# ChenWu98/cycle-diffusion

Measured on NVIDIA H100. Metric: images/sec (512x512, 50-step encode+decode) at 1/2/4/8 H100; ms/U-Net-call, higher is better.
Workload: dtype fp32

## Files before the change

cycle_diffusion_b200/_cabi.py:

```python
import ctypes as C
import os

HERE = os.path.dirname(os.path.abspath(__file__))
LIB_PATH = os.path.join(HERE, 'libcdx.so')

CDX_UNET_OPENAI = 1
CDX_UNET_IDDPM = 2
CDX_UNET_DDPM = 3
CDX_TEXT_OPENCLIP = 4
CDX_PRED_EPS = 0
CDX_PRED_V = 1


class UnetConfig(C.Structure):
    _fields_ = [('kind', C.c_int), ('in_channels', C.c_int), ('out_channels', C.c_int), ('model_channels', C.c_int),
                ('num_res_blocks', C.c_int), ('n_mult', C.c_int), ('channel_mult', C.c_int * 8), ('n_attn', C.c_int),
                ('attention_ds', C.c_int * 8), ('num_heads', C.c_int), ('num_head_channels', C.c_int),
                ('context_dim', C.c_int)]


class VaeConfig(C.Structure):
    _fields_ = [('ch', C.c_int), ('n_mult', C.c_int), ('ch_mult', C.c_int * 8), ('num_res_blocks', C.c_int),
                ('in_channels', C.c_int), ('out_ch', C.c_int), ('z_channels', C.c_int), ('embed_dim', C.c_int), ('vq', C.c_int), ('n_embed', C.c_int)]


class TextConfig(C.Structure):
    _fields_ = [('vocab_size', C.c_int), ('width', C.c_int), ('layers', C.c_int), ('heads', C.c_int), ('max_len', C.c_int),
                ('mlp_width', C.c_int), ('kind', C.c_int), ('dim_head', C.c_int), ('proj_dim', C.c_int), ('patch', C.c_int), ('image_size', C.c_int)]


class DdimCoef(C.Structure):
    _fields_ = [('sqrt_at', C.c_float), ('sqrt_1m_at', C.c_float), ('sqrt_1m_at_tab', C.c_float),
                ('sqrt_aprev', C.c_float), ('dir_coef', C.c_float), ('sigma', C.c_float)]


class PixelCoef(C.Structure):
    _fields_ = [('ddpm', C.c_int), ('sqrt_at', C.c_float), ('sqrt_1m_at', C.c_float), ('sqrt_at_next', C.c_float),
                ('c1', C.c_float), ('c2', C.c_float), ('w0', C.c_float), ('wt', C.c_float), ('post_std', C.c_float),
                ('weight', C.c_float), ('inv_sqrt_1m_bt', C.c_float), ('std_model', C.c_float), ('mask', C.c_float)]


_P = C.c_void_p


class AttnControl(C.Structure):
    _fields_ = [('cross_steps', C.c_int), ('self_steps', C.c_int), ('self_max_tokens', C.c_int), ('token_map', C.c_void_p)]


class GemmDesc(C.Structure):
    _fields_ = [('mode', C.c_int), ('M', C.c_int), ('N', C.c_int), ('K', C.c_int),
                ('A', _P), ('lda', C.c_int), ('C1', C.c_int), ('A2', _P), ('lda2', C.c_int), ('C2', C.c_int),
                ('Hin', C.c_int), ('Win', C.c_int), ('Hout', C.c_int), ('Wout', C.c_int), ('stride', C.c_int), ('pad', C.c_int),
                ('w', _P), ('ldb', C.c_int), ('b_kn', C.c_int), ('bias', _P),
                ('rowvec', _P), ('ld_rowvec', C.c_int), ('rows_per_batch', C.c_int), ('residual', _P), ('ldr', C.c_int),
                ('alpha', C.c_float), ('geglu', C.c_int), ('out_nchw', C.c_int), ('rows_per_img', C.c_int),
                ('C', _P), ('ldc', C.c_int), ('C_lo', _P), ('Ct_hi', _P), ('Ct_lo', _P), ('t_col0', C.c_int), ('ldt', C.c_int64),
                ('a_amax', _P), ('a2_amax', _P), ('c_amax', _P), ('c_stats', _P), ('w_range', C.c_float),
                ('batch', C.c_int), ('heads', C.c_int),
                ('sA_b', C.c_int64), ('sA_h', C.c_int64), ('sB_b', C.c_int64), ('sB_h', C.c_int64), ('sC_b', C.c_int64), ('sC_h', C.c_int64),
                ('up', C.c_int)]


class AttentionNetDesc(C.Structure):
    _fields_ = [('kind', C.c_int), ('causal', C.c_int), ('qkv', C.c_void_p), ('q', C.c_void_p), ('kv', C.c_void_p), ('k', C.c_void_p),
                ('v', C.c_void_p), ('B', C.c_int), ('N', C.c_int), ('L', C.c_int), ('ctx_lp', C.c_int), ('heads', C.c_int), ('d', C.c_int),
                ('scale', C.c_float), ('qk_rows', C.POINTER(C.c_int)), ('kv_rows', C.POINTER(C.c_int)), ('acc_rows', C.POINTER(C.c_int)),
                ('n_acc', C.c_int), ('slot', C.c_float), ('q_slot', C.c_float), ('out', C.c_void_p),
                ('probe_rows', C.POINTER(C.c_int)), ('probe_spans', C.POINTER(C.c_int)), ('n_probe', C.c_int), ('probe_map', C.c_void_p)]


class LatentChain(C.Structure):
    _fields_ = [('row', C.c_int), ('row2', C.c_int), ('scale', C.c_float)]


class LatentChainsDesc(C.Structure):
    _fields_ = [('chw', C.c_int), ('n_src', C.c_int), ('K', C.c_int), ('rows', C.c_int), ('chains', C.POINTER(LatentChain)), ('src', C.c_int),
                ('x0', _P), ('eout', _P), ('c', DdimCoef), ('noise0', _P), ('sa', C.c_float), ('s1', C.c_float), ('xt', _P), ('xn', _P),
                ('next', C.c_int), ('noise_next', _P), ('cnext', DdimCoef), ('xn2', _P), ('z_out', _P), ('z_stride', C.c_int64),
                ('eps_in', _P), ('eps_stride', C.c_int64), ('yt', _P), ('y_out', _P), ('xin', _P), ('pred', C.c_int), ('vsa', C.c_float),
                ('vs1', C.c_float), ('mask', _P), ('hw', C.c_int),
                ('sg_m', C.c_int), ('sg_rows', C.POINTER(C.c_int)), ('sg_thr', _P), ('sg_nu', _P), ('sg_scale', C.c_float * 8),
                ('sg_lambda', C.c_float * 8), ('sg_active', C.c_uint), ('sg_apply', C.c_int), ('sg_mu', C.c_float), ('sg_beta', C.c_float),
                ('sg_beta1', C.c_float)]


class LatentChainsMaskDesc(LatentChainsDesc):
    _fields_ = [('sg_map', _P), ('sg_mask', C.c_int), ('sg_gh', C.c_int), ('sg_gw', C.c_int), ('w', C.c_int)]


class DpmCoef(C.Structure):
    _fields_ = [('a', C.c_float), ('b', C.c_float), ('c', C.c_float), ('n', C.c_float), ('order', C.c_int)]


class LatentChainsSamplerDesc(LatentChainsMaskDesc):
    _fields_ = [('solver', C.c_int), ('dc', DpmCoef), ('d_src', _P), ('d_tgt', _P), ('qa', C.c_float), ('q1', C.c_float)]


CDX_SAMPLER_DDIM_POSTERIOR = 0
CDX_SAMPLER_DDIM_DRAWS = 1
CDX_SAMPLER_DPMSOLVER_DRAWS = 2


class SamplerC(C.Structure):
    _fields_ = [('kind', C.c_int), ('dpm', C.POINTER(DpmCoef)), ('qa', C.POINTER(C.c_float)), ('q1', C.POINTER(C.c_float))]


class MutualControlC(C.Structure):
    _fields_ = [('start_step', C.c_int), ('start_layer', C.c_int)]


class PnpControlC(C.Structure):
    _fields_ = [('feature_steps', C.c_int), ('attention_steps', C.c_int), ('attention_start_layer', C.c_int),
                ('feature_blocks', C.POINTER(C.c_int)), ('n_feature_blocks', C.c_int)]


CDX_SEMANTIC_MAX = 8


class SemanticGuidanceC(C.Structure):
    _fields_ = [('m', C.c_int), ('scale', C.c_float * CDX_SEMANTIC_MAX), ('threshold', C.c_float * CDX_SEMANTIC_MAX),
                ('cooldown', C.c_int * CDX_SEMANTIC_MAX), ('warmup', C.c_int), ('momentum_scale', C.c_float), ('beta', C.c_float),
                ('beta1', C.c_float)]


class SemanticAttnMaskC(C.Structure):
    _fields_ = [('intersect', C.c_int), ('n_tokens', C.c_int * CDX_SEMANTIC_MAX)]


_F = C.c_float
_I = C.c_int
_S = C.c_size_t

SIGNATURES = {
    'cdx_abi_version': (_I, []),
    'cdx_last_error': (C.c_char_p, []),
    'cdx_engine_create': (_I, [_I, C.POINTER(_P)]),
    'cdx_engine_destroy': (None, [_P]),
    'cdx_engine_workspace_bytes': (_S, [_P]),
    'cdx_engine_launch_count': (C.c_uint64, [_P]),
    'cdx_engine_set_mma_mode': (_I, [_P, _I]),
    'cdx_engine_profile': (_I, [_P, _I]),
    'cdx_engine_profile_read': (_I, [_P, _I, C.POINTER(C.c_double), C.POINTER(C.c_double), C.POINTER(C.c_double), C.POINTER(C.c_uint64)]),
    'cdx_unet_create': (_I, [_P, C.POINTER(UnetConfig), C.POINTER(_P)]),
    'cdx_vae_create': (_I, [_P, C.POINTER(VaeConfig), C.POINTER(_P)]),
    'cdx_text_create': (_I, [_P, C.POINTER(TextConfig), C.POINTER(_P)]),
    'cdx_net_destroy': (None, [_P]),
    'cdx_net_num_params': (_I, [_P]),
    'cdx_net_param_name': (C.c_char_p, [_P, _I]),
    'cdx_net_param_shape': (_I, [_P, _I, C.POINTER(C.c_int64)]),
    'cdx_net_load_param': (_I, [_P, C.c_char_p, _P, _I, C.POINTER(C.c_int64), _I]),
    'cdx_net_finalize': (_I, [_P]),
    'cdx_net_weight_blob': (_I, [_P, C.POINTER(_P), C.POINTER(_S)]),
    'cdx_net_adopt_blob': (_I, [_P]),
    'cdx_unet_set_time_freqs': (_I, [_P, C.POINTER(_F), _I]),
    'cdx_unet_set_prediction': (_I, [_P, _I, C.POINTER(_F), C.POINTER(_F), _I]),
    'cdx_unet_forward': (_I, [_P, _P, _P, _P, _I, _P, _I, _I, _I, _P]),
    'cdx_vae_encode': (_I, [_P, _P, _P, _I, _I, _P]),
    'cdx_text_encode': (_I, [_P, _P, _I, _I, _P, _P]),
    'cdx_vae_decode': (_I, [_P, _P, _P, _I, _I, _P]),
    'cdx_vae_encode_hw': (_I, [_P, _P, _P, _I, _I, _I, _P]),
    'cdx_vae_decode_hw': (_I, [_P, _P, _P, _I, _I, _I, _P]),
    'cdx_affine': (_I, [_P, _P, _F, _F, _P, _S, _P]),
    'cdx_shift_scale': (_I, [_P, _P, _F, _F, _P, _S, _P]),
    'cdx_q_sample': (_I, [_P, _P, _P, _F, _F, _P, _S, _P]),
    'cdx_vae_posterior': (_I, [_P, _P, _P, _F, _P, _I, _I, _I, _P]),
    'cdx_ddim_posterior_sample': (_I, [_P, _P, _P, _P, C.POINTER(DdimCoef), _P, _S, _P]),
    'cdx_ddim_compute_eps': (_I, [_P, _P, _P, _P, _P, _F, C.POINTER(DdimCoef), _P, _S, _P]),
    'cdx_ddim_step_with_eps': (_I, [_P, _P, _P, _P, _F, _P, C.POINTER(DdimCoef), _P, _S, _P]),
    'cdx_pixel_posterior_sample': (_I, [_P, _P, _P, _P, C.POINTER(PixelCoef), _P, _S, _P]),
    'cdx_pixel_compute_eps': (_I, [_P, _P, _P, _P, C.POINTER(PixelCoef), _P, _I, _I, _I, _P]),
    'cdx_pixel_step_with_eps': (_I, [_P, _P, _P, _P, C.POINTER(PixelCoef), _P, _I, _I, _I, _P]),
    'cdx_latent_encode': (_I, [_P, _P, _P, _P, _I, _F, C.POINTER(DdimCoef), C.POINTER(_F), _I, _I, _P, _F, _F, _P, _I, _I,
                               _I, _I, _P]),
    'cdx_latent_decode': (_I, [_P, _P, _I, _P, _P, _I, _F, C.POINTER(DdimCoef), C.POINTER(_F), _I, _P, _P, _I, _I, _I, _I,
                               _P]),
    'cdx_cycle_lockstep': (_I, [_P, _P, _P, _P, _P, _I, _F, _F, C.POINTER(DdimCoef), C.POINTER(_F), _I, _P, _F, _F, _P, _P, _I, _I, _I, _I,
                                _P]),
    'cdx_cycle_lockstep_masked': (_I, [_P, _P, _P, _P, _P, _I, _F, _F, C.POINTER(DdimCoef), C.POINTER(_F), _I, _P, _F, _F, _P, _P, _I, _I, _I,
                                       _I, _P, _P]),
    'cdx_cycle_lockstep_ctl': (_I, [_P, _P, _P, _P, _P, _I, _F, _F, C.POINTER(DdimCoef), C.POINTER(_F), _I, _P, _F, _F, _P, _P, _I, _I, _I,
                                    _I, _P, _P, C.POINTER(AttnControl)]),
    'cdx_cycle_lockstep_refine': (_I, [_P, _P, _P, _P, _P, _I, _F, _F, C.POINTER(DdimCoef), C.POINTER(_F), _I, _P, _F, _F, _P, _P, _I, _I,
                                       _I, _I, _P, _P, C.POINTER(AttnControl), _P]),
    'cdx_cycle_lockstep_mutual': (_I, [_P, _P, _P, _P, _P, _I, _F, _F, C.POINTER(DdimCoef), C.POINTER(_F), _I, _P, _F, _F, _P, _P, _I, _I,
                                       _I, _I, _P, _P, _I, _I]),
    'cdx_cycle_lockstep_pnp': (_I, [_P, _P, _P, _P, _P, _I, _F, _F, C.POINTER(DdimCoef), C.POINTER(_F), _I, _P, _F, _F, _P, _P, _I, _I,
                                    _I, _I, _P, _P, _I, _I, _I, C.POINTER(_I), _I]),
    'cdx_cycle_lockstep_semantic': (_I, [_P, _P, _P, _P, _P, _I, _F, _F, C.POINTER(DdimCoef), C.POINTER(_F), _I, _P, _F, _F, _P, _P, _I, _I,
                                         _I, _I, _P, _P, _P, C.POINTER(SemanticGuidanceC)]),
    'cdx_cycle_lockstep_semantic_attn': (_I, [_P, _P, _P, _P, _P, _I, _F, _F, C.POINTER(DdimCoef), C.POINTER(_F), _I, _P, _F, _F, _P, _P, _I,
                                              _I, _I, _I, _P, _P, _P, C.POINTER(SemanticGuidanceC), C.POINTER(SemanticAttnMaskC)]),
    'cdx_cycle_lockstep_sampler': (_I, [_P, _P, _P, _P, _P, _I, _F, _F, C.POINTER(DdimCoef), C.POINTER(_F), _I, _P, _F, _F, _P, _P, _I, _I,
                                        _I, _I, _P, C.POINTER(SamplerC), _P, C.POINTER(AttnControl), _P, C.POINTER(MutualControlC),
                                        C.POINTER(PnpControlC), _P, C.POINTER(SemanticGuidanceC), C.POINTER(SemanticAttnMaskC)]),
    'cdx_mask_pool': (_I, [_P, _P, _P, _I, _I, _I, _I, _P]),
    'cdx_mask_composite': (_I, [_P, _P, _P, _P, _P, _I, _I, _I, _I, _P]),
    'cdx_edit_map': (_I, [_P, _P, _P, _P, _I, _F, _F, _F, _P, _I, _I, _P, _I, _I, _I, _I, _P]),
    'cdx_edit_map_from_eps': (_I, [_P, _P, _P, _F, _I, _I, _P, _I, _I, _I, _I, _P]),
    'cdx_edit_mask': (_I, [_P, _P, _I, _F, _P, _P, _P, _I, _I, _I, _I, _I, _P]),
    'cdx_latent_loop_ens': (_I, [_P, _I, _P, _P, _P, _P, _I, _P, _P, C.POINTER(DdimCoef), C.POINTER(_F), _I, _I, _P, _F, _F, _P, _I, _P, _P, _P,
                                 _I, _I, _I, _I, _P]),
    'cdx_clip_preprocess': (_I, [_P, _P, _I, _I, _I, _P, _P]),
    'cdx_clip_image_features': (_I, [_P, _P, _I, _P, _P]),
    'cdx_text_features': (_I, [_P, _P, _I, _I, _P, _P]),
    'cdx_dclip_scores': (_I, [_P, _P, _P, _P, _P, _I, _I, _P, _P, _P]),
    'cdx_image_metrics': (_I, [_P, _P, _P, _I, _I, _I, _P, _P]),
    'cdx_pixel_encode': (_I, [_P, _P, C.POINTER(PixelCoef), C.POINTER(_F), _I, _P, _F, _F, _P, _I, _I, _I, _P]),
    'cdx_pixel_decode': (_I, [_P, _P, _I, C.POINTER(PixelCoef), C.POINTER(_F), _I, _P, _P, _I, _I, _I, _P]),
    'cdx_pixel_cycle_lockstep': (_I, [_P, _P, _P, C.POINTER(PixelCoef), C.POINTER(_F), _I, _I, _P, _F, _F, _P, _I, _I, _I, _P]),
    'cdx_latent_cycle_pair': (_I, [_P, _P, _P, C.POINTER(DdimCoef), C.POINTER(_F), _I, _I, _P, _F, _F, _P, _P, _I, _I, _I, _I, _P]),
    'cdx_latent_cycle_fan': (_I, [_P, _I, _I, _P, _P, _P, _P, _I, C.POINTER(_F), C.POINTER(_F), C.POINTER(DdimCoef), C.POINTER(_F), _I, _P,
                                  _F, _F, _P, _P, _I, _I, _I, _P]),
    'cdx_latent_cycle_fan_masked': (_I, [_P, _I, _I, _P, _P, _P, _P, _I, C.POINTER(_F), C.POINTER(_F), C.POINTER(DdimCoef), C.POINTER(_F), _I,
                                         _P, _F, _F, _P, _P, _I, _I, _I, _P, _P]),
    'cdx_ensemble_select': (_I, [_P, _I, _P, _P, _P, _P, _P, _P, _P, _P, _I, _I, _I, _I, _P]),
    'cdx_op_conv3x3': (_I, [_P, _P, _P, _P, _P, _I, _I, _I, _I, _I, _I, _I, _I, _P]),
    'cdx_op_linear': (_I, [_P, _P, _P, _P, _P, _I, _I, _I, _P]),
    'cdx_op_groupnorm': (_I, [_P, _P, _P, _P, _F, _I, _P, _I, _I, _I, _P]),
    'cdx_op_layernorm': (_I, [_P, _P, _P, _P, _P, _I, _I, _P]),
    'cdx_op_attention': (_I, [_P, _P, _P, _P, _P, _I, _I, _I, _I, _I, _F, _P]),
    'cdx_op_attention_rows': (_I, [_P, _P, _P, _P, _P, _I, _I, _I, _I, _I, _F, C.POINTER(_I), _P]),
    'cdx_op_attention_kv_rows': (_I, [_P, _P, _P, _P, _P, _I, _I, _I, _I, _I, _F, C.POINTER(_I), _P]),
    'cdx_op_attention_accum': (_I, [_P, _P, _P, _P, _P, _I, _I, _I, _I, _I, _F, C.POINTER(_I), _I, _P]),
    'cdx_op_nchw_to_nhwc': (_I, [_P, _P, _P, _I, _I, _I, _P]),
    'cdx_op_nhwc_to_nchw': (_I, [_P, _P, _P, _I, _I, _I, _P]),
    'cdx_op_groupnorm_ex': (_I, [_P, _P, _I, _P, _I, _P, _P, _F, _I, _P, _P, _I, _P, _P, _P, _I, _I, _P]),
    'cdx_op_groupnorm_rows': (_I, [_P, _P, _I, _P, _I, _P, _P, _F, _I, _P, _P, _I, C.POINTER(_I), _P, _P, _P, _P, _I, _I, _P]),
    'cdx_op_layernorm_ex': (_I, [_P, _P, _P, _P, _P, _P, _I, _I, _P]),
    'cdx_op_softmax_rows': (_I, [_P, _P, C.c_int64, _I, _I, _I, _P]),
    'cdx_op_produce_norm': (_I, [_P, _P, _P, _P, _I, _I, _I, _I, _I, _I, _P, _P, _F, _P, _P, _P, _P, C.POINTER(_I), _P]),
    'cdx_op_gemm': (_I, [_P, C.POINTER(GemmDesc), C.POINTER(_I), _P]),
    'cdx_op_attention_net': (_I, [_P, C.POINTER(AttentionNetDesc), C.POINTER(_I), _P]),
    'cdx_op_latent_chains': (_I, [_P, C.POINTER(LatentChainsDesc), _I, _P]),
    'cdx_op_pixel_lockstep': (_I, [_P, _P, _P, _P, _P, _P, _P, C.POINTER(PixelCoef), _I, _I, _I, _I, _P]),
}


def _load():
    if not os.path.exists(LIB_PATH):
        raise ImportError(
            f'{LIB_PATH} is missing: build it with `python -c "import __graft_entry__ as g; g.build()"` '
            f'(nvcc, sm_90a).  The engine has no CPU fallback.')
    lib = C.CDLL(LIB_PATH)
    for name, (res, args) in SIGNATURES.items():
        fn = getattr(lib, name)
        fn.restype = res
        fn.argtypes = args
    return lib


lib = _load()


class CdxError(RuntimeError):
    pass


def check(rc):
    if rc == 0:
        return
    msg = (lib.cdx_last_error() or b'').decode('utf-8', 'replace')
    if rc == -1:
        raise AssertionError(msg)
    raise CdxError(f'libcdx error {rc}: {msg}')
```

cycle_diffusion_b200/csrc/cabi.cu:

```cuda
#include <stdio.h>
#include <stdlib.h>
#include <string.h>

#include <algorithm>

#include "nets.cuh"

struct cdx_engine { cdx::Engine e; };
struct cdx_net { cdx::Net* n; cdx_engine* owner; };

namespace cdx {
const std::string& last_error();

namespace {

template <class F>
int guard(F&& f) {
  try {
    f();
    return CDX_OK;
  } catch (const Error& err) {
    set_last_error(err.what());
    return err.code;
  } catch (const std::exception& err) {
// ... 220 lines not shown
              p.start_layer >= 0 && p.n_blocks >= 0 && (p.blocks || p.n_blocks == 0),
              "Plug-and-Play: feature_steps=%d attention_steps=%d (of %d) attention_start_layer=%d n_blocks=%d", p.feature_steps,
              p.attention_steps, a.n_steps, p.start_layer, p.n_blocks);
    const int n_out = unet.ucfg.n_mult * (unet.ucfg.num_res_blocks + 1);
    for (int i = 0; i < p.n_blocks; ++i) {
      CDX_CHECK(p.blocks[i] >= 0 && p.blocks[i] < n_out, "Plug-and-Play: feature block %d outside the net's %d output blocks", p.blocks[i], n_out);
      for (int j = 0; j < i; ++j) CDX_CHECK(p.blocks[j] != p.blocks[i], "Plug-and-Play: feature block %d given twice", p.blocks[i]);
    }
  }
  const int solver = a.sampler ? a.sampler->kind : 0;
  if (solver) {
    const cdx_sampler& sp = *a.sampler;
    CDX_CHECK(solver == CDX_SAMPLER_DDIM_DRAWS || solver == CDX_SAMPLER_DPMSOLVER_DRAWS, "sampler: kind %d", solver);
    CDX_CHECK(a.src && a.K > 0 && a.n_rec == a.n_steps && !tgt_net && a.noise,
              "edit-friendly inversion: needs the lock-step loop with a source chain at every step");
    CDX_CHECK(sp.qa && sp.q1 && sp.qa[0] == a.sa && sp.q1[0] == a.s1,
              "edit-friendly inversion: the draw scalars qa / q1 must be given, their step 0 the x_T scalars");
    if (solver == CDX_SAMPLER_DPMSOLVER_DRAWS) {
      CDX_CHECK(sp.dpm, "SDE-DPM-Solver++: null coefficient table");
      for (int i = 0; i < a.n_steps; ++i) {
        const cdx_dpm_coef& d = sp.dpm[i];
        CDX_CHECK(d.n > 0.f && std::isfinite(d.n) && (d.order == 1 || d.order == 2), "SDE-DPM-Solver++: step %d n=%g order %d", i, d.n, d.order);
        CDX_CHECK(i > 0 || d.order == 1, "SDE-DPM-Solver++: order %d on the loop's first step (no previous x0-prediction)", d.order);
      }
    }
  }
  Scope sc(e.arena);
  unet.ctxkv.valid = false;
  struct Invalidate { Net& u; ~Invalidate() { u.ctxkv.valid = false; } } inval{unet};
  float* xin = (float*)e.arena.alloc((size_t)rows * chw * sizeof(float));
  float* eout = (float*)e.arena.alloc((size_t)rows * chw * sizeof(float));
  float* ctx_in = (float*)e.arena.alloc((size_t)rows * ctx_n * sizeof(float));
  float* xb[3] = {nullptr, nullptr, nullptr};
  float* yb[2] = {nullptr, nullptr};
  if (a.src) for (float*& p : xb) p = (float*)e.arena.alloc(n * sizeof(float));
  if (a.K) for (float*& p : yb) p = (float*)e.arena.alloc((size_t)n_tgt_chains * chw * sizeof(float));
  float* tdev = (float*)e.arena.alloc((size_t)std::max(loop_steps, 1) * rows * sizeof(float));
  Chain* chd = (Chain*)e.arena.alloc(ch.size() * sizeof(Chain));
  upload_timesteps(e, a.t_host, loop_steps, rows, tdev, s);
  if (!e.dry()) {
    CDX_CUDA(cudaMemcpyAsync(chd, ch.data(), ch.size() * sizeof(Chain), cudaMemcpyHostToDevice, s));
    auto scales_to = [&](Chain* c, const float* scales, int count) {
      CDX_CUDA(cudaMemcpy2DAsync(&c->scale, sizeof(Chain), scales, sizeof(float), sizeof(float), count, cudaMemcpyDeviceToDevice, s));
    };
    if (a.scales_on_device && a.src) scales_to(chd, a.s_scales, a.n_src);
    if (a.scales_on_device && a.K) scales_to(chd + a.n_src, a.t_scales, n_tgt_chains);
  }
  if (ctx_n) {
    auto ctx_rows = [&](const Chain& c, const float* cond, int j) {
      const bool uncond_only = a.uc && !a.scales_on_device && c.scale == 0.0f;
      copy_dd(e, (uncond_only ? a.uc : cond) + j * ctx_n, ctx_in + (size_t)c.row * ctx_n, ctx_n, s);
      if (c.row2 >= 0) copy_dd(e, a.uc + j * ctx_n, ctx_in + (size_t)c.row2 * ctx_n, ctx_n, s);
    };
    for (int j = 0; j < a.n_src; ++j) {
      if (a.src) ctx_rows(ch[j], a.c_src, j);
      for (int k = 0; k < a.K; ++k) ctx_rows(ch[a.n_src + (size_t)j * a.K + k], a.c_tgt, j);
    }
    for (int t = 0; t < n_tgt_chains; ++t)
      for (int q = 0; q < sg_m; ++q)
        copy_dd(e, a.c_edit + ((size_t)(t / a.K) * sg_m + q) * ctx_n, ctx_in + (size_t)sg_rows[(size_t)t * sg_m + q] * ctx_n, ctx_n, s);
  }
  int* sg_rows_dev = nullptr;
  float *sg_thr = nullptr, *sg_nu = nullptr;
  AttnProbe probe;
  const int sg_mask = a.sega_mask ? 1 + (a.sega_mask->intersect != 0) : 0, gh = a.h / 4, gw = a.w / 4;
  if (sg_m) {
    sg_rows_dev = (int*)e.arena.alloc(sg_rows.size() * sizeof(int));
    sg_thr = (float*)e.arena.alloc(sg_rows.size() * std::max(a.C, 2) * sizeof(float));
    sg_nu = (float*)e.arena.alloc((size_t)n_tgt_chains * chw * sizeof(float));
    if (!e.dry()) {
      CDX_CUDA(cudaMemcpyAsync(sg_rows_dev, sg_rows.data(), sg_rows.size() * sizeof(int), cudaMemcpyHostToDevice, s));
      CDX_CUDA(cudaMemsetAsync(sg_nu, 0, (size_t)n_tgt_chains * chw * sizeof(float), s));
    }
  }
  if (sg_mask) {
    std::vector<int> span(sg_rows.size());
    for (size_t r = 0; r < span.size(); ++r) span[r] = a.sega_mask->n_tokens[r % sg_m];
    int* span_dev = (int*)e.arena.alloc(span.size() * sizeof(int));
    if (!e.dry()) CDX_CUDA(cudaMemcpyAsync(span_dev, span.data(), span.size() * sizeof(int), cudaMemcpyHostToDevice, s));
    probe.rows = sg_rows_dev; probe.span = span_dev; probe.n_rows = (int)sg_rows.size(); probe.tokens = gh * gw;
    probe.map = (float*)e.arena.alloc(sg_rows.size() * gh * gw * sizeof(float));
  }
  AttnControl actl;
  if (a.ctl) {
    std::vector<int> qk(rows);
    for (int r = 0; r < rows; ++r) qk[r] = r;
    for (int j = 0; j < a.n_src; ++j) {
      CDX_CHECK(!a.uc || ch[j].scale != 0.0f, "attention control: the source chain at scale 0 has no source-prompt row");
      for (int k = 0; k < a.K; ++k) {
        const Chain& t = ch[a.n_src + (size_t)j * a.K + k];
        CDX_CHECK(!a.uc || t.scale != 0.0f, "attention control: the target chain at scale 0 has no target-prompt row");
        qk[t.row] = ch[j].row;
      }
    }
    int* qk_dev = (int*)e.arena.alloc((size_t)rows * sizeof(int));
    if (!e.dry()) CDX_CUDA(cudaMemcpyAsync(qk_dev, qk.data(), qk.size() * sizeof(int), cudaMemcpyHostToDevice, s));
    actl.qk_row = qk_dev;
    actl.self_max_tokens = a.ctl->self_max_tokens;
    auto ctx_products = [&](const float* A, float* out) {
      const int D = unet.ucfg.context_dim;
      ExactFp32 exact(e);
      for (int j = 0; j < a.n_src; ++j)
        for (int k = 0; k < a.K; ++k) {
          GemmArgs g;
          g.mode = 0;
          g.M = a.L; g.N = D; g.K = a.L;
          g.A = A + (size_t)j * a.L * a.L; g.lda = a.L; g.C1 = a.L;
          g.Bw = a.c_tgt + (size_t)j * ctx_n; g.ldb = D; g.b_kn = 1;
          g.Cout = out + (size_t)ch[a.n_src + (size_t)j * a.K + k].row * ctx_n; g.ldc = D;
          gemm(e, g, s);
        }
    };
    if (a.ctl->token_map) {
      float* cv = (float*)e.arena.alloc((size_t)rows * ctx_n * sizeof(float));
      copy_dd(e, ctx_in, cv, (size_t)rows * ctx_n, s);
      ctx_products(a.ctl->token_map, cv);
      actl.ctx_v = cv;
    }
    if (a.own_weight) {
      float* cw = (float*)e.arena.alloc((size_t)rows * ctx_n * sizeof(float));
      float* dg = (float*)e.arena.alloc((size_t)a.n_src * a.L * a.L * sizeof(float));
      std::vector<int> own;
      for (int j = 0; j < a.n_src; ++j)
        for (int k = 0; k < a.K; ++k) own.push_back(ch[a.n_src + (size_t)j * a.K + k].row);
      int* own_dev = (int*)e.arena.alloc(own.size() * sizeof(int));
      if (!e.dry()) {
        CDX_CUDA(cudaMemcpyAsync(own_dev, own.data(), own.size() * sizeof(int), cudaMemcpyHostToDevice, s));
        CDX_CUDA(cudaMemsetAsync(cw, 0, (size_t)rows * ctx_n * sizeof(float), s));
        CDX_CUDA(cudaMemsetAsync(dg, 0, (size_t)a.n_src * a.L * a.L * sizeof(float), s));
        for (int j = 0; j < a.n_src; ++j)
          CDX_CUDA(cudaMemcpy2DAsync(dg + (size_t)j * a.L * a.L, (size_t)(a.L + 1) * sizeof(float), a.own_weight + (size_t)j * a.L, sizeof(float),
                                     sizeof(float), a.L, cudaMemcpyDeviceToDevice, s));
      }
      ctx_products(dg, cw);
      actl.ctx_w = cw;
      actl.own_rows = own_dev;
      actl.n_own = (int)own.size();
    }
  }
  if (a.mutual || a.pnp) {
    std::vector<int> src_row(rows);
    for (int r = 0; r < rows; ++r) src_row[r] = r;
    for (int j = 0; j < a.n_src; ++j)
      for (int k = 0; k < a.K; ++k) {
        const Chain& t = ch[a.n_src + (size_t)j * a.K + k];
        src_row[t.row] = ch[j].row;
        if (t.row2 >= 0) src_row[t.row2] = ch[j].row2 >= 0 ? ch[j].row2 : ch[j].row;
      }
    int* dev = (int*)e.arena.alloc((size_t)rows * sizeof(int));
    if (!e.dry()) CDX_CUDA(cudaMemcpyAsync(dev, src_row.data(), src_row.size() * sizeof(int), cudaMemcpyHostToDevice, s));
    if (a.mutual) {
      actl.kv_row = dev;
      actl.start_layer = a.start_layer;
    } else {
      actl.pnp_row = dev;
      actl.pnp_layer = a.pnp->start_layer;
      actl.feat_blocks = a.pnp->blocks;
      actl.n_feat = a.pnp->n_blocks;
    }
  }
  auto next_kind = [&](int i_next) {
    if (i_next >= a.n_rec) return 0;
    return (a.n_steps - 1 - i_next) == 0 ? 2 : solver ? 3 : 1;
  };
  float *d_src = nullptr, *d_tgt = nullptr;
  if (solver == CDX_SAMPLER_DPMSOLVER_DRAWS) {
    d_src = (float*)e.arena.alloc(n * sizeof(float));
    d_tgt = (float*)e.arena.alloc((size_t)n_tgt_chains * chw * sizeof(float));
  }
  const int n_given = a.src ? a.n_rec : a.n_eps;
  LatentChains f;
  f.n = n; f.chw = chw; f.n_src = a.n_src; f.K = a.K; f.chains = chd; f.x0 = a.x0; f.xin = xin; f.mask = a.mask; f.hw = a.h * a.w;
  f.z_stride = (long long)(a.n_rec + 1) * chw;
  f.solver = solver; f.d_src = d_src; f.d_tgt = d_tgt;
  if (sg_m) {
    const cdx_semantic_guidance& g = *a.sega;
    f.sg_m = sg_m; f.sg_rows = sg_rows_dev; f.sg_thr = sg_thr; f.sg_nu = sg_nu;
    for (int q = 0; q < sg_m; ++q) { f.sg_scale[q] = g.scale[q]; f.sg_lambda[q] = g.threshold[q]; }
    f.sg_mu = g.momentum_scale; f.sg_beta = g.beta; f.sg_beta1 = g.beta1;
    f.sg_mask = sg_mask; f.sg_map = probe.map; f.sg_gh = gh; f.sg_gw = gw; f.w = a.w;
  }
  {
    LatentChains in = f;
    in.src = a.src;
    in.noise0 = a.noise; in.sa = a.sa; in.s1 = a.s1; in.z_out = a.z_out;
    in.eps_in = a.z_in; in.eps_stride = (long long)(a.n_eps + 1) * chw;
    in.xt = xb[0]; in.xn = xb[1]; in.yt = yb[0];
    in.next = a.src ? next_kind(0) : 0;
    if (in.next) { in.noise_next = a.noise + n; in.cnext = a.coef[0]; }
    if (in.next == 3) { in.qa = a.sampler->qa[1]; in.q1 = a.sampler->q1[1]; }
    latent_chains_init(e, in, s);
  }
  const int iters = e.dry() ? std::min(loop_steps, 1) : loop_steps;
  PairStreams ps(e, tgt_net ? *tgt_net->eng : e, s);
  for (int i = 0; i < iters; ++i) {
    const bool src_i = a.src && i < a.n_rec;
    if (!tgt_net) {
      actl.cross = a.ctl && i < a.ctl->cross_steps;
      actl.self = a.ctl && i < a.ctl->self_steps;
      actl.mutual = a.mutual && i >= a.start_step;
      actl.pnp_feat = a.pnp && i < a.pnp->feature_steps;
      actl.pnp_attn = a.pnp && i < a.pnp->attention_steps;
      const size_t stat0 = e.stat_dry;
      unet_forward(unet, xin, tdev + (size_t)i * rows, ctx_in, a.L, eout, rows, a.h, a.w, s, true,
                   a.ctl || a.mutual || a.pnp ? &actl : nullptr, sg_mask ? &probe : nullptr);
      CDX_CHECK(!sg_m || !e.dry() || e.stat_dry - stat0 <= e.stat_cap,
                "semantic guidance: a %d-row U-Net call needs %zu GroupNorm statistics doubles, the pool holds %zu: fewer images or concepts",
                rows, e.stat_dry - stat0, e.stat_cap);
    } else {
      ps.fork();
      if (src_i) unet_forward(unet, xin, tdev + (size_t)i * rows, nullptr, 0, eout, rows_src, a.h, a.w, s);
      unet_forward(*tgt_net, xin + (size_t)rows_src * chw, tdev + (size_t)i * rows + rows_src, nullptr, 0, eout + (size_t)rows_src * chw,
                   rows - rows_src, a.h, a.w, ps.target_stream());
      ps.join();
    }
    LatentChains st = f;
    st.src = src_i; st.eout = eout; st.c = a.coef[i];
    if (src_i) {
      st.xt = xb[0]; st.xn = xb[1]; st.xn2 = xb[2];
      if (a.z_out) st.z_out = a.z_out + (size_t)(1 + i) * chw;
      st.next = next_kind(i + 1);
      if (st.next) { st.noise_next = a.noise + (size_t)(2 + i) * n; st.cnext = a.coef[i + 1]; }
      if (st.next == 3) { st.qa = a.sampler->qa[i + 2]; st.q1 = a.sampler->q1[i + 2]; }
      if (solver == CDX_SAMPLER_DPMSOLVER_DRAWS) st.dc = a.sampler->dpm[i];
    } else if (i < n_given) {
      st.eps_in = a.z_in + (size_t)(1 + i) * chw; st.eps_stride = (long long)(a.n_eps + 1) * chw;
    } else {
      st.eps_in = a.extra + (size_t)(i - n_given) * n; st.eps_stride = chw;
    }
    st.yt = yb[0]; st.y_out = (i == loop_steps - 1) ? a.x_out : yb[1];
    set_v(unet, a.t_host[i], st);
    if (sg_m) {
      for (int q = 0; q < sg_m; ++q) st.sg_active |= (unsigned)(i < a.sega->cooldown[q]) << q;
      st.sg_apply = i >= a.sega->warmup;
      semantic_thresholds(e, st, s);
    }
    latent_chains_step(e, st, s);
    if (src_i) { float* t0 = xb[0]; xb[0] = xb[1]; xb[1] = xb[2]; xb[2] = t0; }
    std::swap(yb[0], yb[1]);
  }
}

void run_edit_map(Net& unet, const float* x0, const float* c_src, const float* c_tgt, int L, float t, float sa, float s1, const float* noise,
                  int n_maps, int rows_per_call, float* acc, int B, int C, int h, int w, cudaStream_t s) {
  Engine& e = *unet.eng;
  const int chw = C * h * w, hw = h * w, n_pairs = n_maps * B, per_call = std::min(rows_per_call / 2, n_pairs), rows = 2 * per_call;
  const size_t ctx_n = (size_t)L * unet.ucfg.context_dim;
  check_v_steps(unet, &t, 1);
  const float vscale = unet.pred ? unet.sa_v[(int)t] : 1.f;
  Scope sc(e.arena);
  float* xin = (float*)e.arena.alloc((size_t)rows * chw * sizeof(float));
  float* eout = (float*)e.arena.alloc((size_t)rows * chw * sizeof(float));
  float* ctx_in = (float*)e.arena.alloc((size_t)rows * ctx_n * sizeof(float));
  float* tdev = (float*)e.arena.alloc((size_t)rows * sizeof(float));
  upload_timesteps(e, &t, 1, rows, tdev, s);
  if (!e.dry()) CDX_CUDA(cudaMemsetAsync(acc, 0, (size_t)B * hw * sizeof(float), s));
  const int calls = e.dry() ? 1 : cdiv(n_pairs, per_call);
  for (int c = 0; c < calls; ++c) {
    const int p0 = c * per_call, p1 = std::min(p0 + per_call, n_pairs), nr = 2 * (p1 - p0);
    for (int q = p0; q < p1; ++q) {
      const int b = q % B, r = 2 * (q - p0);
      copy_dd(e, c_src + (size_t)b * ctx_n, ctx_in + (size_t)r * ctx_n, ctx_n, s);
      copy_dd(e, c_tgt + (size_t)b * ctx_n, ctx_in + (size_t)(r + 1) * ctx_n, ctx_n, s);
    }
    edit_rows(e, x0, noise, sa, s1, xin, B, n_maps, chw, p0, p1, s);
    const size_t stat0 = e.stat_dry;
    unet_forward(unet, xin, tdev, ctx_in, L, eout, nr, h, w, s);
    CDX_CHECK(!e.dry() || e.stat_dry - stat0 <= e.stat_cap,
              "edit_map: a %d-row U-Net call needs %zu GroupNorm statistics doubles, the pool holds %zu: lower rows_per_call", nr,
              e.stat_dry - stat0, e.stat_cap);
    edit_map_accum(e, eout, eout + chw, 2LL * chw, 2LL * B * chw, 2LL * p0 * chw, vscale, acc, B, C, hw, p0, p1, s);
  }
}

}
}

using namespace cdx;

static inline cdx::Engine& engine_of(cdx_engine* h) { return h->e; }

extern "C" {

int cdx_abi_version(void) { return CDX_ABI_VERSION; }
const char* cdx_last_error(void) { return cdx::last_error().c_str(); }

int cdx_engine_create(int device, cdx_engine** out) {
  return guard([&] {
    CDX_CHECK(out != nullptr, "engine_create: null out");
    int count = 0;
    cudaError_t err = cudaGetDeviceCount(&count);
    if (err != cudaSuccess || count <= 0)
      throw Error(CDX_E_CUDA, std::string("no usable CUDA device (there is no CPU fallback): ") + cudaGetErrorString(err));
    CDX_CHECK(device >= 0 && device < count, "engine_create: device %d out of range (count %d)", device, count);
    CDX_CUDA(cudaSetDevice(device));
    cudaDeviceProp prop;
    CDX_CUDA(cudaGetDeviceProperties(&prop, device));
    cdx_engine* eng = new cdx_engine();
    eng->e.device = device;
    if (prop.major != 9 || prop.minor != 0)
      throw Error(CDX_E_CUDA, "libcdx is built for sm_90a (H100) only; device " + std::to_string(device) + " is sm_" +
                                  std::to_string(prop.major) + std::to_string(prop.minor));
    eng->e.num_sms = prop.multiProcessorCount;
    *out = eng;
  });
}
void cdx_engine_destroy(cdx_engine* e) {
  if (!e) return;
  cudaSetDevice(e->e.device);
  cudaDeviceSynchronize();
  e->e.arena.destroy();
  if (e->e.done_ev) cudaEventDestroy(e->e.done_ev);
  if (e->e.side) cudaStreamDestroy(e->e.side);
  if (e->e.fork_ev) cudaEventDestroy(e->e.fork_ev);
  if (e->e.join_ev) cudaEventDestroy(e->e.join_ev);
  if (e->e.amax_pool) cudaFree(e->e.amax_pool);
  delete e;
}
size_t cdx_engine_workspace_bytes(const cdx_engine* e) { return e ? e->e.arena.cap : 0; }
uint64_t cdx_engine_launch_count(const cdx_engine* e) { return e ? e->e.launches : 0; }
int cdx_engine_set_mma_mode(cdx_engine* e, int mode) {
  return guard([&] {
    CDX_CHECK(e != nullptr && mode >= 0 && mode <= 5, "set_mma_mode: bad arguments");
    e->e.mma_mode = mode == 0 ? 0 : 1;
    e->e.flash_attn = mode != 2 && mode != 0;
    e->e.tc_kind = mode == 3 ? 0 : mode >= 4 ? 2 : 1;
    e->e.attn_one = mode == 5;
  });
}

int cdx_engine_profile(cdx_engine* e, int enable) {
  return guard([&] {
    CDX_CHECK(e != nullptr, "profile: null engine");
    CDX_CUDA(cudaSetDevice(e->e.device));
    CDX_CUDA(cudaDeviceSynchronize());
    for (ProfRec& r : e->e.prof.recs) { cudaEventDestroy(r.a); cudaEventDestroy(r.b); }
    e->e.prof.recs.clear();
    e->e.prof.on = enable != 0;
  });
}
int cdx_engine_profile_read(cdx_engine* e, int tag, double* ms, double* flops, double* bytes, uint64_t* launches) {
  return guard([&] {
    CDX_CHECK(e && ms && flops && bytes && launches && tag >= 0 && tag < PROF_NTAGS, "profile_read: bad arguments");
    CDX_CUDA(cudaSetDevice(e->e.device));
    CDX_CUDA(cudaDeviceSynchronize());
    *ms = 0; *flops = 0; *bytes = 0; *launches = 0;
    const bool dump = getenv("CDX_PROF_DUMP") != nullptr;
    for (const ProfRec& r : e->e.prof.recs) {
      if (r.tag != tag) continue;
      float t = 0.f;
      CDX_CUDA(cudaEventElapsedTime(&t, r.a, r.b));
      if (dump) fprintf(stderr, "[cdx prof] tag %d  %8.3f ms  %8.1f GFLOP  %7.1f TF/s  %s\n", tag, t, r.flops * 1e-9, t > 0 ? r.flops / (t * 1e9) : 0.0, r.note);
      *ms += t; *flops += r.flops; *bytes += r.bytes; *launches += (uint64_t)r.launches;
    }
  });
}

int cdx_unet_create(cdx_engine* e, const cdx_unet_config* cfg, cdx_net** out) {
  return guard([&] {
    CDX_CHECK(cfg && out, "unet_create: null argument");
    cdx_net* h = new cdx_net();
    h->owner = e;
    static Engine host_only;
    h->n = make_unet(e ? &e->e : &host_only, *cfg);
    *out = h;
  });
}
int cdx_vae_create(cdx_engine* e, const cdx_vae_config* cfg, cdx_net** out) {
  return guard([&] {
    CDX_CHECK(cfg && out, "vae_create: null argument");
    cdx_net* h = new cdx_net();
    h->owner = e;
    static Engine host_only;
    h->n = make_vae(e ? &e->e : &host_only, *cfg);
    *out = h;
  });
}
int cdx_text_create(cdx_engine* e, const cdx_text_config* cfg, cdx_net** out) {
  return guard([&] {
    CDX_CHECK(cfg && out, "text_create: null argument");
    cdx_net* h = new cdx_net();
    h->owner = e;
    static Engine host_only;
    h->n = make_text(e ? &e->e : &host_only, *cfg);
    *out = h;
  });
}
void cdx_net_destroy(cdx_net* n) {
  if (!n) return;
  destroy_net(n->n);
  delete n;
}
int cdx_net_num_params(const cdx_net* n) { return n ? (int)n->n->params.size() : 0; }
const char* cdx_net_param_name(const cdx_net* n, int i) {
  if (!n || i < 0 || i >= (int)n->n->params.size()) return nullptr;
  return n->n->params[i].name.c_str();
}
int cdx_net_param_shape(const cdx_net* n, int i, int64_t dims[4]) {
  if (!n || i < 0 || i >= (int)n->n->params.size()) return CDX_E_INVALID;
  const Param& p = n->n->params[i];
  for (int k = 0; k < 4; ++k) dims[k] = k < p.rank ? p.dims[k] : 1;
  return p.rank;
}
int cdx_net_load_param(cdx_net* n, const char* name, const float* data, int on_device, const int64_t* dims, int rank) {
  return guard([&] {
    CDX_CHECK(n && n->owner && name && data && dims, "load_param: null argument (nets created without an engine are inventory-only)");
    net_load_param(*n->n, name, data, on_device != 0, dims, rank);
  });
}
int cdx_net_finalize(cdx_net* n) {
  return guard([&] {
    CDX_CHECK(n && n->owner, "finalize: null / inventory-only net");
    net_finalize(*n->n);
  });
}
int cdx_net_weight_blob(cdx_net* n, void** dev_ptr, size_t* bytes) {
  return guard([&] {
    CDX_CHECK(n && n->owner && dev_ptr && bytes, "weight_blob: null argument");
    net_ensure_blob(*n->n);
    *dev_ptr = n->n->blob;
    *bytes = n->n->blob_floats * sizeof(float);
  });
}
int cdx_net_adopt_blob(cdx_net* n) {
  return guard([&] {
    CDX_CHECK(n && n->owner, "adopt_blob: null / inventory-only net");
    net_ensure_blob(*n->n);
    for (Param& p : n->n->params) p.loaded = true;
    n->n->planes_valid = false;
    n->n->ctxkv.valid = false;
    n->n->finalized = false;
    net_finalize(*n->n);
  });
}
int cdx_unet_set_time_freqs(cdx_net* n, const float* freqs, int half) {
  return guard([&] {
    CDX_CHECK(n && freqs, "set_time_freqs: null argument");
    CDX_CHECK(n->n->kind != NET_VAE, "set_time_freqs on a VAE");
    CDX_CHECK(half == n->n->ucfg.model_channels / 2, "set_time_freqs: half=%d, expected %d", half, n->n->ucfg.model_channels / 2);
    n->n->freqs_host.assign(freqs, freqs + half);
    if (n->n->finalized) net_finalize(*n->n);
  });
}

int cdx_unet_set_prediction(cdx_net* n, int prediction, const float* sa_v, const float* s1_v, int T) {
  return guard([&] {
    CDX_CHECK(n && n->n, "set_prediction: null net");
    CDX_CHECK(n->n->kind == NET_UNET_OPENAI, "set_prediction: SD / LDM U-Nets only");
    CDX_CHECK(prediction == CDX_PRED_EPS || prediction == CDX_PRED_V, "set_prediction: prediction %d", prediction);
    if (prediction == CDX_PRED_EPS) {
      n->n->pred = 0; n->n->sa_v.clear(); n->n->s1_v.clear();
      return;
    }
    CDX_CHECK(sa_v && s1_v && T > 0, "set_prediction: v needs both tables");
    n->n->sa_v.assign(sa_v, sa_v + T);
    n->n->s1_v.assign(s1_v, s1_v + T);
    n->n->pred = 1;
  });
}

int cdx_unet_forward(cdx_net* n, const float* x, const float* t_dev, const float* ctx, int ctx_len, float* out, int B, int H, int W,
                     void* stream) {
  return guard([&] {
    CDX_CHECK(n && n->owner && x && t_dev && out && B > 0, "unet_forward: bad arguments");
    with_arena(n->owner->e, S(stream), [&] { unet_forward(*n->n, x, t_dev, ctx, ctx_len, out, B, H, W, S(stream)); });
  });
}
int cdx_vae_encode_hw(cdx_net* n, const float* img, float* moments, int B, int H, int W, void* stream) {
  return guard([&] {
    CDX_CHECK(n && n->owner && img && moments && B > 0, "vae_encode: bad arguments");
    with_arena(n->owner->e, S(stream), [&] { vae_encode(*n->n, img, moments, B, H, W, S(stream)); });
  });
}
int cdx_vae_encode(cdx_net* n, const float* img, float* moments, int B, int R, void* stream) {
  return cdx_vae_encode_hw(n, img, moments, B, R, R, stream);
}
int cdx_text_encode(cdx_net* n, const int* ids, int B, int L, float* out, void* stream) {
  return guard([&] {
    CDX_CHECK(n && n->owner && ids && out && B > 0, "text_encode: bad arguments");
    with_arena(n->owner->e, S(stream), [&] { text_encode(*n->n, ids, out, B, L, S(stream)); });
  });
}
#define ENG_CALL_(EH_, ...)                                \
  return guard([&] {                                       \
    CDX_CHECK((EH_) != nullptr, "null engine");            \
    CDX_CUDA(cudaSetDevice(engine_of(EH_).device));        \
    __VA_ARGS__;                                           \
  })
int cdx_text_features(cdx_net* n, const int* ids, int B, int L, float* out, void* stream) {
  return guard([&] {
    CDX_CHECK(n && n->owner && ids && out && B > 0, "text_features: bad arguments");
    with_arena(n->owner->e, S(stream), [&] { text_features(*n->n, ids, out, B, L, S(stream)); });
  });
}
int cdx_clip_image_features(cdx_net* n, const float* pixels, int B, float* out, void* stream) {
  return guard([&] {
    CDX_CHECK(n && n->owner && pixels && out && B > 0, "clip_image_features: bad arguments");
    with_arena(n->owner->e, S(stream), [&] { clip_image_features(*n->n, pixels, out, B, S(stream)); });
  });
}
int cdx_clip_preprocess(cdx_engine* e, const float* img, int B, int R, int size, float* out, void* s) {
  ENG_CALL_(e, CDX_CHECK(img && out && B > 0 && R > 0 && size > 0, "clip_preprocess: bad arguments"); clip_preprocess(e->e, img, B, R, size, out, S(s)));
}
int cdx_dclip_scores(cdx_engine* e, const float* img_f, const float* orig_f, const float* enc_f, const float* dec_f, int B, int D, float* clip_out,
                     float* dclip_out, void* s) {
  ENG_CALL_(e, CDX_CHECK(img_f && orig_f && enc_f && dec_f && clip_out && dclip_out && B > 0 && D > 0, "dclip_scores: bad arguments");
            dclip_scores(e->e, img_f, orig_f, enc_f, dec_f, B, D, clip_out, dclip_out, S(s)));
}
int cdx_image_metrics(cdx_engine* eh, const float* a, const float* b, int B, int H, int W, float* out, void* stream) {
  return guard([&] {
    CDX_CHECK(eh && a && b && out && B > 0, "image_metrics: bad arguments");
    with_arena(eh->e, S(stream), [&] { image_metrics(eh->e, a, b, B, H, W, out, S(stream)); });
  });
}
int cdx_vae_decode_hw(cdx_net* n, const float* z, float* img, int B, int h, int w, void* stream) {
  return guard([&] {
    CDX_CHECK(n && n->owner && z && img && B > 0, "vae_decode: bad arguments");
    with_arena(n->owner->e, S(stream), [&] { vae_decode(*n->n, z, img, B, h, w, S(stream)); });
  });
}
int cdx_vae_decode(cdx_net* n, const float* z, float* img, int B, int h, void* stream) {
  return cdx_vae_decode_hw(n, z, img, B, h, h, stream);
}

#define ENG_CALL(EH_, ...)                                 \
  return guard([&] {                                       \
    CDX_CHECK((EH_) != nullptr, "null engine");            \
    CDX_CUDA(cudaSetDevice(engine_of(EH_).device));        \
    __VA_ARGS__;                                           \
  })

int cdx_affine(cdx_engine* e, const float* x, float a, float b, float* out, size_t n, void* s) { ENG_CALL(e, affine(e->e, x, a, b, out, n, S(s))); }
int cdx_shift_scale(cdx_engine* e, const float* x, float b, float a, float* out, size_t n, void* s) { ENG_CALL(e, shift_scale(e->e, x, b, a, out, n, S(s))); }
int cdx_q_sample(cdx_engine* e, const float* x0, const float* nz, float sa, float s1, float* out, size_t n, void* s) {
  ENG_CALL(e, q_sample(e->e, x0, nz, sa, s1, out, n, S(s)));
}
int cdx_vae_posterior(cdx_engine* e, const float* mom, const float* nz, float sf, float* out, int B, int C, int hw, void* s) {
  ENG_CALL(e, vae_posterior(e->e, mom, nz, sf, out, B, C, hw, S(s)));
}
int cdx_ddim_posterior_sample(cdx_engine* e, const float* x0, const float* xt, const float* nz, const cdx_ddim_coef* c, float* o, size_t n, void* s) {
  ENG_CALL(e, CDX_CHECK(c, "null coef"); ddim_posterior_sample(e->e, x0, xt, nz, *c, o, n, S(s)));
}
int cdx_ddim_compute_eps(cdx_engine* e, const float* xt, const float* xn, const float* e_c, const float* e_uc, float scale, const cdx_ddim_coef* c,
                         float* o, size_t n, void* s) {
  ENG_CALL(e, CDX_CHECK(c, "null coef"); ddim_compute_eps(e->e, xt, xn, e_c, e_uc, scale, *c, o, n, S(s)));
}
int cdx_ddim_step_with_eps(cdx_engine* e, const float* x, const float* e_c, const float* e_uc, float scale, const float* eps, const cdx_ddim_coef* c,
                           float* o, size_t n, void* s) {
  ENG_CALL(e, CDX_CHECK(c, "null coef"); ddim_step_with_eps(e->e, x, e_c, e_uc, scale, eps, *c, o, n, S(s)));
}
int cdx_pixel_posterior_sample(cdx_engine* e, const float* x0, const float* xt, const float* nz, const cdx_pixel_coef* c, float* o, size_t n, void* s) {
  ENG_CALL(e, CDX_CHECK(c, "null coef"); pixel_posterior_sample(e->e, x0, xt, nz, *c, o, n, S(s)));
}
int cdx_pixel_compute_eps(cdx_engine* e, const float* xt, const float* xn, const float* et, const cdx_pixel_coef* c, float* o, int B, int chw,
                          int net_chw, void* s) {
  ENG_CALL(e, CDX_CHECK(c, "null coef"); pixel_compute_eps(e->e, xt, xn, et, *c, o, B, chw, net_chw, S(s)));
}
int cdx_pixel_step_with_eps(cdx_engine* e, const float* xt, const float* et, const float* eps, const cdx_pixel_coef* c, float* o, int B, int chw,
                            int net_chw, void* s) {
  ENG_CALL(e, CDX_CHECK(c, "null coef"); pixel_step_with_eps(e->e, xt, et, eps, *c, o, B, chw, net_chw, S(s)));
}

int cdx_latent_encode(cdx_net* un, const float* x0, const float* c, const float* uc, int L, float scale, const cdx_ddim_coef* coef,
                      const float* t_host, int n_steps, int n_rec, const float* noise, float sqrt_a_T, float sqrt_1ma_T, float* z_out, int B,
                      int C, int h, int w, void* stream) {
  return guard([&] {
    CDX_CHECK(un && un->owner && x0 && (c || L == 0) && coef && t_host && noise && z_out, "latent_encode: null argument");
    CDX_CHECK(n_steps >= 1 && n_rec >= 0 && n_rec <= n_steps, "latent_encode: n_steps=%d n_rec=%d", n_steps, n_rec);
    for (int i = 0; i < n_rec; ++i) CDX_CHECK(coef[i].sigma > 0.f, "latent_encode: eta must be > 0 (sigma[%d] == 0), ddim.py:268", i);
    const std::vector<float> scales((size_t)std::max(B, 0), scale);
    ChainLoopArgs a;
    a.n_src = B; a.src = true;
    a.x0 = x0; a.c_src = c; a.uc = uc; a.L = L; a.s_scales = scales.data();
    a.coef = coef; a.t_host = t_host; a.n_steps = n_steps; a.n_rec = n_rec; a.noise = noise; a.sa = sqrt_a_T; a.s1 = sqrt_1ma_T;
    a.z_out = z_out; a.C = C; a.h = h; a.w = w;
    with_arena(un->owner->e, S(stream), [&] { run_latent_chains(*un->n, a, S(stream)); });
  });
}

int cdx_latent_decode(cdx_net* un, const float* z, int n_eps, const float* c, const float* uc, int L, float scale, const cdx_ddim_coef* coef,
                      const float* t_host, int n_steps, const float* extra_noise, float* x_out, int B, int C, int h, int w, void* stream) {
  return guard([&] {
    CDX_CHECK(un && un->owner && z && (c || L == 0) && coef && t_host && x_out, "latent_decode: null argument");
    CDX_CHECK(n_steps >= 1 && n_eps >= 0, "latent_decode: n_steps=%d n_eps=%d", n_steps, n_eps);
    CDX_CHECK(n_eps >= n_steps || extra_noise != nullptr, "latent_decode: %d steps but only %d recovered noises and no extra noise", n_steps, n_eps);
    const std::vector<float> scales((size_t)std::max(B, 0), scale);
    ChainLoopArgs a;
    a.n_src = B; a.K = 1;
    a.c_tgt = c; a.uc = uc; a.L = L; a.t_scales = scales.data();
    a.coef = coef; a.t_host = t_host; a.n_steps = n_steps;
    a.z_in = z; a.n_eps = n_eps; a.extra = extra_noise; a.x_out = x_out;
    a.C = C; a.h = h; a.w = w;
    with_arena(un->owner->e, S(stream), [&] { run_latent_chains(*un->n, a, S(stream)); });
  });
}

int cdx_cycle_lockstep(cdx_net* un, const float* x0, const float* c_src, const float* c_tgt, const float* uc, int L, float src_scale,
                       float tgt_scale, const cdx_ddim_coef* coef, const float* t_host, int n_steps, const float* noise, float sqrt_a_T,
                       float sqrt_1ma_T, float* x_out, float* z_out, int B, int C, int h, int w, void* stream) {
  return cdx_cycle_lockstep_masked(un, x0, c_src, c_tgt, uc, L, src_scale, tgt_scale, coef, t_host, n_steps, noise, sqrt_a_T, sqrt_1ma_T,
                                   x_out, z_out, B, C, h, w, stream, nullptr);
}

int cdx_cycle_lockstep_masked(cdx_net* un, const float* x0, const float* c_src, const float* c_tgt, const float* uc, int L, float src_scale,
                              float tgt_scale, const cdx_ddim_coef* coef, const float* t_host, int n_steps, const float* noise,
                              float sqrt_a_T, float sqrt_1ma_T, float* x_out, float* z_out, int B, int C, int h, int w, void* stream,
                              const float* mask) {
  return cdx_cycle_lockstep_ctl(un, x0, c_src, c_tgt, uc, L, src_scale, tgt_scale, coef, t_host, n_steps, noise, sqrt_a_T, sqrt_1ma_T,
                                x_out, z_out, B, C, h, w, stream, mask, nullptr);
}

int cdx_cycle_lockstep_ctl(cdx_net* un, const float* x0, const float* c_src, const float* c_tgt, const float* uc, int L, float src_scale,
                           float tgt_scale, const cdx_ddim_coef* coef, const float* t_host, int n_steps, const float* noise,
                           float sqrt_a_T, float sqrt_1ma_T, float* x_out, float* z_out, int B, int C, int h, int w, void* stream,
                           const float* mask, const cdx_attn_control* ctl) {
  return cdx_cycle_lockstep_refine(un, x0, c_src, c_tgt, uc, L, src_scale, tgt_scale, coef, t_host, n_steps, noise, sqrt_a_T, sqrt_1ma_T,
                                   x_out, z_out, B, C, h, w, stream, mask, ctl, nullptr);
}

static int cycle_lockstep(cdx_net* un, const float* x0, const float* c_src, const float* c_tgt, const float* uc, int L, float src_scale,
                          float tgt_scale, const cdx_ddim_coef* coef, const float* t_host, int n_steps, const float* noise, float sqrt_a_T,
                          float sqrt_1ma_T, float* x_out, float* z_out, int B, int C, int h, int w, void* stream, const float* mask,
                          const cdx_attn_control* ctl, const float* own_weight, bool mutual, int start_step, int start_layer,
                          const PnpLoop* pnp = nullptr, const cdx_semantic_guidance* sega = nullptr, const float* c_edit = nullptr,
                          const cdx_semantic_attn_mask* sega_mask = nullptr, const cdx_sampler* sampler = nullptr) {
  return guard([&] {
    CDX_CHECK(un && un->owner && x0 && c_src && c_tgt && coef && t_host && noise && x_out, "cycle_lockstep: null argument");
    CDX_CHECK(n_steps >= 1, "cycle_lockstep: n_steps=%d", n_steps);
    for (int i = 0; i < n_steps; ++i) CDX_CHECK(coef[i].sigma > 0.f, "cycle_lockstep: eta must be > 0 (sigma[%d] == 0), ddim.py:268", i);
    const std::vector<float> s_scales((size_t)std::max(B, 0), src_scale), t_scales((size_t)std::max(B, 0), tgt_scale);
// ... 911 lines not shown
```

cycle_diffusion_b200/csrc/common.cuh:

```cuda
#pragma once
#include <cuda_runtime.h>
#include <stdint.h>
#include <stdio.h>
#include <string>
#include <vector>
#include <stdexcept>

#include "../../include/cdx.h"

namespace cdx {

struct Error : std::runtime_error {
  int code;
  Error(int c, const std::string& m) : std::runtime_error(m), code(c) {}
};
void set_last_error(const std::string& m);

#define CDX_CHECK(cond, ...)                                                     \
  do {                                                                           \
    if (!(cond)) {                                                               \
      char _b[512];                                                              \
      snprintf(_b, sizeof(_b), __VA_ARGS__);                                     \
      throw ::cdx::Error(CDX_E_INVALID, std::string(_b) + " [" #cond "]");       \
    }                                                                            \
  } while (0)

#define CDX_CUDA(expr)                                                                         \
  do {                                                                                         \
    cudaError_t _e = (expr);                                                                   \
    if (_e != cudaSuccess) {                                                                   \
      char _b[512];                                                                            \
      snprintf(_b, sizeof(_b), "%s failed: %s (%s:%d)", #expr, cudaGetErrorString(_e), __FILE__, __LINE__); \
      throw ::cdx::Error(CDX_E_CUDA, _b);                                                      \
    }                                                                                          \
  } while (0)

struct Arena {
  char* base = nullptr;
  size_t cap = 0, off = 0, high = 0;
  bool dry = false;
  void* alloc(size_t bytes);
  size_t mark() const { return off; }
  void release(size_t m) { off = m; }
  void begin_dry();
  void end_dry();
  void destroy();
};

enum ProfTag {
  PROF_CONV_FFMA = 0, PROF_DENSE_FFMA = 1, PROF_BATCHED_FFMA = 2, PROF_CONV_TC = 3, PROF_DENSE_TC = 4, PROF_BATCHED_TC = 5,
  PROF_GROUPNORM = 6, PROF_LAYERNORM = 7, PROF_SOFTMAX = 8, PROF_ELEMENTWISE = 9, PROF_NTAGS = 10
};
struct ProfRec { cudaEvent_t a, b; int tag; double flops, bytes; int launches; char note[56]; };
struct Profiler {
  bool on = false;
  std::vector<ProfRec> recs;
  std::vector<cudaEvent_t> pool;
};

struct Engine {
  Profiler prof;
  int device = 0;
  int num_sms = 132;
  bool flash_attn = true;
  int mma_mode = 1;
  int tc_kind = 1;
  bool attn_one = false;
  float* amax_pool = nullptr;
  int amax_cap = 1 << 15, amax_used = 0, amax_high = 0;
  float* amax_slot();
  double* stat_pool = nullptr;
  size_t stat_cap = (size_t)8 << 20, stat_used = 0, stat_high = 0;
  size_t stat_dry = 0;
  double* stat_alloc(size_t n);
  void pools_reset(cudaStream_t s);
  Arena arena;
  cudaStream_t last_stream = nullptr;
  cudaEvent_t done_ev = nullptr;
  bool ev_recorded = false;
  cudaStream_t side = nullptr;
  cudaEvent_t fork_ev = nullptr, join_ev = nullptr;
  uint64_t launches = 0;
  bool dry() const { return arena.dry; }
};

struct ProfScope {
  Engine& e;
  cudaStream_t s;
  int idx = -1;
  ProfScope(Engine& eng, cudaStream_t st, int tag, double flops, double bytes, int launches);
  ~ProfScope();
  void note(const char* fmt, ...);
};

struct Scope {
  Arena& a;
  size_t m;
  explicit Scope(Arena& ar) : a(ar), m(ar.mark()) {}
  ~Scope() { a.release(m); }
};

struct Tensor {
  float* p = nullptr;
  int B = 0, H = 0, W = 0, C = 0;
  float* amax = nullptr;
  double* stats = nullptr;
  size_t numel() const { return (size_t)B * H * W * C; }
  int rows() const { return B * H * W; }
};
inline Tensor alloc_tensor(Engine& e, int B, int H, int W, int C) {
  Tensor t;
  t.B = B; t.H = H; t.W = W; t.C = C;
  t.p = (float*)e.arena.alloc(t.numel() * sizeof(float));
  return t;
}

struct GemmArgs {
  int M = 0, N = 0, K = 0;
  int mode = 0;
  const float* A = nullptr;  int lda = 0;  int C1 = 0;
  const float* A2 = nullptr; int lda2 = 0; int C2 = 0;
  int Hin = 0, Win = 0, Hout = 0, Wout = 0, stride = 1, pad = 1, up = 1;
  const float* Bw = nullptr; int ldb = 0; int b_kn = 0;
  const float* Bw_hi = nullptr; const float* Bw_lo = nullptr;
  const void* Bw_h_hi = nullptr; const void* Bw_h_lo = nullptr; int b_exp = 0;
  const float* a_amax = nullptr; const float* a2_amax = nullptr;
  float* c_amax = nullptr;
  double* c_stats = nullptr;
  float* Cout = nullptr; int ldc = 0;
  float* Cout_lo = nullptr;
  float* Ct_hi = nullptr; float* Ct_lo = nullptr; int t_col0 = 0; long long ldt = 0;
  const float* bias = nullptr;
  const float* rowvec = nullptr; int ld_rowvec = 0; int rows_per_batch = 1;
  const float* residual = nullptr; int ldr = 0;
  float alpha = 1.f;
  int geglu = 0;
  int out_nchw = 0;
  int rows_per_img = 0;
  int batch = 1, heads = 1;
  long long sA_b = 0, sA_h = 0, sB_b = 0, sB_h = 0, sC_b = 0, sC_h = 0;
};
void gemm(Engine& e, const GemmArgs& a, cudaStream_t s, int* route = nullptr);
bool gemm_tc(Engine& e, const GemmArgs& a, cudaStream_t s, int* side_done = nullptr);
enum { ROUTE_KIND_SS = 0, ROUTE_KIND_TS = 1, ROUTE_KIND_H16 = 2, ROUTE_KIND_H16_FAST = 3 };
inline int route_plan(int kind, int width, int splits) { return kind << 4 | width << 8 | splits << 16; }
bool flash_eligible(const Engine& e, int N, int Nk, int d, int C);
struct AttnPlanes {
  enum Fmt { TF32, H16 } fmt;
  const void* q_hi; const void* q_lo; int ldq;
  const void* k_hi; const void* k_lo; int ldk;
  const void* vt_hi; const void* vt_lo;
  const float* q_amax = nullptr; const float* k_amax = nullptr; const float* v_amax = nullptr;
};
bool flash_attention(Engine& e, const AttnPlanes& a, float* out, int ldo, int B, int N, int Nk, int Nks, int Nvs, int heads, int d, float scale,
                     cudaStream_t s, const int* qk_row = nullptr, const int* acc_rows = nullptr, int n_acc = 0, const int* kv_row = nullptr);
void split_rows_h16(Engine& e, const float* src, long long rows, int cols, long long ld, void* hi, void* lo, long long ldh, const float* amax,
                    cudaStream_t s);
void split_transpose_h16(Engine& e, const float* src, int R, int Cc, long long ld, void* hi, void* lo, const float* amax, cudaStream_t s,
                         int images = 1, int Rp = 0);
struct FlashPlan { int qrows, rag, ksplit, ring; };
FlashPlan flash_plan(int d, bool h16, bool one, int N);
bool self_attention_h16(Engine& e, const float* qkv, const float* slot, float* out, int B, int HW, int C, int heads, int d, float scale, bool lo,
                        cudaStream_t s, const int* qk_row, const int* kv_row, const int* acc_rows = nullptr, int n_acc = 0, int* Nvs_out = nullptr);
bool self_attention_tf32_padded(Engine& e, const float* qk_hi, const float* qk_lo, const float* vr, float* out, int B, int HW, int C, int heads,
                                int d, float scale, cudaStream_t s, const int* qk_row, const int* kv_row, const int* acc_rows = nullptr,
                                int n_acc = 0, int* Nvs_out = nullptr);
void context_split_h16(Engine& e, const float* kv, int Mk, int C, const float* slot, void* k_hi, void* k_lo, void* vt_hi, void* vt_lo,
                       cudaStream_t s);
struct ProbeOperands {
  enum Fmt { F32, H16, TF32 } fmt = F32;
  const float* q = nullptr; const float* q_lo = nullptr; int ldq = 0;
  const void* k = nullptr; const void* k_lo = nullptr; int ldk = 0; int Lk = 0;
  const float* k_amax = nullptr;
};
void attn_probe(Engine& e, const ProbeOperands& o, const int* rows, const int* span, int n_rows, float* map, int N, int L, int heads, int d,
                float scale, bool accumulate, cudaStream_t s);
void split_planes(Engine& e, const float* w, float* hi, float* lo, size_t n, cudaStream_t s);
void split_planes_h16(Engine& e, const float* w, void* hi, void* lo, size_t n, int exp, cudaStream_t s);
void amax_rows(Engine& e, const float* x, long long rows, int C, long long ld, float* slot, cudaStream_t s);
int h16_exp_host(float amax);
bool attention_tc(Engine& e, const float* q, int ldq, const float* k, int ldk, int head_stride, const float* vt, float* out, int ldo, int B,
                  int Nq, int Nk, int heads, int d, float scale, cudaStream_t s);

void groupnorm(Engine& e, const float* x1, int C1, const float* x2, int C2, const float* gamma, const float* beta,
               float eps, bool silu, const float* scale, const float* shift, int ld_ss, float* y, int B, int HW,
               cudaStream_t s, const double* st1 = nullptr, const double* st2 = nullptr, float* amax = nullptr, float2* ab_out = nullptr,
               const int* src_img = nullptr);
double* gn_channel_stats(Engine& e, const float* x, int C, int B, int HW, cudaStream_t s);
void gn_channel_stats_into(Engine& e, const float* x, int C, int B, int HW, double* stats, cudaStream_t s);
void layernorm(Engine& e, const float* x, const float* gamma, const float* beta, float* y, int M, int C, cudaStream_t s, float* amax = nullptr);
void softmax_rows(Engine& e, float* x, long long rows, int L, int ld, cudaStream_t s, int causal_nq = 0);
void silu(Engine& e, const float* x, float* y, size_t n, cudaStream_t s);
void geglu(Engine& e, const float* x, float* y, int M, int C, cudaStream_t s, bool interleaved = false);
void interleave_geglu_rows(Engine& e, const float* src, float* dst, int rows, int rowlen, cudaStream_t s);
void add(Engine& e, const float* a, const float* b, float* y, size_t n, cudaStream_t s);
void avgpool2(Engine& e, const float* x, float* y, int B, int H, int W, int C, cudaStream_t s);
void upsample2(Engine& e, const float* x, float* y, int B, int H, int W, int C, cudaStream_t s);
void nchw_to_nhwc(Engine& e, const float* x, float* y, int B, int C, int HW, cudaStream_t s);
void nhwc_to_nchw(Engine& e, const float* x, float* y, int B, int C, int HW, cudaStream_t s);
void timestep_embedding(Engine& e, const float* t, const float* freqs, float* emb, int B, int half, cudaStream_t s, bool sin_first = false);
void repack_conv3x3(Engine& e, const float* w, float* o, int O, int I, cudaStream_t s, int Ipad = 0);
void pad_channels(Engine& e, const float* x, float* y, size_t rows, int C, int Cp, cudaStream_t s);
void embed_tokens(Engine& e, const int* ids, const float* tok, const float* pos, float* out, int B, int L, int W, int vocab, cudaStream_t s);
void quick_gelu(Engine& e, const float* x, float* y, size_t n, cudaStream_t s);
void gelu(Engine& e, const float* x, float* y, size_t n, cudaStream_t s);
void copy_rows(Engine& e, const float* src, float* dst, size_t n, cudaStream_t s);
void vq_quantize(Engine& e, const float* z, const float* codebook, float* out, size_t npix, int dim, int n_embed, cudaStream_t s);
void clip_preprocess(Engine& e, const float* img, int B, int R, int size, float* out, cudaStream_t s);
void patchify(Engine& e, const float* img, float* out, int B, int S, int P, cudaStream_t s);
void vit_tokens(Engine& e, const float* patches, const float* cls, const float* pos, float* out, int B, int N, int W, cudaStream_t s);
void gather_rows(Engine& e, const float* x, const int* row_of_batch, float* out, int B, int L, int W, cudaStream_t s);
void eot_rows(Engine& e, const int* ids, int* rows, int B, int L, cudaStream_t s);
void dclip_scores(Engine& e, const float* img_f, const float* orig_f, const float* enc_f, const float* dec_f, int B, int D, float* clip_out,
                  float* dclip_out, cudaStream_t s);
void image_metrics(Engine& e, const float* a, const float* b, int B, int H, int W, float* out, cudaStream_t s);
void attention(Engine& e, const float* q, int ldq, const float* k, int ldk, const float* v, int ldv, float* out, int ldo,
               int B, int Nq, int Nk, int heads, int d, int head_stride, float scale, cudaStream_t s, bool causal = false);

void affine(Engine& e, const float* x, float a, float b, float* out, size_t n, cudaStream_t s);
void shift_scale(Engine& e, const float* x, float b, float a, float* out, size_t n, cudaStream_t s);
void q_sample(Engine& e, const float* x0, const float* noise, float sa, float s1ma, float* out, size_t n, cudaStream_t s);
void vae_posterior(Engine& e, const float* moments, const float* noise, float sf, float* out, int B, int C, int hw, cudaStream_t s);
void ddim_posterior_sample(Engine& e, const float* x0, const float* xt, const float* noise, const cdx_ddim_coef& c, float* out, size_t n, cudaStream_t s);
void ddim_compute_eps(Engine& e, const float* xt, const float* xt_next, const float* e_c, const float* e_uc, float scale,
                      const cdx_ddim_coef& c, float* out, size_t n, cudaStream_t s);
void ddim_step_with_eps(Engine& e, const float* x, const float* e_c, const float* e_uc, float scale, const float* eps,
                        const cdx_ddim_coef& c, float* out, size_t n, cudaStream_t s);
struct Chain { int row, row2; float scale; };
struct LatentChains {
  size_t n = 0; int chw = 0, n_src = 0, K = 0;
  const Chain* chains = nullptr;
  int src = 0;
  const float* x0 = nullptr;
  const float* eout = nullptr;
  cdx_ddim_coef c{};
  const float* noise0 = nullptr; float sa = 0.f, s1 = 0.f;
  float* xt = nullptr; float* xn = nullptr;
  int next = 0;
  const float* noise_next = nullptr; cdx_ddim_coef cnext{};
  float* xn2 = nullptr;
  float* z_out = nullptr; long long z_stride = 0;
  const float* eps_in = nullptr; long long eps_stride = 0;
  float* yt = nullptr; float* y_out = nullptr;
  float* xin = nullptr;
  int pred = 0; float vsa = 0.f, vs1 = 0.f;
  const float* mask = nullptr; int hw = 0;
  int sg_m = 0;
  const int* sg_rows = nullptr;
  float* sg_thr = nullptr;
  float* sg_nu = nullptr;
  float sg_scale[8] = {};
  float sg_lambda[8] = {};
  unsigned sg_active = 0;
  int sg_apply = 0;
  float sg_mu = 0.f, sg_beta = 0.f, sg_beta1 = 0.f;
  int sg_mask = 0;
  const float* sg_map = nullptr;
  int sg_gh = 0, sg_gw = 0;
  int w = 0;
  int solver = 0;
  cdx_dpm_coef dc{};
  float* d_src = nullptr; float* d_tgt = nullptr;
  float qa = 0.f, q1 = 0.f;
};
constexpr int SEMANTIC_MAX_CONCEPTS = 8;
void latent_chains_init(Engine& e, const LatentChains& a, cudaStream_t s);
void latent_chains_step(Engine& e, const LatentChains& a, cudaStream_t s);
void semantic_thresholds(Engine& e, const LatentChains& a, cudaStream_t s);
void mask_pool(Engine& e, const float* mask, float* out, int B, int H, int W, int f, cudaStream_t s);
void mask_composite(Engine& e, const float* dec, const float* image, const float* mask, float* out, int B, int C, int H, int W,
                    cudaStream_t s);
void edit_rows(Engine& e, const float* x0, const float* noise, float sa, float s1, float* xin, int B, int n_maps, int chw, int p0, int p1,
               cudaStream_t s);
void edit_map_accum(Engine& e, const float* src, const float* tgt, long long sb, long long sk, long long off0, float vscale, float* acc, int B,
                    int C, int hw, int p0, int p1, cudaStream_t s);
void edit_mask(Engine& e, const float* acc, int n_maps, float ratio, float* map_out, float* mask_out, float* img_out, int f, int B, int C, int h,
               int w, cudaStream_t s);
void ensemble_select(Engine& e, int n, const float* scores, const long long* cand, const int* sample, const float* images, float* best_score,
                     long long* best_idx, float* best_img, float* score_mat, int B, int n_total, size_t img_n, cudaStream_t s);

void pixel_posterior_sample(Engine& e, const float* x0, const float* xt, const float* noise, const cdx_pixel_coef& c, float* out, size_t n, cudaStream_t s);
void pixel_compute_eps(Engine& e, const float* xt, const float* xt_next, const float* et, const cdx_pixel_coef& c, float* out,
                       int B, int chw, int net_chw, cudaStream_t s);
void pixel_step_with_eps(Engine& e, const float* xt, const float* et, const float* eps, const cdx_pixel_coef& c, float* out,
                         int B, int chw, int net_chw, cudaStream_t s);
void pixel_lockstep_step(Engine& e, const float* x0, float* xs, float* ys, const float* et_src, const float* et_tgt, const float* noise,
                         const cdx_pixel_coef& c, int B, int chw, int net_chw_src, int net_chw_tgt, cudaStream_t s);

inline int cdiv(long long a, long long b) { return (int)((a + b - 1) / b); }

}
```

cycle_diffusion_b200/csrc/kernels_tc.cu:

```cuda
#include <algorithm>

#include <mutex>
#include <array>
#include <map>
#include <unordered_map>
#include <vector>
#include <cstdlib>
#include <cmath>
#include <type_traits>

#include <cuda_fp16.h>

#include "tc_common.cuh"

namespace cdx {
namespace {

using namespace tc;

constexpr int TBM = 128, TBN = 128, TBK = 32;
constexpr int TILE_BYTES = TBM * TBK * 4;
constexpr int TC_THREADS = 384;
constexpr int SMEM_MAX = 232448;
constexpr int BAR_BYTES = 256, ALIGN_SLACK = 1024;

enum { KIND_SS = 0, KIND_TS = 1, KIND_H16 = 2, KIND_H16_FAST = 3 };

template <int KIND, int BN>
struct Cfg {
  static constexpr bool H16 = KIND == KIND_H16 || KIND == KIND_H16_FAST;
  static constexpr int BK = TBK;
  static constexpr int KSTEPS = H16 ? 2 : 4;
  static constexpr int KCHUNK = 256 / BK;
  static constexpr int A_BYTES = TILE_BYTES;
  static constexpr int B_ROW = H16 ? 64 : 128;
  static constexpr int B_PLANE = BN * B_ROW;
  static constexpr int STAGE_BYTES = A_BYTES + 2 * B_PLANE;
  static constexpr int STAGES = (SMEM_MAX - BAR_BYTES - ALIGN_SLACK) / STAGE_BYTES;
  static constexpr int SMEM_BYTES = STAGES * STAGE_BYTES + BAR_BYTES + ALIGN_SLACK;
  static constexpr int EPI_BOX = TBM * TBK * 4;
  static constexpr int EPI_PER_SLOT = STAGE_BYTES / EPI_BOX;
  static constexpr int EPI_SLOTS = (BN / TBK + EPI_PER_SLOT - 1) / EPI_PER_SLOT;
  static_assert(STAGES >= 2 + EPI_SLOTS, "the epilogue's slots never include the last stages' slots");
  static_assert(STAGES >= 3 && (2 * STAGES + 1) * 8 <= BAR_BYTES, "barrier area holds a full and an empty barrier per stage and bar_res");
  static_assert(STAGE_BYTES % 1024 == 0 && B_PLANE % 1024 == 0, "stage and plane bases stay 1024-byte aligned (swizzle atoms)");
  static_assert(SMEM_BYTES <= SMEM_MAX, "smem overflow");
};

struct TcParams {
  int M, N, K;
  int mode;
  int C1, C2;
  int H, W, B;
  int bw, bh, bn;
  int tiles_x, tiles_y;
  int cstride, cpad;
  float* C; int ldc;
  float* C_lo;
  float* Ct_hi; float* Ct_lo; int t_col0; long long ldt;
  const float* bias;
  const float* rowvec; int ld_rowvec; int rows_per_batch;
  const float* residual; int ldr;
  float alpha;
  int geglu;
  int out_nchw, rows_per_img;
  int heads;
  int a_code[4], b_code[4];
  int a_rowoff_h, b_rowoff_h;
  long long sC_b, sC_h;
  int tiles_m, tiles_n, total_tiles;
  int tn_w;
  int splits, kb_per_split;
  float* ws;
  const float* a_amax; const float* a2_amax;
  int b_exp;
  float* c_amax;
  double* c_stats;
};

__host__ __device__ __forceinline__ bool staged_store(const TcParams& p) {
  return p.mode != 2 && p.splits == 1 && !p.out_nchw && !p.Ct_hi && !p.C_lo;
}

__device__ __forceinline__ int h16_a_exp(const TcParams& p) {
  float m = p.a_amax ? *p.a_amax : 0.f;
  if (p.a2_amax) m = fmaxf(m, *p.a2_amax);
  return h16_exp_of(m);
}

struct TileCoord { int n0, nend, m0, x0, y0, b0, zb, zh, kb0, kb1, split; };

constexpr int RASTER_M = 8;

__device__ __forceinline__ TileCoord tile_coord(const TcParams& p, int t, int num_kb) {
  TileCoord c;
  c.split = t % p.splits;
  t /= p.splits;
  c.kb0 = c.split * p.kb_per_split;
  c.kb1 = min(num_kb, c.kb0 + p.kb_per_split);
  const int per_z = p.tiles_m * p.tiles_n;
  const int z = t / per_z;
  int u = t - z * per_z;
  const int m_lo = u / (RASTER_M * p.tiles_n) * RASTER_M;
  const int bm = min(RASTER_M, p.tiles_m - m_lo);
  u -= m_lo * p.tiles_n;
  const int tm = m_lo + u % bm, tn = u / bm;
  c.n0 = tn * p.tn_w;
  c.nend = min(p.N, c.n0 + p.tn_w);
  c.m0 = 0; c.x0 = 0; c.y0 = 0; c.b0 = 0; c.zb = 0; c.zh = 0;
  if (p.mode == 1) {
    int u = tm;
    const int tx = u % p.tiles_x; u /= p.tiles_x;
    const int ty = u % p.tiles_y; u /= p.tiles_y;
    c.x0 = tx * p.bw; c.y0 = ty * p.bh; c.b0 = u * p.bn;
  } else {
    c.m0 = tm * TBM;
    c.zb = z / p.heads;
    c.zh = z - c.zb * p.heads;
  }
  return c;
}

__device__ __forceinline__ uint32_t tf32_lo(float x, uint32_t hi) { return rn_tf32(__float_as_uint(x - __uint_as_float(hi))); }

template <int KIND, int BN>
__global__ void __launch_bounds__(TC_THREADS, 1)
tc_gemm_kernel(const __grid_constant__ CUtensorMap mapA, const __grid_constant__ CUtensorMap mapA2,
               const __grid_constant__ CUtensorMap mapB, const __grid_constant__ CUtensorMap mapBlo,
               const __grid_constant__ CUtensorMap mapR, const __grid_constant__ CUtensorMap mapC, const TcParams p) {
  using CF = Cfg<KIND, BN>;
  constexpr bool H16 = CF::H16, FAST = KIND == KIND_H16_FAST;
  constexpr int BK = CF::BK, KSTEPS = CF::KSTEPS, A_BYTES = CF::A_BYTES, B_PLANE = CF::B_PLANE, STAGE_BYTES = CF::STAGE_BYTES;
  constexpr int STAGES = CF::STAGES, EPI_BOX = CF::EPI_BOX, EPI_PER_SLOT = CF::EPI_PER_SLOT, EPI_SLOTS = CF::EPI_SLOTS;
  constexpr int NACC = BN / 2;
  pdl_trigger();
  extern __shared__ uint8_t smem_raw[];
  const uint32_t base = (smem_u32(smem_raw) + 1023u) & ~1023u;
  const uint32_t bars = base + STAGES * STAGE_BYTES;
  auto bar_full = [&](int s) { return bars + 8u * s; };
  auto bar_empty = [&](int s) { return bars + 8u * (STAGES + s); };
  const uint32_t bar_res = bars + 16u * STAGES;

  const int warp = threadIdx.x >> 5, lane = threadIdx.x & 31;
  const int num_kb = (p.K + BK - 1) / BK;
  const TileCoord tc_ = tile_coord(p, blockIdx.x, num_kb);
  const int nst = tc_.kb1 - tc_.kb0;
  const bool staged = staged_store(p);
  auto epi_box = [&](int k) { return base + ((nst + k / EPI_PER_SLOT) % STAGES) * STAGE_BYTES + (k % EPI_PER_SLOT) * EPI_BOX; };

  if (threadIdx.x == 0) {
    for (int s = 0; s < STAGES; ++s) {
      mbar_init(bar_full(s), 1);
      mbar_init(bar_empty(s), 8);
    }
    mbar_init(bar_res, 1);
    asm volatile("fence.mbarrier_init.release.cluster;" ::: "memory");
  }
  __syncthreads();
  pdl_wait();

  if (warp < 4) {
    asm volatile("setmaxnreg.dec.sync.aligned.u32 40;");
    if (threadIdx.x == 0) {
      const int cblocks = p.mode == 1 ? p.C1 / TBK : 0;
      int it = 0;
      for (int kb = tc_.kb0; kb < tc_.kb1; ++kb, ++it) {
        const int s = it % STAGES;
        mbar_wait(bar_empty(s), ((it / STAGES) & 1) ^ 1);
        const uint32_t st = base + s * STAGE_BYTES;
        const uint32_t sb = st + A_BYTES;
        const int k0 = kb * BK;
        if (p.mode == 2) {
          mbar_expect_tx(bar_full(s), TILE_BYTES + BN * 128);
          int ca[4], cb4[4];
#pragma unroll
          for (int i = 0; i < 4; ++i) {
            const int ac = p.a_code[i], bc = p.b_code[i];
            ca[i] = ac == 0 ? k0 : ac == 1 ? tc_.m0 + tc_.zh * p.a_rowoff_h : ac == 2 ? tc_.zh : ac == 3 ? tc_.zb : 0;
            cb4[i] = bc == 0 ? k0 : bc == 1 ? tc_.n0 + tc_.zh * p.b_rowoff_h : bc == 2 ? tc_.zh : bc == 3 ? tc_.zb : 0;
          }
          tma_load_4d(st, &mapA, ca[0], ca[1], ca[2], ca[3], bar_full(s));
          tma_load_4d(sb, &mapB, cb4[0], cb4[1], cb4[2], cb4[3], bar_full(s));
          continue;
        }
        mbar_expect_tx(bar_full(s), TILE_BYTES + (KIND == KIND_SS ? 1 : 2) * B_PLANE);
        if (p.mode == 0) {
          if (k0 < p.C1) tma_load_2d(st, &mapA, k0, tc_.m0, bar_full(s));
          else tma_load_2d(st, &mapA2, k0 - p.C1, tc_.m0, bar_full(s));
        } else {
          const int tap = kb / cblocks, cb = kb - tap * cblocks;
          const int dy = tap / 3, dx = tap - dy * 3;
          tma_load_4d(st, &mapA, cb * TBK, tc_.x0 * p.cstride + dx - p.cpad, tc_.y0 * p.cstride + dy - p.cpad, tc_.b0,
                      bar_full(s));
        }
        tma_load_2d(sb, &mapB, k0, tc_.n0, bar_full(s));
        if (KIND != KIND_SS) tma_load_2d(sb + B_PLANE, &mapBlo, k0, tc_.n0, bar_full(s));
      }
      if (staged) {
        if (p.residual) mbar_expect_tx(bar_res, BN * TBM * 4);
        for (int k = 0; k < EPI_SLOTS; ++k, ++it) {
          const int s = it % STAGES;
          mbar_wait(bar_empty(s), ((it / STAGES) & 1) ^ 1);
          if (!p.residual) continue;
          for (int b = k * EPI_PER_SLOT; b < min(BN / TBK, (k + 1) * EPI_PER_SLOT); ++b) {
            const uint32_t dst = epi_box(b);
            if (p.mode == 0) tma_load_2d(dst, &mapR, tc_.n0 + b * TBK, tc_.m0, bar_res);
            else tma_load_4d(dst, &mapR, tc_.n0 + b * TBK, tc_.x0, tc_.y0, tc_.b0, bar_res);
          }
        }
        if (!p.residual) mbar_arrive(bar_res);
      }
    }
    return;
  }

  asm volatile("setmaxnreg.inc.sync.aligned.u32 232;");
  const int wg = (warp >> 2) - 1;
  const int wi = warp & 3, g = lane >> 2, qd = lane & 3;
  const int r0 = wg * 64 + wi * 16 + g;
  const int ea = H16 ? h16_a_exp(p) : 0;
  const float asc = exp2i(ea);
  const int kchunk = (tc_.kb1 - tc_.kb0) <= 2 * CF::KCHUNK ? 2 * CF::KCHUNK : CF::KCHUNK;
  int px[2] = {0, 0}, py[2] = {0, 0}, pb[2] = {0, 0};
  if (p.mode == 1) {
#pragma unroll
    for (int i = 0; i < 2; ++i) {
      const int r = r0 + 8 * i;
      px[i] = tc_.x0 + r % p.bw; py[i] = tc_.y0 + (r / p.bw) % p.bh; pb[i] = tc_.b0 + r / (p.bw * p.bh);
    }
  }

  float acc[NACC], tot[NACC];
#pragma unroll
  for (int j = 0; j < NACC; ++j) { acc[j] = 0.f; tot[j] = 0.f; }

  struct Frag { uint32_t h[KSTEPS][4], l[KSTEPS][4]; };

  auto load_split = [&](int it, Frag& f) {
    const int s = it % STAGES;
    mbar_wait(bar_full(s), (it / STAGES) & 1);
    const uint32_t st = base + s * STAGE_BYTES;
    if (KIND == KIND_SS) {
      const uint32_t sb = st + A_BYTES;
      const int ct = threadIdx.x - 128;
#pragma unroll 4
      for (int i = ct; i < B_PLANE / 16; i += 256) {
        const uint32_t a = sb + (uint32_t)i * 16u;
        uint32_t v[4], h[4], l[4];
        asm volatile("ld.shared.v4.u32 {%0, %1, %2, %3}, [%4];" : "=r"(v[0]), "=r"(v[1]), "=r"(v[2]), "=r"(v[3]) : "r"(a));
#pragma unroll
        for (int c = 0; c < 4; ++c) { h[c] = rn_tf32(v[c]); l[c] = tf32_lo(__uint_as_float(v[c]), h[c]); }
        asm volatile("st.shared.v4.u32 [%0], {%1, %2, %3, %4};" ::"r"(a), "r"(h[0]), "r"(h[1]), "r"(h[2]), "r"(h[3]) : "memory");
        asm volatile("st.shared.v4.u32 [%0], {%1, %2, %3, %4};" ::"r"(a + B_PLANE), "r"(l[0]), "r"(l[1]), "r"(l[2]), "r"(l[3]) : "memory");
      }
      asm volatile("fence.proxy.async.shared::cta;" ::: "memory");
      asm volatile("bar.sync 1, 256;" ::: "memory");
    }
#pragma unroll
    for (int kk = 0; kk < KSTEPS; ++kk) {
      if (H16) {
#pragma unroll
        for (int i = 0; i < 2; ++i) {
          const int r = r0 + 8 * i;
#pragma unroll
          for (int hk = 0; hk < 2; ++hk) {
            const int k = kk * 16 + hk * 8 + 2 * qd;
            float2 x;
            asm volatile("ld.shared.v2.f32 {%0, %1}, [%2];" : "=f"(x.x), "=f"(x.y)
                         : "r"(st + (uint32_t)r * 128u + ((((uint32_t)k >> 2) ^ (uint32_t)(r & 7)) << 4) + (uint32_t)(k & 3) * 4u));
            if (ea != 0) { x.x *= asc; x.y *= asc; }
            const __half2 h = __floats2half2_rn(x.x, x.y);
            f.h[kk][hk * 2 + i] = *reinterpret_cast<const uint32_t*>(&h);
            if (!FAST) {
              const float2 hf = __half22float2(h);
              const __half2 l = __floats2half2_rn(x.x - hf.x, x.y - hf.y);
              f.l[kk][hk * 2 + i] = *reinterpret_cast<const uint32_t*>(&l);
            }
          }
        }
      } else {
#pragma unroll
        for (int i = 0; i < 2; ++i) {
          const int r = r0 + 8 * i;
#pragma unroll
          for (int hk = 0; hk < 2; ++hk) {
            const int k = kk * 8 + hk * 4 + qd;
            float x;
            asm volatile("ld.shared.f32 %0, [%1];" : "=f"(x)
                         : "r"(st + (uint32_t)r * 128u + ((((uint32_t)k >> 2) ^ (uint32_t)(r & 7)) << 4) + (uint32_t)(k & 3) * 4u));
            const uint32_t h = rn_tf32(__float_as_uint(x));
            f.h[kk][hk * 2 + i] = h;
            f.l[kk][hk * 2 + i] = tf32_lo(x, h);
          }
        }
      }
    }
  };

  auto mma = [&](int it, const Frag& f) {
    const uint32_t sb = base + (it % STAGES) * STAGE_BYTES + A_BYTES;
    const uint64_t bhi = H16 ? make_desc_sw64(sb) : make_desc(sb), blo = H16 ? make_desc_sw64(sb + B_PLANE) : make_desc(sb + B_PLANE);
    wgmma_pin(acc);
    wgmma_fence();
#pragma unroll
    for (int kk = 0; kk < KSTEPS; ++kk) {
      const uint64_t adv = (uint64_t)kk * 2u;
      if (H16) {
        if (!FAST) {
          Wgmma<BN>::f16_rs(acc, f.l[kk], bhi + adv);
          Wgmma<BN>::f16_rs(acc, f.h[kk], blo + adv);
        }
        Wgmma<BN>::f16_rs(acc, f.h[kk], bhi + adv);
      } else {
        Wgmma<BN>::tf32_rs(acc, f.l[kk], bhi + adv);
        Wgmma<BN>::tf32_rs(acc, f.h[kk], blo + adv);
        Wgmma<BN>::tf32_rs(acc, f.h[kk], bhi + adv);
      }
    }
    wgmma_commit();
  };

  int kin = 0;
  auto step = [&](int it, const Frag& cur, Frag& nxt) {
    mma(it, cur);
    wgmma_wait1();
    if (it > 0) {
      __syncwarp();
      if (lane == 0) mbar_arrive(bar_empty((it - 1) % STAGES));
    }
    if (it + 1 < nst) load_split(it + 1, nxt);
    if (++kin == kchunk || it == nst - 1) {
      wgmma_wait0();
      wgmma_pin(acc);
#pragma unroll
      for (int j = 0; j < NACC; ++j) { tot[j] += acc[j]; acc[j] = 0.f; }
      kin = 0;
    }
  };

  Frag fa, fb;
  load_split(0, fa);
#pragma unroll 1
  for (int it = 0; it < nst; it += 2) {
    step(it, fa, fb);
    if (it + 1 < nst) step(it + 1, fb, fa);
  }

  const bool fin = p.splits == 1;
  const float alpha = H16 ? p.alpha * exp2i(-ea) * exp2i(-p.b_exp) : p.alpha;
  long long mrow[2];
  bool rok[2];
#pragma unroll
  for (int i = 0; i < 2; ++i) {
    const int r = r0 + 8 * i;
    if (p.mode != 1) {
      mrow[i] = (long long)tc_.m0 + r;
      rok[i] = mrow[i] < p.M;
    } else {
      rok[i] = pb[i] < p.B && px[i] < p.W && py[i] < p.H;
      mrow[i] = ((long long)pb[i] * p.H + py[i]) * p.W + px[i];
    }
  }
  float omax = 0.f;
  const int n0 = tc_.n0, nend = tc_.nend;
  if (!fin) {
    float* const dst = p.ws + (long long)tc_.split * p.M * p.N;
#pragma unroll
    for (int j = 0; j < BN / 8; ++j)
#pragma unroll
      for (int i = 0; i < 2; ++i)
#pragma unroll
        for (int c = 0; c < 2; ++c) {
          const int n = n0 + 8 * j + 2 * qd + c;
          if (rok[i] && n < nend) dst[mrow[i] * p.N + n] = tot[j * 4 + i * 2 + c];
        }
    return;
  }
#pragma unroll
  for (int j = 0; j < BN / 8; ++j)
#pragma unroll
    for (int c = 0; c < 2; ++c) {
      const int n = n0 + 8 * j + 2 * qd + c;
      const float bv = (p.bias && n < nend) ? p.bias[n] : 0.f;
#pragma unroll
      for (int i = 0; i < 2; ++i) {
        float v = alpha * tot[j * 4 + i * 2 + c] + bv;
        if (p.rowvec && rok[i] && n < nend) v += p.rowvec[(mrow[i] / p.rows_per_batch) * p.ld_rowvec + n];
        tot[j * 4 + i * 2 + c] = v;
      }
    }
  if (p.out_nchw) {
#pragma unroll
    for (int i = 0; i < 2; ++i) {
      if (!rok[i]) continue;
      const long long bimg = mrow[i] / p.rows_per_img, rimg = mrow[i] - bimg * p.rows_per_img;
#pragma unroll
      for (int j = 0; j < BN / 8; ++j)
#pragma unroll
        for (int c = 0; c < 2; ++c) {
          const int n = n0 + 8 * j + 2 * qd + c;
          if (n < nend) p.C[(bimg * p.N + n) * p.rows_per_img + rimg] = tot[j * 4 + i * 2 + c];
        }
    }
    return;
  }
  if (p.Ct_hi && n0 >= p.t_col0) {
#pragma unroll
    for (int j = 0; j < BN / 8; ++j)
#pragma unroll
      for (int i = 0; i < 2; ++i)
#pragma unroll
        for (int c = 0; c < 2; ++c) {
          const int n = n0 + 8 * j + 2 * qd + c;
          if (rok[i] && n < nend) {
            const float o = tot[j * 4 + i * 2 + c];
            const uint32_t hi = rn_tf32(__float_as_uint(o));
            const long long at = (long long)(n - p.t_col0) * p.ldt + mrow[i];
            p.Ct_hi[at] = __uint_as_float(hi);
            p.Ct_lo[at] = __uint_as_float(tf32_lo(o, hi));
            omax = fmaxf(omax, fabsf(o));
          }
        }
  } else {
    float* const dst = p.C + tc_.zb * p.sC_b + tc_.zh * p.sC_h;
    float* const dst_lo = p.C_lo ? p.C_lo + tc_.zb * p.sC_b + tc_.zh * p.sC_h : nullptr;
    auto store_tile = [&](auto staged_c) {
      constexpr bool STAGED = decltype(staged_c)::value;
#pragma unroll
      for (int j = 0; j < BN / 8; ++j) {
        if (p.geglu && (j & 4)) continue;
        const int n = n0 + 8 * j + 2 * qd;
        const int nout = p.geglu ? (n >> 6) * 32 + (n & 63) : n;
        const int box = p.geglu ? j >> 3 : j >> 2, cc = 8 * (j & 3) + 2 * qd;
        float cs[2] = {0.f, 0.f}, cq[2] = {0.f, 0.f};
#pragma unroll
        for (int i = 0; i < 2; ++i) {
          float2 o = make_float2(tot[j * 4 + i * 2], tot[j * 4 + i * 2 + 1]);
          if (p.geglu) {
            const float g0 = tot[(j + 4) * 4 + i * 2], g1 = tot[(j + 4) * 4 + i * 2 + 1];
            o.x *= 0.5f * g0 * (1.f + erff(g0 * 0.70710678118654752440f));
            o.y *= 0.5f * g1 * (1.f + erff(g1 * 0.70710678118654752440f));
          }
          if (STAGED) {
            const int r = r0 + 8 * i;
            const uint32_t a = epi_box(box) + (uint32_t)r * 128u + ((((uint32_t)cc >> 2) ^ (uint32_t)(r & 7)) << 4) + (uint32_t)(cc & 3) * 4u;
            if (p.residual) {
              float2 rv;
              asm volatile("ld.shared.v2.f32 {%0, %1}, [%2];" : "=f"(rv.x), "=f"(rv.y) : "r"(a));
              o.x += rv.x;
              o.y += rv.y;
            }
            asm volatile("st.shared.v2.f32 [%0], {%1, %2};" ::"r"(a), "f"(o.x), "f"(o.y) : "memory");
          }
          if (!rok[i] || n >= nend) continue;
          if (!STAGED && p.residual) {
            o.x += p.residual[mrow[i] * p.ldr + n];
            o.y += p.residual[mrow[i] * p.ldr + n + 1];
          }
          if (p.c_stats) { cs[0] += o.x; cq[0] += o.x * o.x; cs[1] += o.y; cq[1] += o.y * o.y; }
          if (!STAGED) {
            float* const d = dst + mrow[i] * p.ldc + nout;
            if (dst_lo) {
              const uint32_t hx = rn_tf32(__float_as_uint(o.x)), hy = rn_tf32(__float_as_uint(o.y));
              *reinterpret_cast<float2*>(dst_lo + mrow[i] * p.ldc + nout) = make_float2(__uint_as_float(tf32_lo(o.x, hx)), __uint_as_float(tf32_lo(o.y, hy)));
              o = make_float2(__uint_as_float(hx), __uint_as_float(hy));
            }
            *reinterpret_cast<float2*>(d) = o;
          }
          omax = fmaxf(omax, fmaxf(fabsf(o.x), fabsf(o.y)));
        }
        if (p.c_stats) {
#pragma unroll
          for (int c = 0; c < 2; ++c) {
#pragma unroll
            for (int o2 = 4; o2 < 32; o2 <<= 1) {
              cs[c] += __shfl_xor_sync(0xffffffffu, cs[c], o2);
              cq[c] += __shfl_xor_sync(0xffffffffu, cq[c], o2);
            }
          }
          const long long mq = __shfl_sync(0xffffffffu, rok[0] ? mrow[0] : -1LL, 0);
          if (g == 0 && mq >= 0 && n < nend) {
            double* sp = p.c_stats + ((mq / p.rows_per_batch) * p.N + n) * 2;
            atomicAdd(sp, (double)cs[0]); atomicAdd(sp + 1, (double)cq[0]);
            atomicAdd(sp + 2, (double)cs[1]); atomicAdd(sp + 3, (double)cq[1]);
          }
        }
      }
    };
    if (!staged) {
      store_tile(std::false_type());
    } else {
      mbar_wait(bar_res, 0);
      store_tile(std::true_type());
      asm volatile("fence.proxy.async.shared::cta;" ::: "memory");
      asm volatile("bar.sync 2, 256;" ::: "memory");
      if (threadIdx.x == 128) {
        const int c0 = p.geglu ? n0 / 2 : n0, ncols = p.geglu ? p.N / 2 : p.N;
        for (int b = 0; b < (p.geglu ? BN / 64 : BN / TBK) && c0 + b * TBK < ncols; ++b) {
          if (p.mode == 0) tma_store_2d(epi_box(b), &mapC, c0 + b * TBK, tc_.m0);
          else tma_store_4d(epi_box(b), &mapC, c0 + b * TBK, tc_.x0, tc_.y0, tc_.b0);
        }
        bulk_commit();
        bulk_wait0();
      }
    }
  }
  if (p.c_amax) {
#pragma unroll
    for (int o = 16; o > 0; o >>= 1) omax = fmaxf(omax, __shfl_xor_sync(0xffffffffu, omax, o));
    if (lane == 0) atomicMax(reinterpret_cast<unsigned int*>(p.c_amax), __float_as_uint(omax));
  }
}

__global__ void splitk_reduce_kernel(const float* ws, int splits, TcParams p, int h16) {
  pdl_trigger();
  pdl_wait();
  const long long total4 = (long long)p.M * p.N / 4;
  const float alpha = h16 ? p.alpha * exp2i(-h16_a_exp(p)) * exp2i(-p.b_exp) : p.alpha;
  float omax = 0.f;
  for (long long i = (long long)blockIdx.x * blockDim.x + threadIdx.x; i < total4; i += (long long)gridDim.x * blockDim.x) {
    const long long e = i * 4;
    const long long m = e / p.N;
    const int n = (int)(e - m * p.N);
    float4 a = *reinterpret_cast<const float4*>(ws + e);
    for (int s = 1; s < splits; ++s) {
      const float4 b = *reinterpret_cast<const float4*>(ws + (long long)s * p.M * p.N + e);
      a.x += b.x; a.y += b.y; a.z += b.z; a.w += b.w;
    }
    a.x *= alpha; a.y *= alpha; a.z *= alpha; a.w *= alpha;
    if (p.bias) { a.x += p.bias[n]; a.y += p.bias[n + 1]; a.z += p.bias[n + 2]; a.w += p.bias[n + 3]; }
    if (p.rowvec) { const float4 t = *reinterpret_cast<const float4*>(p.rowvec + (m / p.rows_per_batch) * p.ld_rowvec + n); a.x += t.x; a.y += t.y; a.z += t.z; a.w += t.w; }
    if (p.residual) { const float4 t = *reinterpret_cast<const float4*>(p.residual + m * p.ldr + n); a.x += t.x; a.y += t.y; a.z += t.z; a.w += t.w; }
    if (p.C_lo) {
      float4 hi, lo;
      hi.x = __uint_as_float(rn_tf32(__float_as_uint(a.x))); lo.x = __uint_as_float(rn_tf32(__float_as_uint(a.x - hi.x)));
      hi.y = __uint_as_float(rn_tf32(__float_as_uint(a.y))); lo.y = __uint_as_float(rn_tf32(__float_as_uint(a.y - hi.y)));
      hi.z = __uint_as_float(rn_tf32(__float_as_uint(a.z))); lo.z = __uint_as_float(rn_tf32(__float_as_uint(a.z - hi.z)));
      hi.w = __uint_as_float(rn_tf32(__float_as_uint(a.w))); lo.w = __uint_as_float(rn_tf32(__float_as_uint(a.w - hi.w)));
      *reinterpret_cast<float4*>(p.C_lo + m * p.ldc + n) = lo;
      a = hi;
    }
    *reinterpret_cast<float4*>(p.C + m * p.ldc + n) = a;
    omax = fmaxf(omax, fmaxf(fmaxf(fabsf(a.x), fabsf(a.y)), fmaxf(fabsf(a.z), fabsf(a.w))));
  }
  if (p.c_amax) {
#pragma unroll
    for (int o = 16; o > 0; o >>= 1) omax = fmaxf(omax, __shfl_xor_sync(0xffffffffu, omax, o));
    if ((threadIdx.x & 31) == 0) atomicMax(reinterpret_cast<unsigned int*>(p.c_amax), __float_as_uint(omax));
  }
}

__global__ void split_planes_kernel(const float* __restrict__ w, float* __restrict__ hi, float* __restrict__ lo, size_t n) {
  for (size_t i = (size_t)blockIdx.x * blockDim.x + threadIdx.x; i < n; i += (size_t)gridDim.x * blockDim.x) {
    const uint32_t b = __float_as_uint(w[i]);
    const uint32_t h = rn_tf32(b);
    hi[i] = __uint_as_float(h);
    lo[i] = __uint_as_float(rn_tf32(__float_as_uint(w[i] - __uint_as_float(h))));
  }
}

__global__ void split_planes_h16_kernel(const float* __restrict__ w, __half* __restrict__ hi, __half* __restrict__ lo, size_t n, float scale) {
  for (size_t i = (size_t)blockIdx.x * blockDim.x + threadIdx.x; i < n; i += (size_t)gridDim.x * blockDim.x) {
    const float x = w[i] * scale;
    const __half h = __float2half_rn(x);
    hi[i] = h;
    lo[i] = __float2half_rn(x - __half2float(h));
  }
}

__global__ void amax_rows_kernel(const float* __restrict__ x, long long rows, int C, long long ld, float* __restrict__ slot) {
  float m = 0.f;
  const long long total = rows * (long long)(C >> 2);
  const int c4n = C >> 2;
  for (long long i = (long long)blockIdx.x * blockDim.x + threadIdx.x; i < total; i += (long long)gridDim.x * blockDim.x) {
    const long long r = i / c4n;
    const int c4 = (int)(i - r * c4n);
    const float4 v = *reinterpret_cast<const float4*>(x + r * ld + 4 * c4);
    m = fmaxf(m, fmaxf(fmaxf(fabsf(v.x), fabsf(v.y)), fmaxf(fabsf(v.z), fabsf(v.w))));
  }
#pragma unroll
  for (int o = 16; o > 0; o >>= 1) m = fmaxf(m, __shfl_xor_sync(0xffffffffu, m, o));
  if ((threadIdx.x & 31) == 0) atomicMax(reinterpret_cast<unsigned int*>(slot), __float_as_uint(m));
}

__global__ void amax_rows_scalar_kernel(const float* __restrict__ x, long long rows, int C, long long ld, float* __restrict__ slot) {
  float m = 0.f;
  const long long total = rows * (long long)C;
  for (long long i = (long long)blockIdx.x * blockDim.x + threadIdx.x; i < total; i += (long long)gridDim.x * blockDim.x) {
    const long long r = i / C;
    m = fmaxf(m, fabsf(x[r * ld + (i - r * C)]));
  }
#pragma unroll
  for (int o = 16; o > 0; o >>= 1) m = fmaxf(m, __shfl_xor_sync(0xffffffffu, m, o));
  if ((threadIdx.x & 31) == 0) atomicMax(reinterpret_cast<unsigned int*>(slot), __float_as_uint(m));
}

template <int KIND, int BN>
void set_smem_attr() {
  CDX_CUDA(cudaFuncSetAttribute(tc_gemm_kernel<KIND, BN>, cudaFuncAttributeMaxDynamicSharedMemorySize, Cfg<KIND, BN>::SMEM_BYTES));
}

void ensure_attr(int device) {
  static bool attr_set[64] = {};
  static std::mutex mtx;
  std::lock_guard<std::mutex> lock(mtx);
  const int d = device & 63;
  if (!attr_set[d]) {
    set_smem_attr<KIND_SS, 128>();
    set_smem_attr<KIND_TS, 128>();
    set_smem_attr<KIND_TS, 64>();
    set_smem_attr<KIND_H16, 128>();
    set_smem_attr<KIND_H16, 64>();
    set_smem_attr<KIND_H16_FAST, 128>();
    set_smem_attr<KIND_H16_FAST, 64>();
    attr_set[d] = true;
  }
}

template <int KIND, int BN>
void launch_gemm(const TcParams& p, const CUtensorMap& mA, const CUtensorMap& mA2, const CUtensorMap& mB, const CUtensorMap& mBlo,
                 const CUtensorMap& mR, const CUtensorMap& mC, cudaStream_t s) {
  launch_ex(tc_gemm_kernel<KIND, BN>, dim3((unsigned)p.total_tiles), dim3(TC_THREADS), Cfg<KIND, BN>::SMEM_BYTES, s, 1, mA, mA2, mB, mBlo, mR, mC, p);
}

}

void split_planes(Engine& e, const float* w, float* hi, float* lo, size_t n, cudaStream_t s) {
  if (e.dry()) return;
  size_t blocks = (n + 255) / 256;
  if (blocks > (size_t)e.num_sms * 16) blocks = (size_t)e.num_sms * 16;
  split_planes_kernel<<<(unsigned)(blocks ? blocks : 1), 256, 0, s>>>(w, hi, lo, n);
  CDX_CUDA(cudaGetLastError());
  e.launches++;
}

void split_planes_h16(Engine& e, const float* w, void* hi, void* lo, size_t n, int exp, cudaStream_t s) {
  if (e.dry()) return;
  size_t blocks = (n + 255) / 256;
  if (blocks > (size_t)e.num_sms * 16) blocks = (size_t)e.num_sms * 16;
  split_planes_h16_kernel<<<(unsigned)(blocks ? blocks : 1), 256, 0, s>>>(w, (__half*)hi, (__half*)lo, n, ldexpf(1.f, exp));
  CDX_CUDA(cudaGetLastError());
  e.launches++;
}

void amax_rows(Engine& e, const float* x, long long rows, int C, long long ld, float* slot, cudaStream_t s) {
  if (e.dry()) return;
  if ((C & 3) || (ld & 3) || !a16(x)) {
    const long long total = rows * (long long)C;
    const int blocks = (int)std::min<long long>((total + 255) / 256, (long long)e.num_sms * 8);
    amax_rows_scalar_kernel<<<blocks > 0 ? blocks : 1, 256, 0, s>>>(x, rows, C, ld, slot);
    CDX_CUDA(cudaGetLastError());
    e.launches++;
    return;
  }
  const long long total = rows * (long long)(C >> 2);
  const int blocks = (int)std::min<long long>((total + 255) / 256, (long long)e.num_sms * 8);
  amax_rows_kernel<<<blocks > 0 ? blocks : 1, 256, 0, s>>>(x, rows, C, ld, slot);
  CDX_CUDA(cudaGetLastError());
  e.launches++;
}

int h16_exp_host(float amax) {
  if (!(amax > 0.f) || !std::isfinite(amax)) return 0;
  int ex;
  frexpf(amax, &ex);
  return std::min(std::max(14 - (ex - 1), -100), 100);
}

bool attention_tc(Engine& e, const float* q, int ldq, const float* k, int ldk, int head_stride, const float* vt, float* out, int ldo, int B,
                  int Nq, int Nk, int heads, int d, float scale, cudaStream_t s) {
  if ((Nk % TBK) || (d & 3) || (ldq & 3) || (ldk & 3) || (head_stride & 3) || (ldo & 3) || Nq < 64) return false;
  if (!a16(q) || !a16(k) || !a16(vt) || !a16(out)) return false;
  Scope sc(e.arena);
  const int ldS = Nk;
  float* S = (float*)e.arena.alloc((size_t)B * heads * Nq * ldS * sizeof(float));
  if (e.dry()) return true;
  ensure_attr(e.device);
  TcParams p;
  {
    memset(&p, 0, sizeof(p));
    p.mode = 2; p.M = Nq; p.N = Nk; p.K = d; p.heads = heads; p.alpha = scale;
    p.C = S; p.ldc = ldS; p.sC_b = (long long)heads * Nq * ldS; p.sC_h = (long long)Nq * ldS;
    p.rows_per_batch = 1;
    const int code[4] = {0, 2, 1, 3};
    for (int i = 0; i < 4; ++i) { p.a_code[i] = code[i]; p.b_code[i] = code[i]; }
    uint64_t da[4] = {(uint64_t)d, (uint64_t)heads, (uint64_t)Nq, (uint64_t)B};
    uint64_t sa[3] = {(uint64_t)head_stride * 4, (uint64_t)ldq * 4, (uint64_t)Nq * ldq * 4};
    uint64_t db[4] = {(uint64_t)d, (uint64_t)heads, (uint64_t)Nk, (uint64_t)B};
    uint64_t sb[3] = {(uint64_t)head_stride * 4, (uint64_t)ldk * 4, (uint64_t)Nk * ldk * 4};
    uint32_t bx[4] = {TBK, 1, TBM, 1};
    const CUtensorMap& mA = get_map(q, 4, da, sa, bx);
    const CUtensorMap& mB = get_map(k, 4, db, sb, bx);
    ProfScope ps(e, s, PROF_BATCHED_TC, 2.0 * Nq * Nk * d * B * heads, 4.0 * B * heads * ((double)Nq * d + (double)Nk * d + (double)Nq * Nk), 1);
    p.splits = 1; p.kb_per_split = cdiv(d, TBK);
    p.tn_w = TBN;
    p.tiles_m = cdiv(Nq, TBM); p.tiles_n = cdiv(Nk, TBN); p.total_tiles = p.tiles_m * p.tiles_n * B * heads;
    launch_gemm<KIND_SS, 128>(p, mA, mA, mB, mB, mA, mA, s);
    CDX_CUDA(cudaGetLastError());
    e.launches++;
  }
  softmax_rows(e, S, (long long)B * heads * Nq, Nk, ldS, s);
  {
    memset(&p, 0, sizeof(p));
    p.mode = 2; p.M = Nq; p.N = d; p.K = Nk; p.heads = heads; p.alpha = 1.f;
    p.C = out; p.ldc = ldo; p.sC_b = (long long)Nq * ldo; p.sC_h = d;
    p.rows_per_batch = 1;
    const int ac[4] = {0, 1, 2, 3};
    const int bc[4] = {0, 3, 1, 4};
    for (int i = 0; i < 4; ++i) { p.a_code[i] = ac[i]; p.b_code[i] = bc[i]; }
    p.b_rowoff_h = d;
    uint64_t da[4] = {(uint64_t)Nk, (uint64_t)Nq, (uint64_t)heads, (uint64_t)B};
    uint64_t sa[3] = {(uint64_t)ldS * 4, (uint64_t)Nq * ldS * 4, (uint64_t)heads * Nq * ldS * 4};
    uint32_t bxa[4] = {TBK, TBM, 1, 1};
    uint64_t db[4] = {(uint64_t)Nk, (uint64_t)B, (uint64_t)heads * d, 1};
    uint64_t sb[3] = {(uint64_t)Nk * 4, (uint64_t)B * Nk * 4, (uint64_t)B * Nk * 4 * heads * d};
    uint32_t bxb[4] = {TBK, 1, TBN, 1};
    const CUtensorMap& mA = get_map(S, 4, da, sa, bxa);
    const CUtensorMap& mB = get_map(vt, 4, db, sb, bxb);
    ProfScope ps(e, s, PROF_BATCHED_TC, 2.0 * Nq * Nk * d * B * heads, 4.0 * B * heads * ((double)Nq * Nk + (double)Nk * d + (double)Nq * d), 1);
    p.splits = 1; p.kb_per_split = cdiv(Nk, TBK);
    p.tn_w = TBN;
    p.tiles_m = cdiv(Nq, TBM); p.tiles_n = cdiv(d, TBN); p.total_tiles = p.tiles_m * p.tiles_n * B * heads;
    launch_gemm<KIND_SS, 128>(p, mA, mA, mB, mB, mA, mA, s);
    CDX_CUDA(cudaGetLastError());
    e.launches++;
  }
  return true;
}

static void conv_ragged_tile(int W, int H, int B, int stride, int* bw_out, int* bh_out, int* bn_out) {
  long long best_tiles = -1, best_halo = 0;
  for (int bw = TBM; bw >= 1; bw >>= 1) {
    for (int bh = TBM / bw; bh >= 1; bh >>= 1) {
      const int bn = TBM / (bw * bh);
      if (bw * stride > 256 || bh * stride > 256) continue;
      const long long tiles = (long long)cdiv(W, bw) * cdiv(H, bh) * cdiv(B, bn);
      const long long halo = (long long)bn * (bw + 2) * (bh + 2);
      if (best_tiles < 0 || tiles < best_tiles || (tiles == best_tiles && halo < best_halo)) {
        best_tiles = tiles; best_halo = halo;
        *bw_out = bw; *bh_out = bh; *bn_out = bn;
      }
    }
  }
}

bool gemm_tc(Engine& e, const GemmArgs& a, cudaStream_t s, int* side_done) {
  if (a.batch * a.heads != 1 || a.b_kn) return false;
  if (a.geglu && ((a.N % TBN) || a.out_nchw || a.Cout_lo || a.residual || a.rowvec || a.mode != 0)) return false;
  if (a.Cout_lo && a.out_nchw) return false;
  if (a.Ct_hi && (a.mode != 0 || !a.Ct_lo || a.out_nchw || a.geglu || a.residual || a.rowvec || (a.t_col0 % TBN) || a.t_col0 >= a.N)) return false;
  if (a.out_nchw && (a.rowvec || a.residual)) return false;
  if (!a.out_nchw && ((a.N & 3) || (a.ldc & 3) || !a16(a.Cout))) return false;
  if (!a16(a.Bw) || (a.ldb & 3)) return false;
  if (a.rowvec && (!a16(a.rowvec) || (a.ld_rowvec & 3))) return false;
  if (a.residual && (!a16(a.residual) || (a.ldr & 3))) return false;
  if (!a16(a.A) || (a.lda & 3)) return false;
  if (a.M < 64) return false;
  if (a.N < 32 && a.M < 2048) return false;

  TcParams p;
  memset(&p, 0, sizeof(p));
  p.M = a.M; p.N = a.N; p.K = a.K;
  p.C = a.Cout; p.ldc = a.ldc;
  p.C_lo = a.out_nchw ? nullptr : a.Cout_lo;
  p.Ct_hi = a.Ct_hi; p.Ct_lo = a.Ct_lo; p.t_col0 = a.t_col0; p.ldt = a.ldt;
  p.bias = a.bias;
  p.rowvec = a.rowvec; p.ld_rowvec = a.ld_rowvec; p.rows_per_batch = a.rows_per_batch > 0 ? a.rows_per_batch : 1;
  p.residual = a.residual; p.ldr = a.ldr;
  p.alpha = a.alpha;
  p.geglu = a.geglu;
  p.out_nchw = a.out_nchw; p.rows_per_img = a.rows_per_img > 0 ? a.rows_per_img : 1;
  p.heads = 1;
  const CUtensorMap *mA, *mA2, *mB, *mBlo;
  if (a.mode == 0) {
    if (a.K & 3) return false;
    if (a.A2) {
      if ((a.C1 % TBK) || !a16(a.A2) || (a.lda2 & 3) || (a.C2 & 3)) return false;
    }
    p.mode = 0; p.C1 = a.C1; p.C2 = a.C2;
    {
      uint64_t d[2] = {(uint64_t)a.C1, (uint64_t)a.M}, st[1] = {(uint64_t)a.lda * 4};
      uint32_t bx[2] = {TBK, TBM};
      mA = &get_map(a.A, 2, d, st, bx);
    }
    if (a.A2) {
      uint64_t d[2] = {(uint64_t)a.C2, (uint64_t)a.M}, st[1] = {(uint64_t)a.lda2 * 4};
      uint32_t bx[2] = {TBK, TBM};
      mA2 = &get_map(a.A2, 2, d, st, bx);
    } else {
      mA2 = mA;
    }
    p.tiles_m = cdiv(a.M, TBM);
  } else {
    if ((a.stride != 1 && a.stride != 2) || a.up != 1) return false;
    if (a.C1 % TBK) return false;
    if (a.Hin != a.Hout * a.stride || a.Win != a.Wout * a.stride) return false;
    const int B = a.M / (a.Hout * a.Wout);
    int bw, bh, bn;
    if (pow2(a.Hout) && pow2(a.Wout)) {
      bw = a.Wout < 16 ? a.Wout : 16;
      bh = a.Hout < TBM / bw ? a.Hout : TBM / bw;
      bn = TBM / (bw * bh);
    } else {
      conv_ragged_tile(a.Wout, a.Hout, B, a.stride, &bw, &bh, &bn);
    }
    if (bn > 256 || bw * a.stride > 256 || bh * a.stride > 256) return false;
    p.mode = 1; p.C1 = a.C1; p.H = a.Hout; p.W = a.Wout; p.B = B;
    p.bw = bw; p.bh = bh; p.bn = bn;
    p.cstride = a.stride; p.cpad = a.pad;
    p.tiles_x = cdiv(a.Wout, bw); p.tiles_y = cdiv(a.Hout, bh);
    uint64_t d[4] = {(uint64_t)a.C1, (uint64_t)a.Win, (uint64_t)a.Hin, (uint64_t)B};
    uint64_t st[3] = {(uint64_t)a.lda * 4, (uint64_t)a.lda * 4 * a.Win, (uint64_t)a.lda * 4 * a.Win * a.Hin};
    uint32_t bx[4] = {TBK, (uint32_t)(bw * a.stride), (uint32_t)(bh * a.stride), (uint32_t)bn};
    uint32_t es[4] = {1, (uint32_t)a.stride, (uint32_t)a.stride, 1};
    mA = &get_map(a.A, 4, d, st, bx, es);
    mA2 = mA;
    p.tiles_m = p.tiles_x * p.tiles_y * cdiv(B, bn);
  }
  const bool ts = a.Bw_hi != nullptr && a.Bw_lo != nullptr && a16(a.Bw_hi) && a16(a.Bw_lo);
  const bool h16 = e.tc_kind >= 1 && a.Bw_h_hi && a.Bw_h_lo && a16(a.Bw_h_hi) && a16(a.Bw_h_lo) && (a.K % TBK) == 0 && (a.ldb % 8) == 0 &&
                   (!a.A2 || (a.C2 % TBK) == 0);
  const int bk = h16 ? 64 : TBK;
  const int num_kb = cdiv(a.K, bk);
  int best_w = TBN, best_s = 1;
  {
    static std::map<std::array<int64_t, 6>, int> plan_cache;
    static std::mutex plan_mutex;
    std::lock_guard<std::mutex> plan_lock(plan_mutex);
    const std::array<int64_t, 6> key = {a.M, p.tiles_m, a.N, num_kb, ((a.geglu || a.Ct_hi) ? 1 : 0) | (a.out_nchw ? 2 : 0) | (h16 ? 4 : 0) | (ts ? 8 : 0), e.num_sms};
    const double kc0 = h16 ? 700.0 : 400.0, kc1 = h16 ? 6.0 : 3.0;
    const int min_kbs = h16 ? 4 : 8;
    auto it = plan_cache.find(key);
    if (it != plan_cache.end()) {
      best_w = it->second >> 8;
      best_s = it->second & 255;
    } else {
      const bool only128 = a.geglu || a.Ct_hi || (!h16 && !ts);
      double best = 1e30;
      for (int w = TBN; w >= 64; w -= 64) {
        if (w == 64 && only128) break;
        const int tn = cdiv(a.N, w);
        double base = 0.0;
        for (int S = 1; S <= 8; ++S) {
          const int kbs = cdiv(num_kb, S);
          const int Sx = cdiv(num_kb, kbs);
          if (S > 1 && (Sx != S || kbs < min_kbs || a.out_nchw || a.geglu || a.Ct_hi || (long long)p.tiles_m * tn >= 4LL * e.num_sms)) continue;
          const long long items = (long long)p.tiles_m * tn * S;
          double cost = (double)cdiv(items, (long long)e.num_sms) * (kbs * (kc0 + kc1 * w) + 3000.0);
          if (S == 1) base = cost;
          else cost += 4000.0 + (2.0 * S + 1.0) * (double)a.M * a.N * 4.0 / 3e12 * 1.8e9;
          if (cost < best - 1e-9 && (S == 1 || cost < 0.9 * base)) { best = cost; best_w = w; best_s = S; }
        }
      }
      plan_cache[key] = (best_w << 8) | best_s;
    }
  }
  p.tn_w = best_w;
  p.tiles_n = cdiv(a.N, best_w);
  const int tiles = p.tiles_m * p.tiles_n;
  p.kb_per_split = cdiv(num_kb, best_s);
  p.splits = cdiv(num_kb, p.kb_per_split);
  p.kb_per_split *= bk / TBK;
  p.total_tiles = tiles * p.splits;
  Scope ws_scope(e.arena);
  if (p.splits > 1) p.ws = (float*)e.arena.alloc((size_t)p.splits * a.M * a.N * sizeof(float));
  if (h16) {
    p.a_amax = a.a_amax;
    p.a2_amax = a.A2 ? a.a2_amax : nullptr;
    if (!p.a_amax) {
      float* slot = e.amax_slot();
      if (a.mode == 1) amax_rows(e, a.A, (long long)(a.M / (a.Hout * a.Wout)) * a.Hin * a.Win, a.C1, a.lda, slot, s);
      else amax_rows(e, a.A, a.M, a.C1, a.lda, slot, s);
      p.a_amax = slot;
    }
    if (a.A2 && !p.a2_amax) {
      float* slot = e.amax_slot();
      amax_rows(e, a.A2, a.M, a.C2, a.lda2, slot, s);
      p.a2_amax = slot;
    }
    p.b_exp = a.b_exp;
  }
  const bool fast = h16 && e.tc_kind == 2;
  p.c_amax = a.out_nchw ? nullptr : a.c_amax;
  const bool quad_ok = a.mode == 1 ? ((p.bw * p.bh) % 32 == 0 && p.tiles_x * p.bw == p.W && p.tiles_y * p.bh == p.H) : (a.rows_per_batch % 32 == 0);
  p.c_stats = (a.c_stats && quad_ok && p.splits == 1 && !a.out_nchw && !a.geglu && !a.Ct_hi && !a.Cout_lo && a.ldc == a.N) ? a.c_stats : nullptr;
  if (side_done)
    *side_done = (p.c_amax ? 1 : 0) | (p.c_stats ? 2 : 0) | (p.splits > 1 ? 4 : 0) |
                 route_plan(fast ? ROUTE_KIND_H16_FAST : h16 ? ROUTE_KIND_H16 : ts ? ROUTE_KIND_TS : ROUTE_KIND_SS, p.tn_w, p.splits);
  if (e.dry()) return true;
  if (h16) {
    uint64_t d[2] = {(uint64_t)a.K, (uint64_t)a.N}, st[1] = {(uint64_t)a.ldb * 2};
    uint32_t bx[2] = {(uint32_t)TBK, (uint32_t)p.tn_w};
    mB = &get_map(a.Bw_h_hi, 2, d, st, bx, nullptr, 2, 64);
    mBlo = &get_map(a.Bw_h_lo, 2, d, st, bx, nullptr, 2, 64);
  } else {
    uint64_t d[2] = {(uint64_t)a.K, (uint64_t)a.N}, st[1] = {(uint64_t)a.ldb * 4};
    uint32_t bx[2] = {TBK, (uint32_t)p.tn_w};
    mB = &get_map(ts ? a.Bw_hi : a.Bw, 2, d, st, bx);
    mBlo = ts ? &get_map(a.Bw_lo, 2, d, st, bx) : mB;
  }
  const CUtensorMap *mR = mA, *mC = mA;
  if (staged_store(p)) {
    auto out_map = [&](const float* ptr, int cols, int ld) -> const CUtensorMap& {
      if (a.mode == 0) {
        uint64_t d[2] = {(uint64_t)cols, (uint64_t)a.M}, st[1] = {(uint64_t)ld * 4};
        uint32_t bx[2] = {TBK, TBM};
        return get_map(ptr, 2, d, st, bx);
      }
      uint64_t d[4] = {(uint64_t)cols, (uint64_t)p.W, (uint64_t)p.H, (uint64_t)p.B};
      uint64_t st[3] = {(uint64_t)ld * 4, (uint64_t)ld * 4 * p.W, (uint64_t)ld * 4 * p.W * p.H};
      uint32_t bx[4] = {TBK, (uint32_t)p.bw, (uint32_t)p.bh, (uint32_t)p.bn};
      return get_map(ptr, 4, d, st, bx);
    };
    mC = &out_map(a.Cout, a.geglu ? a.N / 2 : a.N, a.ldc);
    if (a.residual) mR = &out_map(a.residual, a.N, a.ldr);
  }
  ensure_attr(e.device);
  ProfScope ps(e, s, a.mode == 1 ? PROF_CONV_TC : PROF_DENSE_TC, 2.0 * a.M * a.N * a.K,
               4.0 * ((double)a.M * a.K / (a.mode == 1 ? 9 : 1) + (double)a.N * a.K + (double)a.M * a.N), 1);
  ps.note("M%d N%d K%d w%d tiles%d S%d %s%s%s%s box%dx%dx%d", a.M, a.N, a.K, p.tn_w, tiles, p.splits, h16 ? (fast ? "H16x1" : "H16") : ts ? "TS" : "SS",
          a.Cout_lo ? " planes" : "", a.geglu ? " geglu" : "", a.residual ? " res" : "", p.bw, p.bh, p.bn);
  if (fast && p.tn_w == 128) launch_gemm<KIND_H16_FAST, 128>(p, *mA, *mA2, *mB, *mBlo, *mR, *mC, s);
  else if (fast) launch_gemm<KIND_H16_FAST, 64>(p, *mA, *mA2, *mB, *mBlo, *mR, *mC, s);
  else if (h16 && p.tn_w == 128) launch_gemm<KIND_H16, 128>(p, *mA, *mA2, *mB, *mBlo, *mR, *mC, s);
  else if (h16) launch_gemm<KIND_H16, 64>(p, *mA, *mA2, *mB, *mBlo, *mR, *mC, s);
  else if (ts && p.tn_w == 128) launch_gemm<KIND_TS, 128>(p, *mA, *mA2, *mB, *mBlo, *mR, *mC, s);
  else if (ts) launch_gemm<KIND_TS, 64>(p, *mA, *mA2, *mB, *mBlo, *mR, *mC, s);
  else launch_gemm<KIND_SS, 128>(p, *mA, *mA2, *mB, *mBlo, *mR, *mC, s);
  CDX_CUDA(cudaGetLastError());
  e.launches++;
  if (p.splits > 1) {
    const long long total4 = (long long)a.M * a.N / 4;
    const int blocks = (int)std::min<long long>((total4 + 255) / 256, (long long)e.num_sms * 8);
    launch_ex(splitk_reduce_kernel, dim3((unsigned)blocks), dim3(256), 0, s, 1, p.ws, p.splits, p, h16 ? 1 : 0);
    CDX_CUDA(cudaGetLastError());
    e.launches++;
  }
  return true;
}

}
```

cycle_diffusion_b200/engine.py:

```python
import contextlib
import ctypes as C
import math

import torch

from . import _cabi
from ._cabi import lib, check, UnetConfig, VaeConfig, TextConfig, DdimCoef, PixelCoef
from .attn_control import MutualSelfControl, PnPControl
from .schedule import EditFriendlySchedule
from .semantic import SemanticGuidance


def _ptr(t):
    return C.c_void_p(t.data_ptr()) if t is not None else C.c_void_p(0)


def _f32c(t, device):
    assert t.dtype == torch.float32, f'expected float32, got {t.dtype}'
    if t.device != device:
        t = t.to(device)
    return t.contiguous()


def check_mask(mask, shape, device, what='mask'):
    if not torch.is_tensor(mask) or mask.dtype != torch.float32:
        raise ValueError(f'{what}: expected a float32 tensor, got {getattr(mask, "dtype", type(mask))}')
    if tuple(mask.shape) != tuple(shape):
        raise ValueError(f'{what}: shape {tuple(mask.shape)}, expected {tuple(shape)}')
    if not bool(torch.isfinite(mask).all()) or bool((mask < 0).any()) or bool((mask > 1).any()):
        raise ValueError(f'{what}: values must be finite and within [0, 1]')
    return _f32c(mask, device)


class Engine:

    def __init__(self, device=0):
        if not torch.cuda.is_available():
            raise RuntimeError('cycle_diffusion_b200 needs a CUDA device: the engine has no CPU fallback')
        self.device = torch.device('cuda', device if isinstance(device, int) else torch.device(device).index or 0)
        torch.cuda.set_device(self.device)
        h = C.c_void_p()
        check(lib.cdx_engine_create(self.device.index, C.byref(h)))
        self.h = h
        self.mma_mode = 1

    def close(self):
        if getattr(self, 'h', None):
            lib.cdx_engine_destroy(self.h)
            self.h = None

    def __del__(self):
        try:
            self.close()
        except Exception:
            pass

    @property
    def stream(self):
        return C.c_void_p(torch.cuda.current_stream(self.device).cuda_stream)

    @property
    def launches(self):
        return int(lib.cdx_engine_launch_count(self.h))

    @property
    def workspace_bytes(self):
        return int(lib.cdx_engine_workspace_bytes(self.h))

    def set_mma_mode(self, mode):
        check(lib.cdx_engine_set_mma_mode(self.h, int(mode)))
        self.mma_mode = int(mode)

    PRECISIONS = {'full': None, 'autocast': 5}

    @contextlib.contextmanager
    def precision(self, precision):
        if precision not in self.PRECISIONS:
            raise ValueError(f'precision must be one of {sorted(self.PRECISIONS)}, got {precision!r}')
        mode, prev = self.PRECISIONS[precision], self.mma_mode
        if mode is None:
            yield self
            return
        self.set_mma_mode(mode)
        try:
            yield self
        finally:
            self.set_mma_mode(prev)

    PROF_TAGS = ['conv3x3_ffma', 'dense_ffma', 'batched_ffma', 'conv3x3_tc', 'dense_tc', 'batched_tc', 'groupnorm', 'layernorm',
                 'softmax', 'other']

    def profile(self, enable):
        check(lib.cdx_engine_profile(self.h, int(enable)))

    def profile_read(self):
        out = {}
        for i, name in enumerate(self.PROF_TAGS):
            ms, fl, by, n = C.c_double(), C.c_double(), C.c_double(), C.c_uint64()
            check(lib.cdx_engine_profile_read(self.h, i, C.byref(ms), C.byref(fl), C.byref(by), C.byref(n)))
            if n.value:
                out[name] = dict(ms=ms.value, flops=fl.value, bytes=by.value, launches=int(n.value))
        return out

    def empty(self, *shape):
        return torch.empty(*shape, dtype=torch.float32, device=self.device)

    def affine(self, x, a, b):
        x = _f32c(x, self.device)
        out = torch.empty_like(x)
        check(lib.cdx_affine(self.h, _ptr(x), a, b, _ptr(out), x.numel(), self.stream))
        return out

    def shift_scale(self, x, b, a):
        x = _f32c(x, self.device)
        out = torch.empty_like(x)
        check(lib.cdx_shift_scale(self.h, _ptr(x), b, a, _ptr(out), x.numel(), self.stream))
        return out

    def mask_pool(self, mask, f):
        if mask.dim() != 4 or mask.shape[1] != 1 or mask.shape[2] % f or mask.shape[3] % f:
            raise ValueError(f'mask: expected [B,1,H,W] with H, W multiples of {f}, got {tuple(mask.shape)}')
        mask = check_mask(mask, mask.shape, self.device)
        B, _, H, W = mask.shape
        out = self.empty(B, 1, H // f, W // f)
        check(lib.cdx_mask_pool(self.h, _ptr(mask), _ptr(out), B, H, W, int(f), self.stream))
        return out

    def mask_composite(self, dec, image, mask):
        dec, image = _f32c(dec, self.device), _f32c(image, self.device)
        B, Cc, H, W = dec.shape
        if tuple(image.shape) != tuple(dec.shape):
            raise ValueError(f'image shape {tuple(image.shape)} != decode shape {tuple(dec.shape)}')
        mask = check_mask(mask, (B, 1, H, W), self.device)
        out = torch.empty_like(dec)
        check(lib.cdx_mask_composite(self.h, _ptr(dec), _ptr(image), _ptr(mask), _ptr(out), B, Cc, H, W, self.stream))
        return out

    def edit_map_from_eps(self, e_src, e_tgt, vscale=1.0, maps_per_launch=None):
        e_src, e_tgt = _f32c(e_src, self.device), _f32c(e_tgt, self.device)
        assert e_src.dim() == 5 and e_src.shape == e_tgt.shape, f'{tuple(e_src.shape)} vs {tuple(e_tgt.shape)}'
        B, n, Cc, h, w = e_src.shape
        acc = self.empty(B, h, w)
        check(lib.cdx_edit_map_from_eps(self.h, _ptr(e_src), _ptr(e_tgt), float(vscale), n, int(maps_per_launch or n), _ptr(acc), B, Cc,
                                        h, w, self.stream))
        return acc

    def edit_mask(self, acc, n_maps, ratio=3.0, f=None, channels=4):
        if not ratio > 0:
            raise ValueError(f'mask_thresholding_ratio must be > 0, got {ratio}')
        acc = _f32c(acc, self.device)
        B, h, w = acc.shape
        emap, mask = self.empty(B, 1, h, w), self.empty(B, 1, h, w)
        img = self.empty(B, 1, f * h, f * w) if f else None
        check(lib.cdx_edit_mask(self.h, _ptr(acc), int(n_maps), float(ratio), _ptr(emap), _ptr(mask), _ptr(img), int(f or 1), B,
                                int(channels), h, w, self.stream))
        return emap, mask, img

    def q_sample(self, x0, noise, sqrt_a, sqrt_1ma):
        x0, noise = _f32c(x0, self.device), _f32c(noise, self.device)
        out = torch.empty_like(x0)
        check(lib.cdx_q_sample(self.h, _ptr(x0), _ptr(noise), sqrt_a, sqrt_1ma, _ptr(out), x0.numel(), self.stream))
        return out

    def vae_posterior(self, moments, noise, scale_factor):
        moments = _f32c(moments, self.device)
        B, C2, h, w = moments.shape
        out = self.empty(B, C2 // 2, h, w)
        if noise is not None:
            noise = _f32c(noise, self.device)
            assert noise.shape == out.shape
        check(lib.cdx_vae_posterior(self.h, _ptr(moments), _ptr(noise), scale_factor, _ptr(out), B, C2 // 2, h * w, self.stream))
        return out

    def ddim_posterior_sample(self, x0, xt, noise, coef):
        x0, xt, noise = (_f32c(t, self.device) for t in (x0, xt, noise))
        out = torch.empty_like(x0)
        check(lib.cdx_ddim_posterior_sample(self.h, _ptr(x0), _ptr(xt), _ptr(noise), C.byref(coef), _ptr(out), x0.numel(), self.stream))
        return out

    def ddim_compute_eps(self, xt, xt_next, e_c, e_uc, scale, coef):
        xt, xt_next, e_c = (_f32c(t, self.device) for t in (xt, xt_next, e_c))
        e_uc = _f32c(e_uc, self.device) if e_uc is not None else None
        out = torch.empty_like(xt)
        check(lib.cdx_ddim_compute_eps(self.h, _ptr(xt), _ptr(xt_next), _ptr(e_c), _ptr(e_uc), scale, C.byref(coef), _ptr(out),
                                       xt.numel(), self.stream))
        return out

    def ddim_step_with_eps(self, x, e_c, e_uc, scale, eps, coef):
        x, e_c, eps = (_f32c(t, self.device) for t in (x, e_c, eps))
        e_uc = _f32c(e_uc, self.device) if e_uc is not None else None
        out = torch.empty_like(x)
        check(lib.cdx_ddim_step_with_eps(self.h, _ptr(x), _ptr(e_c), _ptr(e_uc), scale, _ptr(eps), C.byref(coef), _ptr(out),
                                         x.numel(), self.stream))
        return out

    def pixel_posterior_sample(self, x0, xt, noise, coef):
        x0, xt, noise = (_f32c(t, self.device) for t in (x0, xt, noise))
        out = torch.empty_like(x0)
        check(lib.cdx_pixel_posterior_sample(self.h, _ptr(x0), _ptr(xt), _ptr(noise), C.byref(coef), _ptr(out), x0.numel(), self.stream))
        return out

    def pixel_compute_eps(self, xt, xt_next, et, coef):
        xt, xt_next, et = (_f32c(t, self.device) for t in (xt, xt_next, et))
        B = xt.shape[0]
        out = torch.empty_like(xt)
        check(lib.cdx_pixel_compute_eps(self.h, _ptr(xt), _ptr(xt_next), _ptr(et), C.byref(coef), _ptr(out), B, xt[0].numel(),
                                        et[0].numel(), self.stream))
        return out

    def pixel_step_with_eps(self, xt, et, eps, coef):
        xt, et = _f32c(xt, self.device), _f32c(et, self.device)
        eps = _f32c(eps, self.device) if eps is not None else None
        B = xt.shape[0]
        out = torch.empty_like(xt)
        check(lib.cdx_pixel_step_with_eps(self.h, _ptr(xt), _ptr(et), _ptr(eps), C.byref(coef), _ptr(out), B, xt[0].numel(),
                                          et[0].numel(), self.stream))
        return out

    def op_conv3x3(self, x_nhwc, w_oihw, bias, stride=1, pad_lo=1, upsample=1):
        x, w = _f32c(x_nhwc, self.device), _f32c(w_oihw, self.device)
        bias = _f32c(bias, self.device) if bias is not None else None
        B, H, W, Cin = x.shape
        Cout = w.shape[0]
        Hl, Wl = H * upsample, W * upsample
        Ho, Wo = (Hl, Wl) if stride == 1 else (Hl // 2, Wl // 2)
        y = self.empty(B, Ho, Wo, Cout)
        check(lib.cdx_op_conv3x3(self.h, _ptr(x), _ptr(w), _ptr(bias), _ptr(y), B, H, W, Cin, Cout, stride, pad_lo, upsample, self.stream))
        return y

    def op_linear(self, x, w, bias):
        x, w = _f32c(x, self.device), _f32c(w, self.device)
        bias = _f32c(bias, self.device) if bias is not None else None
        M, K = x.shape
        N = w.shape[0]
        y = self.empty(M, N)
        check(lib.cdx_op_linear(self.h, _ptr(x), _ptr(w), _ptr(bias), _ptr(y), M, K, N, self.stream))
        return y

    def clip_preprocess(self, img, size=224):
        x = _f32c(img, self.device)
        B, Cc, R, R2 = x.shape
        assert Cc == 3 and R == R2, 'square RGB batches (the reference feeds R x R sampler outputs)'
        out = self.empty(B, 3, size, size)
        check(lib.cdx_clip_preprocess(self.h, _ptr(x), B, R, size, _ptr(out), self.stream))
        return out

    def dclip_scores(self, img_f, orig_f, enc_f, dec_f):
        fs = [_f32c(t, self.device) for t in (img_f, orig_f, enc_f, dec_f)]
        B, D = fs[0].shape
        clip, dclip = self.empty(B), self.empty(B)
        check(lib.cdx_dclip_scores(self.h, *[_ptr(t) for t in fs], B, D, _ptr(clip), _ptr(dclip), self.stream))
        return clip, dclip

    def image_metrics(self, a, b):
        a, b = _f32c(a, self.device), _f32c(b, self.device)
        B, Cc, H, W = a.shape
        assert Cc == 3 and a.shape == b.shape
        out = self.empty(B, 3)
        check(lib.cdx_image_metrics(self.h, _ptr(a), _ptr(b), B, H, W, _ptr(out), self.stream))
        return out

    def ensemble_select(self, B, n_candidates, H, W):
        return EnsembleSelection(self, B, n_candidates, H, W)

    def op_groupnorm(self, x_nhwc, gamma, beta, eps, silu):
        x, gamma, beta = (_f32c(t, self.device) for t in (x_nhwc, gamma, beta))
        B, H, W, Cc = x.shape
        y = torch.empty_like(x)
        check(lib.cdx_op_groupnorm(self.h, _ptr(x), _ptr(gamma), _ptr(beta), eps, int(silu), _ptr(y), B, H * W, Cc, self.stream))
        return y

    def op_layernorm(self, x, gamma, beta):
        x, gamma, beta = (_f32c(t, self.device) for t in (x, gamma, beta))
        M, Cc = x.shape
        y = torch.empty_like(x)
        check(lib.cdx_op_layernorm(self.h, _ptr(x), _ptr(gamma), _ptr(beta), _ptr(y), M, Cc, self.stream))
        return y

    def _gn_operands(self, x1, x2, gamma, beta, scale, shift):
        x1, gamma, beta = (_f32c(t, self.device) for t in (x1, gamma, beta))
        B, H, W, C1 = x1.shape
        x2 = _f32c(x2, self.device) if x2 is not None else None
        C2 = x2.shape[3] if x2 is not None else 0
        assert (scale is None) == (shift is None)
        ld_ss = 0
        if scale is not None:
            for t in (scale, shift):
                assert t.dtype == torch.float32 and t.device == self.device and tuple(t.shape) == (B, C1 + C2) and t.stride(1) == 1
            assert scale.stride(0) == shift.stride(0), 'scale and shift share one row stride'
            ld_ss = scale.stride(0)
        return x1, x2, gamma, beta, B, H, W, C1, C2, ld_ss

    def op_groupnorm_ex(self, x1, x2, gamma, beta, eps, silu, scale=None, shift=None):
        x1, x2, gamma, beta, B, H, W, C1, C2, ld_ss = self._gn_operands(x1, x2, gamma, beta, scale, shift)
        y = self.empty(B, H, W, C1 + C2)
        amax = torch.zeros(1, dtype=torch.float32, device=self.device)
        ab = self.empty(B, C1 + C2, 2)
        check(lib.cdx_op_groupnorm_ex(self.h, _ptr(x1), C1, _ptr(x2), C2, _ptr(gamma), _ptr(beta), eps, int(silu), _ptr(scale), _ptr(shift),
                                      ld_ss, _ptr(y), _ptr(amax), _ptr(ab), B, H * W, self.stream))
        return y, amax, ab

    def op_groupnorm_rows(self, x1, x2, gamma, beta, eps, silu, src_rows, scale=None, shift=None):
        x1, x2, gamma, beta, B, H, W, C1, C2, ld_ss = self._gn_operands(x1, x2, gamma, beta, scale, shift)
        rows = [int(r) for r in src_rows]
        assert len(rows) == B, f'src_rows: {len(rows)} entries for {B} images'
        y, y_rows = self.empty(B, H, W, C1 + C2), self.empty(B, H, W, C1 + C2)
        amax, amax_rows = (torch.zeros(1, dtype=torch.float32, device=self.device) for _ in range(2))
        check(lib.cdx_op_groupnorm_rows(self.h, _ptr(x1), C1, _ptr(x2), C2, _ptr(gamma), _ptr(beta), eps, int(silu), _ptr(scale), _ptr(shift),
                                        ld_ss, (C.c_int * B)(*rows), _ptr(y), _ptr(amax), _ptr(y_rows), _ptr(amax_rows), B, H * W, self.stream))
        return y, amax, y_rows, amax_rows

    def op_layernorm_ex(self, x, gamma, beta):
        x, gamma, beta = (_f32c(t, self.device) for t in (x, gamma, beta))
        M, Cc = x.shape
        y = torch.empty_like(x)
        amax = torch.zeros(1, dtype=torch.float32, device=self.device)
        check(lib.cdx_op_layernorm_ex(self.h, _ptr(x), _ptr(gamma), _ptr(beta), _ptr(y), _ptr(amax), M, Cc, self.stream))
        return y, amax

    def op_softmax_rows(self, x, causal_nq=0):
        assert x.dtype == torch.float32 and x.device == self.device and x.is_contiguous()
        rows, L = x.shape
        check(lib.cdx_op_softmax_rows(self.h, _ptr(x), rows, L, L, int(causal_nq), self.stream))
        return x

    PRODUCE_PATHS = ('ffma', 'fused', 'tc_standalone', 'splitk')

    def op_produce_norm(self, x, w, bias, gamma, beta, eps, conv=False):
        x, w, gamma, beta = (_f32c(t, self.device) for t in (x, w, gamma, beta))
        bias = _f32c(bias, self.device) if bias is not None else None
        if conv:
            B, H, W, Cin = x.shape
        else:
            B, HW, Cin = x.shape
            H, W = HW, 1
        Cout = w.shape[0]
        y = self.empty(B * H * W, Cout)
        yn = self.empty(B * H * W, Cout)
        amax = torch.zeros(1, dtype=torch.float32, device=self.device)
        stats = torch.empty(B, Cout, 2, dtype=torch.float64, device=self.device)
        path = C.c_int(-1)
        check(lib.cdx_op_produce_norm(self.h, _ptr(x), _ptr(w), _ptr(bias), int(bool(conv)), B, H, W, Cin, Cout, _ptr(gamma), _ptr(beta),
                                      eps, _ptr(y), _ptr(amax), _ptr(stats), _ptr(yn), C.byref(path), self.stream))
        return y, amax, stats, yn, self.PRODUCE_PATHS[path.value]

    GEMM_POINTERS = ('A', 'A2', 'w', 'bias', 'rowvec', 'residual', 'C', 'C_lo', 'Ct_hi', 'Ct_lo', 'a_amax', 'a2_amax', 'c_amax', 'c_stats')
    GEMM_KINDS = ('ss', 'ts', 'h16', 'h16_fast')

    def op_gemm(self, **fields):
        d = _cabi.GemmDesc(alpha=1.0, stride=1, pad=1, batch=1, heads=1, rows_per_batch=1, up=1)
        for name, v in fields.items():
            if name in self.GEMM_POINTERS:
                if v is not None:
                    want = torch.float64 if name == 'c_stats' else torch.float32
                    assert torch.is_tensor(v) and v.dtype == want and v.device == self.device, f'op_gemm: {name} must be a {want} tensor on {self.device}'
                setattr(d, name, v.data_ptr() if v is not None else None)
            else:
                assert hasattr(d, name), f'op_gemm: no field {name}'
                setattr(d, name, v)
        plan = C.c_int(0)
        check(lib.cdx_op_gemm(self.h, C.byref(d), C.byref(plan), self.stream))
        return self.gemm_plan(plan.value)

    @classmethod
    def gemm_plan(cls, p):
        return dict(kind=cls.GEMM_KINDS[(p >> 4) & 3] if p & 8 else 'ffma', width=(p >> 8) & 255, splits=(p >> 16) & 255,
                    amax_fused=bool(p & 1), stats_fused=bool(p & 2))

    def op_latent_chains(self, stage, chains, chw, n_src, K, rows, c=None, cnext=None, **fields):
        sg_rows = fields.pop('sg_rows', None)
        m = len(sg_rows) // max(n_src * K, 1) if sg_rows else 0
        hw = fields.get('hw', 0)
        need = dict(x0=n_src * chw, noise0=n_src * chw, xt=n_src * chw, xn=n_src * chw, noise_next=n_src * chw, xn2=n_src * chw,
                    eout=rows * chw, xin=rows * chw, yt=n_src * K * chw, y_out=n_src * K * chw,
# ... 591 lines not shown
```

include/cdx.h:

```cpp
#ifndef CDX_H_
#define CDX_H_

#include <stddef.h>
#include <stdint.h>

#ifdef __cplusplus
extern "C" {
#endif

#define CDX_ABI_VERSION 2

#define CDX_OK 0
#define CDX_E_INVALID (-1)
#define CDX_E_CUDA (-2)
#define CDX_E_STATE (-3)
#define CDX_E_NOMEM (-4)

typedef struct cdx_engine cdx_engine;
typedef struct cdx_net cdx_net;

int cdx_abi_version(void);
const char* cdx_last_error(void);
int cdx_engine_create(int device, cdx_engine** out);
void cdx_engine_destroy(cdx_engine* e);
size_t cdx_engine_workspace_bytes(const cdx_engine* e);
uint64_t cdx_engine_launch_count(const cdx_engine* e);
#define CDX_PROF_NTAGS 10
int cdx_engine_profile(cdx_engine* e, int enable);
int cdx_engine_profile_read(cdx_engine* e, int tag, double* ms, double* flops, double* bytes, uint64_t* launches);
int cdx_engine_set_mma_mode(cdx_engine* e, int mode);

#define CDX_UNET_OPENAI 1
#define CDX_UNET_IDDPM 2
#define CDX_UNET_DDPM 3

typedef struct cdx_unet_config {
  int kind;
  int in_channels, out_channels, model_channels, num_res_blocks;
  int n_mult;
  int channel_mult[8];
  int n_attn;
  int attention_ds[8];
  int num_heads;
  int num_head_channels;
  int context_dim;
} cdx_unet_config;

typedef struct cdx_vae_config {
  int ch;
  int n_mult;
  int ch_mult[8];
  int num_res_blocks;
  int in_channels, out_ch, z_channels, embed_dim;
  int vq, n_embed;
} cdx_vae_config;

typedef struct cdx_text_config {
  int vocab_size, width, layers, heads, max_len, mlp_width;
  int kind;
  int dim_head;
  int proj_dim, patch, image_size;
} cdx_text_config;
#define CDX_TEXT_CLIP 1
#define CDX_TEXT_XTRANSFORMER 2
#define CDX_CLIP_VISION 3
#define CDX_TEXT_OPENCLIP 4

int cdx_unet_create(cdx_engine* e, const cdx_unet_config* cfg, cdx_net** out);
int cdx_vae_create(cdx_engine* e, const cdx_vae_config* cfg, cdx_net** out);
int cdx_text_create(cdx_engine* e, const cdx_text_config* cfg, cdx_net** out);
void cdx_net_destroy(cdx_net* n);

int cdx_net_num_params(const cdx_net* n);
const char* cdx_net_param_name(const cdx_net* n, int i);
int cdx_net_param_shape(const cdx_net* n, int i, int64_t dims[4]);
int cdx_net_load_param(cdx_net* n, const char* name, const float* data, int data_on_device,
                       const int64_t* dims, int rank);
int cdx_net_finalize(cdx_net* n);
int cdx_net_weight_blob(cdx_net* n, void** dev_ptr, size_t* bytes);
int cdx_net_adopt_blob(cdx_net* n);
int cdx_unet_set_time_freqs(cdx_net* n, const float* freqs_host, int half);

#define CDX_PRED_EPS 0
#define CDX_PRED_V 1
int cdx_unet_set_prediction(cdx_net* unet, int prediction, const float* sa_v_host, const float* s1_v_host, int T);

int cdx_unet_forward(cdx_net* n, const float* x_dev, const float* t_dev, const float* ctx_dev,
                     int ctx_len, float* out_dev, int B, int H, int W, void* stream);

int cdx_vae_encode(cdx_net* n, const float* img_dev, float* moments_dev, int B, int R, void* stream);
int cdx_vae_encode_hw(cdx_net* n, const float* img_dev, float* moments_dev, int B, int H, int W, void* stream);
int cdx_text_encode(cdx_net* n, const int* ids_dev, int B, int L, float* out_dev, void* stream);
int cdx_vae_decode(cdx_net* n, const float* z_dev, float* img_dev, int B, int h, void* stream);
int cdx_vae_decode_hw(cdx_net* n, const float* z_dev, float* img_dev, int B, int h, int w, void* stream);


int cdx_affine(cdx_engine* e, const float* x, float a, float b, float* out, size_t n, void* stream);
int cdx_shift_scale(cdx_engine* e, const float* x, float b, float a, float* out, size_t n, void* stream);
int cdx_q_sample(cdx_engine* e, const float* x0, const float* noise, float sqrt_a, float sqrt_1ma,
                 float* out, size_t n, void* stream);
int cdx_vae_posterior(cdx_engine* e, const float* moments, const float* noise, float scale_factor,
                      float* out, int B, int C, int hw, void* stream);

typedef struct cdx_ddim_coef {
  float sqrt_at;
  float sqrt_1m_at;
  float sqrt_1m_at_tab;
  float sqrt_aprev;
  float dir_coef;
  float sigma;
} cdx_ddim_coef;

int cdx_ddim_posterior_sample(cdx_engine* e, const float* x0, const float* xt, const float* noise,
                              const cdx_ddim_coef* c, float* xt_next, size_t n, void* stream);
int cdx_ddim_compute_eps(cdx_engine* e, const float* xt, const float* xt_next, const float* e_c,
                         const float* e_uc, float scale, const cdx_ddim_coef* c, float* eps_out,
                         size_t n, void* stream);
int cdx_ddim_step_with_eps(cdx_engine* e, const float* x, const float* e_c, const float* e_uc,
                           float scale, const float* eps, const cdx_ddim_coef* c, float* x_prev,
                           size_t n, void* stream);

typedef struct cdx_pixel_coef {
  int ddpm;
  float sqrt_at;
  float sqrt_1m_at;
  float sqrt_at_next;
  float c1, c2;
  float w0, wt, post_std;
  float weight, inv_sqrt_1m_bt, std_model, mask;
} cdx_pixel_coef;

int cdx_pixel_posterior_sample(cdx_engine* e, const float* x0, const float* xt, const float* noise,
                               const cdx_pixel_coef* c, float* xt_next, size_t n, void* stream);
int cdx_pixel_compute_eps(cdx_engine* e, const float* xt, const float* xt_next, const float* et,
                          const cdx_pixel_coef* c, float* eps_out, int B, int chw, int net_chw,
                          void* stream);
int cdx_pixel_step_with_eps(cdx_engine* e, const float* xt, const float* et, const float* eps,
                            const cdx_pixel_coef* c, float* xt_next, int B, int chw, int net_chw,
                            void* stream);

int cdx_latent_encode(cdx_net* unet, const float* x0, const float* c, const float* uc, int ctx_len,
                      float scale, const cdx_ddim_coef* coef, const float* t_host, int n_steps,
                      int n_rec, const float* noise, float sqrt_a_T, float sqrt_1ma_T, float* z_out,
                      int B, int C, int h, int w, void* stream);
int cdx_latent_decode(cdx_net* unet, const float* z, int n_eps, const float* c, const float* uc,
                      int ctx_len, float scale, const cdx_ddim_coef* coef, const float* t_host,
                      int n_steps, const float* extra_noise, float* x_out, int B, int C, int h, int w,
                      void* stream);
int cdx_cycle_lockstep(cdx_net* unet, const float* x0, const float* c_src, const float* c_tgt, const float* uc,
                       int ctx_len, float src_scale, float tgt_scale, const cdx_ddim_coef* coef,
                       const float* t_host, int n_steps, const float* noise, float sqrt_a_T,
                       float sqrt_1ma_T, float* x_out, float* z_out, int B, int C, int h, int w,
                       void* stream);
int cdx_cycle_lockstep_masked(cdx_net* unet, const float* x0, const float* c_src, const float* c_tgt, const float* uc,
                              int ctx_len, float src_scale, float tgt_scale, const cdx_ddim_coef* coef,
                              const float* t_host, int n_steps, const float* noise, float sqrt_a_T,
                              float sqrt_1ma_T, float* x_out, float* z_out, int B, int C, int h, int w,
                              void* stream, const float* mask);
typedef struct cdx_attn_control {
  int cross_steps, self_steps, self_max_tokens;
  const float* token_map;
} cdx_attn_control;
int cdx_cycle_lockstep_ctl(cdx_net* unet, const float* x0, const float* c_src, const float* c_tgt, const float* uc,
                           int ctx_len, float src_scale, float tgt_scale, const cdx_ddim_coef* coef,
                           const float* t_host, int n_steps, const float* noise, float sqrt_a_T,
                           float sqrt_1ma_T, float* x_out, float* z_out, int B, int C, int h, int w,
                           void* stream, const float* mask, const cdx_attn_control* ctl);
int cdx_cycle_lockstep_refine(cdx_net* unet, const float* x0, const float* c_src, const float* c_tgt, const float* uc,
                              int ctx_len, float src_scale, float tgt_scale, const cdx_ddim_coef* coef,
                              const float* t_host, int n_steps, const float* noise, float sqrt_a_T,
                              float sqrt_1ma_T, float* x_out, float* z_out, int B, int C, int h, int w,
                              void* stream, const float* mask, const cdx_attn_control* ctl, const float* own_weight);
int cdx_cycle_lockstep_mutual(cdx_net* unet, const float* x0, const float* c_src, const float* c_tgt, const float* uc,
                              int ctx_len, float src_scale, float tgt_scale, const cdx_ddim_coef* coef,
                              const float* t_host, int n_steps, const float* noise, float sqrt_a_T,
                              float sqrt_1ma_T, float* x_out, float* z_out, int B, int C, int h, int w,
                              void* stream, const float* mask, int start_step, int start_layer);
int cdx_cycle_lockstep_pnp(cdx_net* unet, const float* x0, const float* c_src, const float* c_tgt, const float* uc,
                           int ctx_len, float src_scale, float tgt_scale, const cdx_ddim_coef* coef,
                           const float* t_host, int n_steps, const float* noise, float sqrt_a_T,
                           float sqrt_1ma_T, float* x_out, float* z_out, int B, int C, int h, int w,
                           void* stream, const float* mask, int feature_steps, int attention_steps,
                           int attention_start_layer, const int* feature_blocks, int n_feature_blocks);
#define CDX_SEMANTIC_MAX 8
typedef struct cdx_semantic_guidance {
  int m;
  float scale[CDX_SEMANTIC_MAX];
  float threshold[CDX_SEMANTIC_MAX];
  int cooldown[CDX_SEMANTIC_MAX];
  int warmup;
  float momentum_scale, beta, beta1;
} cdx_semantic_guidance;
int cdx_cycle_lockstep_semantic(cdx_net* unet, const float* x0, const float* c_src, const float* c_tgt, const float* uc,
                                int ctx_len, float src_scale, float tgt_scale, const cdx_ddim_coef* coef,
                                const float* t_host, int n_steps, const float* noise, float sqrt_a_T,
                                float sqrt_1ma_T, float* x_out, float* z_out, int B, int C, int h, int w,
                                void* stream, const float* mask, const float* c_edit, const cdx_semantic_guidance* sg);
typedef struct cdx_semantic_attn_mask {
  int intersect;
  int n_tokens[CDX_SEMANTIC_MAX];
} cdx_semantic_attn_mask;
int cdx_cycle_lockstep_semantic_attn(cdx_net* unet, const float* x0, const float* c_src, const float* c_tgt, const float* uc,
                                     int ctx_len, float src_scale, float tgt_scale, const cdx_ddim_coef* coef,
                                     const float* t_host, int n_steps, const float* noise, float sqrt_a_T,
                                     float sqrt_1ma_T, float* x_out, float* z_out, int B, int C, int h, int w,
                                     void* stream, const float* mask, const float* c_edit, const cdx_semantic_guidance* sg,
                                     const cdx_semantic_attn_mask* am);
#define CDX_SAMPLER_DDIM_POSTERIOR 0
#define CDX_SAMPLER_DDIM_DRAWS 1
#define CDX_SAMPLER_DPMSOLVER_DRAWS 2
typedef struct cdx_dpm_coef {
  float a;
  float b;
  float c;
  float n;
  int order;
} cdx_dpm_coef;
typedef struct cdx_sampler {
  int kind;
  const cdx_dpm_coef* dpm;
  const float* qa; const float* q1;
} cdx_sampler;
typedef struct cdx_mutual_control { int start_step, start_layer; } cdx_mutual_control;
typedef struct cdx_pnp_control {
  int feature_steps, attention_steps, attention_start_layer;
  const int* feature_blocks; int n_feature_blocks;
} cdx_pnp_control;
int cdx_cycle_lockstep_sampler(cdx_net* unet, const float* x0, const float* c_src, const float* c_tgt, const float* uc,
                               int ctx_len, float src_scale, float tgt_scale, const cdx_ddim_coef* coef,
                               const float* t_host, int n_steps, const float* noise, float sqrt_a_T,
                               float sqrt_1ma_T, float* x_out, float* z_out, int B, int C, int h, int w,
                               void* stream, const cdx_sampler* sampler, const float* mask, const cdx_attn_control* ctl,
                               const float* own_weight, const cdx_mutual_control* mutual, const cdx_pnp_control* pnp,
                               const float* c_edit, const cdx_semantic_guidance* sg, const cdx_semantic_attn_mask* am);
int cdx_mask_pool(cdx_engine* e, const float* mask, float* out, int B, int H, int W, int f, void* stream);
int cdx_mask_composite(cdx_engine* e, const float* dec, const float* image, const float* mask, float* out, int B, int C, int H,
                       int W, void* stream);
int cdx_edit_map(cdx_net* unet, const float* x0, const float* c_src, const float* c_tgt, int ctx_len, float t, float sqrt_a,
                 float sqrt_1ma, const float* noise, int n_maps, int rows_per_call, float* acc_out, int B, int C, int h,
                 int w, void* stream);
int cdx_edit_map_from_eps(cdx_engine* e, const float* e_src, const float* e_tgt, float vscale, int n_maps,
                          int maps_per_launch, float* acc_out, int B, int C, int h, int w, void* stream);
int cdx_edit_mask(cdx_engine* e, const float* acc, int n_maps, float ratio, float* map_out, float* mask_out,
                  float* mask_img_out, int f, int B, int C, int h, int w, void* stream);
int cdx_latent_loop_ens(cdx_net* unet, int mode, const float* x0, const float* c_src, const float* c_tgt, const float* uc,
                        int ctx_len, const float* src_scales, const float* tgt_scales, const cdx_ddim_coef* coef,
                        const float* t_host, int n_steps, int n_rec, const float* noise, float sqrt_a_T,
                        float sqrt_1ma_T, const float* z_in, int n_eps, const float* extra_noise, float* z_out,
                        float* x_out, int B, int C, int h, int w, void* stream);
int cdx_clip_preprocess(cdx_engine* e, const float* img, int B, int R, int size, float* out, void* stream);
int cdx_clip_image_features(cdx_net* vision, const float* pixels, int B, float* out, void* stream);
int cdx_text_features(cdx_net* text, const int* ids_dev, int B, int L, float* out, void* stream);
int cdx_dclip_scores(cdx_engine* e, const float* img_f, const float* orig_f, const float* enc_f, const float* dec_f, int B, int D,
                     float* clip_out, float* dclip_out, void* stream);
int cdx_image_metrics(cdx_engine* e, const float* a, const float* b, int B, int H, int W, float* out, void* stream);
int cdx_pixel_encode(cdx_net* unet, const float* x0, const cdx_pixel_coef* coef, const float* t_host,
                     int n_rec, const float* noise, float sqrt_a_T, float sqrt_1ma_T, float* z_out,
                     int B, int C, int R, void* stream);
int cdx_pixel_decode(cdx_net* unet, const float* z, int n_eps, const cdx_pixel_coef* coef,
                     const float* t_host, int n_steps, const float* last_noise, float* x_out, int B,
                     int C, int R, void* stream);

int cdx_pixel_cycle_lockstep(cdx_net* src, cdx_net* tgt, const float* x0, const cdx_pixel_coef* coef, const float* t_host,
                             int i0, int i1, const float* noise, float sqrt_a_T, float sqrt_1ma_T, float* state, int B,
                             int C, int R, void* stream);
int cdx_latent_cycle_pair(cdx_net* src, cdx_net* tgt, const float* x0, const cdx_ddim_coef* coef, const float* t_host,
                          int n_steps, int n_rec, const float* noise, float sqrt_a_T, float sqrt_1ma_T,
                          const float* extra_noise, float* x_out, int B, int C, int h, int w, void* stream);

int cdx_latent_cycle_fan(cdx_net* unet, int n_src, int K, const float* x0, const float* c_src, const float* c_tgt,
                         const float* uc, int ctx_len, const float* src_scales_host, const float* tgt_scales_host,
                         const cdx_ddim_coef* coef, const float* t_host, int n_steps, const float* noise, float sqrt_a_T,
                         float sqrt_1ma_T, float* x_out, float* z_out, int C, int h, int w, void* stream);
int cdx_latent_cycle_fan_masked(cdx_net* unet, int n_src, int K, const float* x0, const float* c_src, const float* c_tgt,
                                const float* uc, int ctx_len, const float* src_scales_host, const float* tgt_scales_host,
                                const cdx_ddim_coef* coef, const float* t_host, int n_steps, const float* noise, float sqrt_a_T,
                                float sqrt_1ma_T, float* x_out, float* z_out, int C, int h, int w, void* stream,
                                const float* mask);
int cdx_ensemble_select(cdx_engine* e, int n, const float* scores, const int64_t* cand_idx, const int* sample_idx,
                        const float* images, float* best_score, int64_t* best_idx, float* best_img, float* score_mat, int B,
                        int n_total, int H, int W, void* stream);

int cdx_op_conv3x3(cdx_engine* e, const float* x_nhwc, const float* w_oihw, const float* bias,
                   float* y_nhwc, int B, int H, int W, int Cin, int Cout, int stride, int pad_lo,
                   int upsample, void* stream);
int cdx_op_linear(cdx_engine* e, const float* x, const float* w, const float* bias, float* y, int M,
                  int K, int N, void* stream);
int cdx_op_groupnorm(cdx_engine* e, const float* x_nhwc, const float* gamma, const float* beta,
                     float eps, int silu, float* y_nhwc, int B, int HW, int C, void* stream);
int cdx_op_layernorm(cdx_engine* e, const float* x, const float* gamma, const float* beta, float* y,
                     int M, int C, void* stream);
int cdx_op_attention(cdx_engine* e, const float* q, const float* k, const float* v, float* out, int B,
                     int Nq, int Nk, int heads, int d, float scale, void* stream);
int cdx_op_attention_rows(cdx_engine* e, const float* q, const float* k, const float* v, float* out, int B,
                          int Nq, int Nk, int heads, int d, float scale, const int* qk_rows, void* stream);
int cdx_op_attention_kv_rows(cdx_engine* e, const float* q, const float* k, const float* v, float* out, int B,
                             int Nq, int Nk, int heads, int d, float scale, const int* kv_rows, void* stream);
int cdx_op_attention_accum(cdx_engine* e, const float* q, const float* k, const float* v, float* out, int B,
                           int Nq, int Nk, int heads, int d, float scale, const int* acc_rows, int n_acc, void* stream);
typedef struct cdx_attention_net_desc {
  int kind, causal;
  const float* qkv;
  const float* q; const float* kv; const float* k; const float* v;
  int B, N, L, ctx_lp, heads, d;
  float scale;
  const int* qk_rows; const int* kv_rows; const int* acc_rows; int n_acc;
  float slot, q_slot;
  float* out;
  const int* probe_rows; const int* probe_spans; int n_probe;
  float* probe_map;
} cdx_attention_net_desc;
int cdx_op_attention_net(cdx_engine* e, const cdx_attention_net_desc* desc, int* plan_out, void* stream);
int cdx_op_nchw_to_nhwc(cdx_engine* e, const float* x, float* y, int B, int C, int HW, void* stream);
int cdx_op_nhwc_to_nchw(cdx_engine* e, const float* x, float* y, int B, int C, int HW, void* stream);
int cdx_op_groupnorm_ex(cdx_engine* e, const float* x1, int C1, const float* x2, int C2, const float* gamma, const float* beta,
                        float eps, int silu, const float* scale, const float* shift, int ld_ss, float* y, float* amax_out,
                        float* ab_out, int B, int HW, void* stream);
int cdx_op_groupnorm_rows(cdx_engine* e, const float* x1, int C1, const float* x2, int C2, const float* gamma, const float* beta,
                          float eps, int silu, const float* scale, const float* shift, int ld_ss, const int* src_rows, float* y,
                          float* amax_out, float* y_rows, float* amax_rows_out, int B, int HW, void* stream);
int cdx_op_layernorm_ex(cdx_engine* e, const float* x, const float* gamma, const float* beta, float* y, float* amax_out, int M,
                        int C, void* stream);
int cdx_op_softmax_rows(cdx_engine* e, float* x, int64_t rows, int L, int ld, int causal_nq, void* stream);
int cdx_op_produce_norm(cdx_engine* e, const float* x, const float* w, const float* bias, int conv, int B, int H, int W, int Cin,
                        int Cout, const float* gamma, const float* beta, float eps, float* y, float* amax_out, double* stats_out,
                        float* yn, int* path_out, void* stream);

typedef struct cdx_gemm_desc {
  int mode, M, N, K;
  const float* A; int lda; int C1;
  const float* A2; int lda2; int C2;
  int Hin, Win, Hout, Wout, stride, pad;
  const float* w; int ldb; int b_kn;
// ... 62 lines not shown
```

Baseline: 0.8092.

## Add persistent-CTA TC GEMM with dedicated epilogue buffer and overlapped stores

Adds a persistent variant of the H16 tensor-core GEMM. A grid of at most one CTA per SM loops over tiles, and the producer warp keeps streaming TMA loads across tile boundaries. A dedicated epilogue buffer plus a store warp lets one tile's output store and residual load overlap with the next tile's mainloop. The tile planner's cost model is changed so that per-launch overhead counts once rather than per wave. In exchange, the extra shared memory for the epilogue buffer reduces pipeline stages, and the change adds a lot of new synchronisation complexity. It is on by default for eligible dense H16 GEMMs.

```diff
diff --git a/cycle_diffusion_b200/_cabi.py b/cycle_diffusion_b200/_cabi.py
--- a/cycle_diffusion_b200/_cabi.py
+++ b/cycle_diffusion_b200/_cabi.py
@@ -139,6 +139,7 @@
     'cdx_engine_workspace_bytes': (_S, [_P]),
     'cdx_engine_launch_count': (C.c_uint64, [_P]),
     'cdx_engine_set_mma_mode': (_I, [_P, _I]),
+    'cdx_engine_set_persist': (_I, [_P, _I, _I]),
     'cdx_engine_profile': (_I, [_P, _I]),
     'cdx_engine_profile_read': (_I, [_P, _I, C.POINTER(C.c_double), C.POINTER(C.c_double), C.POINTER(C.c_double), C.POINTER(C.c_uint64)]),
     'cdx_unet_create': (_I, [_P, C.POINTER(UnetConfig), C.POINTER(_P)]),
diff --git a/cycle_diffusion_b200/csrc/cabi.cu b/cycle_diffusion_b200/csrc/cabi.cu
--- a/cycle_diffusion_b200/csrc/cabi.cu
+++ b/cycle_diffusion_b200/csrc/cabi.cu
@@ -546,6 +546,8 @@
       throw Error(CDX_E_CUDA, "libcdx is built for sm_90a (H100) only; device " + std::to_string(device) + " is sm_" +
                                   std::to_string(prop.major) + std::to_string(prop.minor));
     eng->e.num_sms = prop.multiProcessorCount;
+    const char* persist = getenv("CDX_PERSIST");
+    eng->e.persist = persist == nullptr || atoi(persist) != 0;
     *out = eng;
   });
 }
@@ -570,6 +572,14 @@
     e->e.flash_attn = mode != 2 && mode != 0;
     e->e.tc_kind = mode == 3 ? 0 : mode >= 4 ? 2 : 1;
     e->e.attn_one = mode == 5;
+  });
+}
+
+int cdx_engine_set_persist(cdx_engine* e, int enable, int max_ctas) {
+  return guard([&] {
+    CDX_CHECK(e != nullptr && max_ctas >= 0, "set_persist: bad arguments");
+    e->e.persist = enable != 0;
+    e->e.persist_grid = max_ctas;
   });
 }
 
diff --git a/cycle_diffusion_b200/csrc/common.cuh b/cycle_diffusion_b200/csrc/common.cuh
--- a/cycle_diffusion_b200/csrc/common.cuh
+++ b/cycle_diffusion_b200/csrc/common.cuh
@@ -66,6 +66,8 @@
   int mma_mode = 1;
   int tc_kind = 1;
   bool attn_one = false;
+  bool persist = true;
+  int persist_grid = 0;
   float* amax_pool = nullptr;
   int amax_cap = 1 << 15, amax_used = 0, amax_high = 0;
   float* amax_slot();
diff --git a/cycle_diffusion_b200/csrc/kernels_tc.cu b/cycle_diffusion_b200/csrc/kernels_tc.cu
--- a/cycle_diffusion_b200/csrc/kernels_tc.cu
+++ b/cycle_diffusion_b200/csrc/kernels_tc.cu
@@ -26,7 +26,7 @@
 
 enum { KIND_SS = 0, KIND_TS = 1, KIND_H16 = 2, KIND_H16_FAST = 3 };
 
-template <int KIND, int BN>
+template <int KIND, int BN, bool PERSIST = false>
 struct Cfg {
   static constexpr bool H16 = KIND == KIND_H16 || KIND == KIND_H16_FAST;
   static constexpr int BK = TBK;
@@ -36,13 +36,16 @@
   static constexpr int B_ROW = H16 ? 64 : 128;
   static constexpr int B_PLANE = BN * B_ROW;
   static constexpr int STAGE_BYTES = A_BYTES + 2 * B_PLANE;
-  static constexpr int STAGES = (SMEM_MAX - BAR_BYTES - ALIGN_SLACK) / STAGE_BYTES;
-  static constexpr int SMEM_BYTES = STAGES * STAGE_BYTES + BAR_BYTES + ALIGN_SLACK;
   static constexpr int EPI_BOX = TBM * TBK * 4;
+  static constexpr int EPI_BYTES = PERSIST ? BN / TBK * EPI_BOX : 0;
+  static constexpr int STAGES = (SMEM_MAX - BAR_BYTES - ALIGN_SLACK - EPI_BYTES) / STAGE_BYTES;
+  static constexpr int SMEM_BYTES = STAGES * STAGE_BYTES + EPI_BYTES + BAR_BYTES + ALIGN_SLACK;
   static constexpr int EPI_PER_SLOT = STAGE_BYTES / EPI_BOX;
   static constexpr int EPI_SLOTS = (BN / TBK + EPI_PER_SLOT - 1) / EPI_PER_SLOT;
-  static_assert(STAGES >= 2 + EPI_SLOTS, "the epilogue's slots never include the last stages' slots");
-  static_assert(STAGES >= 3 && (2 * STAGES + 1) * 8 <= BAR_BYTES, "barrier area holds a full and an empty barrier per stage and bar_res");
+  static_assert(PERSIST || STAGES >= 2 + EPI_SLOTS, "the epilogue's slots never include the last stages' slots");
+  static_assert(!PERSIST || (H16 && STAGES == (BN == 128 ? 5 : 8)), "persistent ring: 5 stages at BN 128, 8 at BN 64 beside the epilogue buffer");
+  static_assert(EPI_BYTES % 1024 == 0, "the barriers after the epilogue buffer stay aligned");
+  static_assert(STAGES >= 3 && (2 * STAGES + 2) * 8 <= BAR_BYTES, "barrier area holds a full and an empty barrier per stage, bar_res and bar_out");
   static_assert(STAGE_BYTES % 1024 == 0 && B_PLANE % 1024 == 0, "stage and plane bases stay 1024-byte aligned (swizzle atoms)");
   static_assert(SMEM_BYTES <= SMEM_MAX, "smem overflow");
 };
@@ -123,30 +126,48 @@
 
 __device__ __forceinline__ uint32_t tf32_lo(float x, uint32_t hi) { return rn_tf32(__float_as_uint(x - __uint_as_float(hi))); }
 
-template <int KIND, int BN>
+#ifdef CDX_GEMM_TIMELINE
+constexpr int TL_SLOTS = 8;
+__device__ unsigned long long* g_gemm_timeline = nullptr;
+__device__ __forceinline__ void tl_stamp(int k) {
+  unsigned long long t;
+  asm volatile("mov.u64 %0, %%globaltimer;" : "=l"(t) :: "memory");
+  if (g_gemm_timeline) g_gemm_timeline[(size_t)blockIdx.x * TL_SLOTS + k] = t;
+}
+#define TL_STAMP(k) tl_stamp(k)
+#else
+#define TL_STAMP(k) ((void)0)
+#endif
+
+template <int KIND, int BN, bool PERSIST = false>
 __global__ void __launch_bounds__(TC_THREADS, 1)
 tc_gemm_kernel(const __grid_constant__ CUtensorMap mapA, const __grid_constant__ CUtensorMap mapA2,
                const __grid_constant__ CUtensorMap mapB, const __grid_constant__ CUtensorMap mapBlo,
                const __grid_constant__ CUtensorMap mapR, const __grid_constant__ CUtensorMap mapC, const TcParams p) {
-  using CF = Cfg<KIND, BN>;
+  using CF = Cfg<KIND, BN, PERSIST>;
   constexpr bool H16 = CF::H16, FAST = KIND == KIND_H16_FAST;
   constexpr int BK = CF::BK, KSTEPS = CF::KSTEPS, A_BYTES = CF::A_BYTES, B_PLANE = CF::B_PLANE, STAGE_BYTES = CF::STAGE_BYTES;
   constexpr int STAGES = CF::STAGES, EPI_BOX = CF::EPI_BOX, EPI_PER_SLOT = CF::EPI_PER_SLOT, EPI_SLOTS = CF::EPI_SLOTS;
   constexpr int NACC = BN / 2;
+  if (threadIdx.x == 0) TL_STAMP(0);
   pdl_trigger();
   extern __shared__ uint8_t smem_raw[];
   const uint32_t base = (smem_u32(smem_raw) + 1023u) & ~1023u;
-  const uint32_t bars = base + STAGES * STAGE_BYTES;
+  const uint32_t epi = base + STAGES * STAGE_BYTES;
+  const uint32_t bars = epi + CF::EPI_BYTES;
   auto bar_full = [&](int s) { return bars + 8u * s; };
   auto bar_empty = [&](int s) { return bars + 8u * (STAGES + s); };
   const uint32_t bar_res = bars + 16u * STAGES;
+  const uint32_t bar_out = bar_res + 8u;
 
   const int warp = threadIdx.x >> 5, lane = threadIdx.x & 31;
   const int num_kb = (p.K + BK - 1) / BK;
-  const TileCoord tc_ = tile_coord(p, blockIdx.x, num_kb);
-  const int nst = tc_.kb1 - tc_.kb0;
-  const bool staged = staged_store(p);
-  auto epi_box = [&](int k) { return base + ((nst + k / EPI_PER_SLOT) % STAGES) * STAGE_BYTES + (k % EPI_PER_SLOT) * EPI_BOX; };
+  TileCoord tc_ = tile_coord(p, blockIdx.x, num_kb);
+  int nst = tc_.kb1 - tc_.kb0;
+  const bool staged = PERSIST || staged_store(p);
+  auto epi_box = [&](int k) {
+    return PERSIST ? epi + k * EPI_BOX : base + ((nst + k / EPI_PER_SLOT) % STAGES) * STAGE_BYTES + (k % EPI_PER_SLOT) * EPI_BOX;
+  };
 
   if (threadIdx.x == 0) {
     for (int s = 0; s < STAGES; ++s) {
@@ -154,10 +175,65 @@
       mbar_init(bar_empty(s), 8);
     }
     mbar_init(bar_res, 1);
+    if (PERSIST) mbar_init(bar_out, 1);
     asm volatile("fence.mbarrier_init.release.cluster;" ::: "memory");
   }
   __syncthreads();
   pdl_wait();
+  if (threadIdx.x == 0) TL_STAMP(1);
+
+  if (PERSIST && warp < 4) {
+    asm volatile("setmaxnreg.dec.sync.aligned.u32 40;");
+    if (threadIdx.x == 0) {
+      int it = 0;
+      for (int t = blockIdx.x; t < p.total_tiles; t += gridDim.x) {
+        const TileCoord c = tile_coord(p, t, num_kb);
+        for (int kb = c.kb0; kb < c.kb1; ++kb, ++it) {
+          const int s = it % STAGES;
+          mbar_wait(bar_empty(s), ((it / STAGES) & 1) ^ 1);
+          const uint32_t st = base + s * STAGE_BYTES;
+          const int k0 = kb * BK;
+          mbar_expect_tx(bar_full(s), TILE_BYTES + 2 * B_PLANE);
+          if (k0 < p.C1) tma_load_2d(st, &mapA, k0, c.m0, bar_full(s));
+          else tma_load_2d(st, &mapA2, k0 - p.C1, c.m0, bar_full(s));
+          tma_load_2d(st + A_BYTES, &mapB, k0, c.n0, bar_full(s));
+          tma_load_2d(st + A_BYTES + B_PLANE, &mapBlo, k0, c.n0, bar_full(s));
+        }
+      }
+    } else if (threadIdx.x == 32) {
+      const int c0_div = p.geglu ? 2 : 1, ncols = p.geglu ? p.N / 2 : p.N, nbox = p.geglu ? BN / 64 : BN / TBK;
+      auto store = [&](const TileCoord& c) {
+        const int c0 = c.n0 / c0_div;
+        for (int b = 0; b < nbox && c0 + b * TBK < ncols; ++b) tma_store_2d(epi_box(b), &mapC, c0 + b * TBK, c.m0);
+        bulk_commit();
+      };
+      int j = 0;
+      TileCoord prev;
+      for (int t = blockIdx.x; t < p.total_tiles; t += gridDim.x, ++j) {
+        const TileCoord c = tile_coord(p, t, num_kb);
+        if (j > 0) {
+          mbar_wait(bar_out, (j - 1) & 1);
+          store(prev);
+          bulk_wait_read0();
+        }
+        if (p.residual) {
+          mbar_expect_tx(bar_res, BN * TBM * 4);
+          for (int b = 0; b < BN / TBK; ++b) tma_load_2d(epi_box(b), &mapR, c.n0 + b * TBK, c.m0, bar_res);
+        } else {
+          mbar_arrive(bar_res);
+        }
+        prev = c;
+      }
+      if (j > 0) {
+        mbar_wait(bar_out, (j - 1) & 1);
+        store(prev);
+        TL_STAMP(5);
+        bulk_wait0();
+        TL_STAMP(6);
+      }
+    }
+    return;
+  }
 
   if (warp < 4) {
     asm volatile("setmaxnreg.dec.sync.aligned.u32 40;");
@@ -220,295 +296,319 @@
   const int r0 = wg * 64 + wi * 16 + g;
   const int ea = H16 ? h16_a_exp(p) : 0;
   const float asc = exp2i(ea);
-  const int kchunk = (tc_.kb1 - tc_.kb0) <= 2 * CF::KCHUNK ? 2 * CF::KCHUNK : CF::KCHUNK;
-  int px[2] = {0, 0}, py[2] = {0, 0}, pb[2] = {0, 0};
-  if (p.mode == 1) {
+  float omax_cta = 0.f;
+  int g0 = 0;
+#pragma unroll 1
+  for (int t = blockIdx.x, item = 0;;) {
+    const int kchunk = (tc_.kb1 - tc_.kb0) <= 2 * CF::KCHUNK ? 2 * CF::KCHUNK : CF::KCHUNK;
+    int px[2] = {0, 0}, py[2] = {0, 0}, pb[2] = {0, 0};
+    if (p.mode == 1) {
+#pragma unroll
+      for (int i = 0; i < 2; ++i) {
+        const int r = r0 + 8 * i;
+        px[i] = tc_.x0 + r % p.bw; py[i] = tc_.y0 + (r / p.bw) % p.bh; pb[i] = tc_.b0 + r / (p.bw * p.bh);
+      }
+    }
+
+    float acc[NACC], tot[NACC];
+#pragma unroll
+    for (int j = 0; j < NACC; ++j) { acc[j] = 0.f; tot[j] = 0.f; }
+
+    struct Frag { uint32_t h[KSTEPS][4], l[KSTEPS][4]; };
+
+    auto load_split = [&](int it, Frag& f) {
+      const int s = (g0 + it) % STAGES;
+      mbar_wait(bar_full(s), ((g0 + it) / STAGES) & 1);
+      const uint32_t st = base + s * STAGE_BYTES;
+      if (KIND == KIND_SS) {
+        const uint32_t sb = st + A_BYTES;
+        const int ct = threadIdx.x - 128;
+#pragma unroll 4
+        for (int i = ct; i < B_PLANE / 16; i += 256) {
+          const uint32_t a = sb + (uint32_t)i * 16u;
+          uint32_t v[4], h[4], l[4];
+          asm volatile("ld.shared.v4.u32 {%0, %1, %2, %3}, [%4];" : "=r"(v[0]), "=r"(v[1]), "=r"(v[2]), "=r"(v[3]) : "r"(a));
+#pragma unroll
+          for (int c = 0; c < 4; ++c) { h[c] = rn_tf32(v[c]); l[c] = tf32_lo(__uint_as_float(v[c]), h[c]); }
+          asm volatile("st.shared.v4.u32 [%0], {%1, %2, %3, %4};" ::"r"(a), "r"(h[0]), "r"(h[1]), "r"(h[2]), "r"(h[3]) : "memory");
+          asm volatile("st.shared.v4.u32 [%0], {%1, %2, %3, %4};" ::"r"(a + B_PLANE), "r"(l[0]), "r"(l[1]), "r"(l[2]), "r"(l[3]) : "memory");
+        }
+        asm volatile("fence.proxy.async.shared::cta;" ::: "memory");
+        asm volatile("bar.sync 1, 256;" ::: "memory");
+      }
+#pragma unroll
+      for (int kk = 0; kk < KSTEPS; ++kk) {
+        if (H16) {
+#pragma unroll
+          for (int i = 0; i < 2; ++i) {
+            const int r = r0 + 8 * i;
+#pragma unroll
+            for (int hk = 0; hk < 2; ++hk) {
+              const int k = kk * 16 + hk * 8 + 2 * qd;
+              float2 x;
+              asm volatile("ld.shared.v2.f32 {%0, %1}, [%2];" : "=f"(x.x), "=f"(x.y)
+                           : "r"(st + (uint32_t)r * 128u + ((((uint32_t)k >> 2) ^ (uint32_t)(r & 7)) << 4) + (uint32_t)(k & 3) * 4u));
+              if (ea != 0) { x.x *= asc; x.y *= asc; }
+              const __half2 h = __floats2half2_rn(x.x, x.y);
+              f.h[kk][hk * 2 + i] = *reinterpret_cast<const uint32_t*>(&h);
+              if (!FAST) {
+                const float2 hf = __half22float2(h);
+                const __half2 l = __floats2half2_rn(x.x - hf.x, x.y - hf.y);
+                f.l[kk][hk * 2 + i] = *reinterpret_cast<const uint32_t*>(&l);
+              }
+            }
+          }
+        } else {
+#pragma unroll
+          for (int i = 0; i < 2; ++i) {
+            const int r = r0 + 8 * i;
+#pragma unroll
+            for (int hk = 0; hk < 2; ++hk) {
+              const int k = kk * 8 + hk * 4 + qd;
+              float x;
+              asm volatile("ld.shared.f32 %0, [%1];" : "=f"(x)
+                           : "r"(st + (uint32_t)r * 128u + ((((uint32_t)k >> 2) ^ (uint32_t)(r & 7)) << 4) + (uint32_t)(k & 3) * 4u));
+              const uint32_t h = rn_tf32(__float_as_uint(x));
+              f.h[kk][hk * 2 + i] = h;
+              f.l[kk][hk * 2 + i] = tf32_lo(x, h);
+            }
+          }
+        }
+      }
+    };
+
+    auto mma = [&](int it, const Frag& f) {
+      const uint32_t sb = base + ((g0 + it) % STAGES) * STAGE_BYTES + A_BYTES;
+      const uint64_t bhi = H16 ? make_desc_sw64(sb) : make_desc(sb), blo = H16 ? make_desc_sw64(sb + B_PLANE) : make_desc(sb + B_PLANE);
+      wgmma_pin(acc);
+      wgmma_fence();
+#pragma unroll
+      for (int kk = 0; kk < KSTEPS; ++kk) {
+        const uint64_t adv = (uint64_t)kk * 2u;
+        if (H16) {
+          if (!FAST) {
+            Wgmma<BN>::f16_rs(acc, f.l[kk], bhi + adv);
+            Wgmma<BN>::f16_rs(acc, f.h[kk], blo + adv);
+          }
+          Wgmma<BN>::f16_rs(acc, f.h[kk], bhi + adv);
+        } else {
+          Wgmma<BN>::tf32_rs(acc, f.l[kk], bhi + adv);
+          Wgmma<BN>::tf32_rs(acc, f.h[kk], blo + adv);
+          Wgmma<BN>::tf32_rs(acc, f.h[kk], bhi + adv);
+        }
+      }
+      wgmma_commit();
+    };
+
+    int kin = 0;
+    auto step = [&](int it, const Frag& cur, Frag& nxt) {
+      mma(it, cur);
+      wgmma_wait1();
+      if (it > 0) {
+        __syncwarp();
+        if (lane == 0) mbar_arrive(bar_empty((g0 + it - 1) % STAGES));
+      }
+      if (it + 1 < nst) load_split(it + 1, nxt);
+      if (++kin == kchunk || it == nst - 1) {
+        wgmma_wait0();
+        wgmma_pin(acc);
+#pragma unroll
+        for (int j = 0; j < NACC; ++j) { tot[j] += acc[j]; acc[j] = 0.f; }
+        kin = 0;
+      }
+    };
+
+    Frag fa, fb;
+    load_split(0, fa);
+    if (threadIdx.x == 128 && item == 0) TL_STAMP(2);
+#pragma unroll 1
+    for (int it = 0; it < nst; it += 2) {
+      step(it, fa, fb);
+      if (it + 1 < nst) step(it + 1, fb, fa);
+    }
+    if (PERSIST) {
+      __syncwarp();
+      if (lane == 0) mbar_arrive(bar_empty((g0 + nst - 1) % STAGES));
+    }
+    if (threadIdx.x == 128) TL_STAMP(3);
+
+    const bool fin = PERSIST || p.splits == 1;
+    const float alpha = H16 ? p.alpha * exp2i(-ea) * exp2i(-p.b_exp) : p.alpha;
+    long long mrow[2];
+    bool rok[2];
 #pragma unroll
     for (int i = 0; i < 2; ++i) {
       const int r = r0 + 8 * i;
-      px[i] = tc_.x0 + r % p.bw; py[i] = tc_.y0 + (r / p.bw) % p.bh; pb[i] = tc_.b0 + r / (p.bw * p.bh);
-    }
-  }
-
-  float acc[NACC], tot[NACC];
-#pragma unroll
-  for (int j = 0; j < NACC; ++j) { acc[j] = 0.f; tot[j] = 0.f; }
-
-  struct Frag { uint32_t h[KSTEPS][4], l[KSTEPS][4]; };
-
-  auto load_split = [&](int it, Frag& f) {
-    const int s = it % STAGES;
-    mbar_wait(bar_full(s), (it / STAGES) & 1);
-    const uint32_t st = base + s * STAGE_BYTES;
-    if (KIND == KIND_SS) {
-      const uint32_t sb = st + A_BYTES;
-      const int ct = threadIdx.x - 128;
-#pragma unroll 4
-      for (int i = ct; i < B_PLANE / 16; i += 256) {
-        const uint32_t a = sb + (uint32_t)i * 16u;
-        uint32_t v[4], h[4], l[4];
-        asm volatile("ld.shared.v4.u32 {%0, %1, %2, %3}, [%4];" : "=r"(v[0]), "=r"(v[1]), "=r"(v[2]), "=r"(v[3]) : "r"(a));
-#pragma unroll
-        for (int c = 0; c < 4; ++c) { h[c] = rn_tf32(v[c]); l[c] = tf32_lo(__uint_as_float(v[c]), h[c]); }
-        asm volatile("st.shared.v4.u32 [%0], {%1, %2, %3, %4};" ::"r"(a), "r"(h[0]), "r"(h[1]), "r"(h[2]), "r"(h[3]) : "memory");
-        asm volatile("st.shared.v4.u32 [%0], {%1, %2, %3, %4};" ::"r"(a + B_PLANE), "r"(l[0]), "r"(l[1]), "r"(l[2]), "r"(l[3]) : "memory");
-      }
-      asm volatile("fence.proxy.async.shared::cta;" ::: "memory");
-      asm volatile("bar.sync 1, 256;" ::: "memory");
-    }
-#pragma unroll
-    for (int kk = 0; kk < KSTEPS; ++kk) {
-      if (H16) {
+      if (p.mode != 1) {
+        mrow[i] = (long long)tc_.m0 + r;
+        rok[i] = mrow[i] < p.M;
+      } else {
+        rok[i] = pb[i] < p.B && px[i] < p.W && py[i] < p.H;
+        mrow[i] = ((long long)pb[i] * p.H + py[i]) * p.W + px[i];
+      }
+    }
+    float omax = 0.f;
+    const int n0 = tc_.n0, nend = tc_.nend;
+    if (!fin) {
+      float* const dst = p.ws + (long long)tc_.split * p.M * p.N;
+#pragma unroll
+      for (int j = 0; j < BN / 8; ++j)
+#pragma unroll
+        for (int i = 0; i < 2; ++i)
+#pragma unroll
+          for (int c = 0; c < 2; ++c) {
+            const int n = n0 + 8 * j + 2 * qd + c;
+            if (rok[i] && n < nend) dst[mrow[i] * p.N + n] = tot[j * 4 + i * 2 + c];
+          }
+      return;
+    }
+#pragma unroll
+    for (int j = 0; j < BN / 8; ++j)
+#pragma unroll
+      for (int c = 0; c < 2; ++c) {
+        const int n = n0 + 8 * j + 2 * qd + c;
+        const float bv = (p.bias && n < nend) ? p.bias[n] : 0.f;
 #pragma unroll
         for (int i = 0; i < 2; ++i) {
-          const int r = r0 + 8 * i;
-#pragma unroll
-          for (int hk = 0; hk < 2; ++hk) {
-            const int k = kk * 16 + hk * 8 + 2 * qd;
-            float2 x;
-            asm volatile("ld.shared.v2.f32 {%0, %1}, [%2];" : "=f"(x.x), "=f"(x.y)
-                         : "r"(st + (uint32_t)r * 128u + ((((uint32_t)k >> 2) ^ (uint32_t)(r & 7)) << 4) + (uint32_t)(k & 3) * 4u));
-            if (ea != 0) { x.x *= asc; x.y *= asc; }
-            const __half2 h = __floats2half2_rn(x.x, x.y);
-            f.h[kk][hk * 2 + i] = *reinterpret_cast<const uint32_t*>(&h);
-            if (!FAST) {
-              const float2 hf = __half22float2(h);
-              const __half2 l = __floats2half2_rn(x.x - hf.x, x.y - hf.y);
-              f.l[kk][hk * 2 + i] = *reinterpret_cast<const uint32_t*>(&l);
+          float v = alpha * tot[j * 4 + i * 2 + c] + bv;
+          if (p.rowvec && rok[i] && n < nend) v += p.rowvec[(mrow[i] / p.rows_per_batch) * p.ld_rowvec + n];
+          tot[j * 4 + i * 2 + c] = v;
+        }
+      }
+    if (!PERSIST && p.out_nchw) {
+#pragma unroll
+      for (int i = 0; i < 2; ++i) {
+        if (!rok[i]) continue;
+        const long long bimg = mrow[i] / p.rows_per_img, rimg = mrow[i] - bimg * p.rows_per_img;
+#pragma unroll
+        for (int j = 0; j < BN / 8; ++j)
+#pragma unroll
+          for (int c = 0; c < 2; ++c) {
+            const int n = n0 + 8 * j + 2 * qd + c;
+            if (n < nend) p.C[(bimg * p.N + n) * p.rows_per_img + rimg] = tot[j * 4 + i * 2 + c];
+          }
+      }
+      return;
+    }
+    if (!PERSIST && p.Ct_hi && n0 >= p.t_col0) {
+#pragma unroll
+      for (int j = 0; j < BN / 8; ++j)
+#pragma unroll
+        for (int i = 0; i < 2; ++i)
+#pragma unroll
+          for (int c = 0; c < 2; ++c) {
+            const int n = n0 + 8 * j + 2 * qd + c;
+            if (rok[i] && n < nend) {
+              const float o = tot[j * 4 + i * 2 + c];
+              const uint32_t hi = rn_tf32(__float_as_uint(o));
+              const long long at = (long long)(n - p.t_col0) * p.ldt + mrow[i];
+              p.Ct_hi[at] = __uint_as_float(hi);
+              p.Ct_lo[at] = __uint_as_float(tf32_lo(o, hi));
+              omax = fmaxf(omax, fabsf(o));
             }
           }
-        }
-      } else {
-#pragma unroll
-        for (int i = 0; i < 2; ++i) {
-          const int r = r0 + 8 * i;
-#pragma unroll
-          for (int hk = 0; hk < 2; ++hk) {
-            const int k = kk * 8 + hk * 4 + qd;
-            float x;
-            asm volatile("ld.shared.f32 %0, [%1];" : "=f"(x)
-                         : "r"(st + (uint32_t)r * 128u + ((((uint32_t)k >> 2) ^ (uint32_t)(r & 7)) << 4) + (uint32_t)(k & 3) * 4u));
-            const uint32_t h = rn_tf32(__float_as_uint(x));
-            f.h[kk][hk * 2 + i] = h;
-            f.l[kk][hk * 2 + i] = tf32_lo(x, h);
+    } else {
+      float* const dst = p.C + tc_.zb * p.sC_b + tc_.zh * p.sC_h;
+      float* const dst_lo = p.C_lo ? p.C_lo + tc_.zb * p.sC_b + tc_.zh * p.sC_h : nullptr;
+      auto store_tile = [&](auto staged_c) {
+        constexpr bool STAGED = decltype(staged_c)::value;
+#pragma unroll
+        for (int j = 0; j < BN / 8; ++j) {
+          if (p.geglu && (j & 4)) continue;
+          const int n = n0 + 8 * j + 2 * qd;
+          const int nout = p.geglu ? (n >> 6) * 32 + (n & 63) : n;
+          const int box = p.geglu ? j >> 3 : j >> 2, cc = 8 * (j & 3) + 2 * qd;
+          float cs[2] = {0.f, 0.f}, cq[2] = {0.f, 0.f};
+#pragma unroll
+          for (int i = 0; i < 2; ++i) {
+            float2 o = make_float2(tot[j * 4 + i * 2], tot[j * 4 + i * 2 + 1]);
+            if (p.geglu) {
+              const float g0 = tot[(j + 4) * 4 + i * 2], g1 = tot[(j + 4) * 4 + i * 2 + 1];
+              o.x *= 0.5f * g0 * (1.f + erff(g0 * 0.70710678118654752440f));
+              o.y *= 0.5f * g1 * (1.f + erff(g1 * 0.70710678118654752440f));
+            }
+            if (STAGED) {
+              const int r = r0 + 8 * i;
+              const uint32_t a = epi_box(box) + (uint32_t)r * 128u + ((((uint32_t)cc >> 2) ^ (uint32_t)(r & 7)) << 4) + (uint32_t)(cc & 3) * 4u;
+              if (p.residual) {
+                float2 rv;
+                asm volatile("ld.shared.v2.f32 {%0, %1}, [%2];" : "=f"(rv.x), "=f"(rv.y) : "r"(a));
+                o.x += rv.x;
+                o.y += rv.y;
+              }
+              asm volatile("st.shared.v2.f32 [%0], {%1, %2};" ::"r"(a), "f"(o.x), "f"(o.y) : "memory");
+            }
+            if (!rok[i] || n >= nend) continue;
+            if (!STAGED && p.residual) {
+              o.x += p.residual[mrow[i] * p.ldr + n];
+              o.y += p.residual[mrow[i] * p.ldr + n + 1];
+            }
+            if (p.c_stats) { cs[0] += o.x; cq[0] += o.x * o.x; cs[1] += o.y; cq[1] += o.y * o.y; }
+            if (!STAGED) {
+              float* const d = dst + mrow[i] * p.ldc + nout;
+              if (dst_lo) {
+                const uint32_t hx = rn_tf32(__float_as_uint(o.x)), hy = rn_tf32(__float_as_uint(o.y));
+                *reinterpret_cast<float2*>(dst_lo + mrow[i] * p.ldc + nout) = make_float2(__uint_as_float(tf32_lo(o.x, hx)), __uint_as_float(tf32_lo(o.y, hy)));
+                o = make_float2(__uint_as_float(hx), __uint_as_float(hy));
+              }
+              *reinterpret_cast<float2*>(d) = o;
+            }
+            omax = fmaxf(omax, fmaxf(fabsf(o.x), fabsf(o.y)));
           }
-        }
-      }
-    }
-  };
-
-  auto mma = [&](int it, const Frag& f) {
-    const uint32_t sb = base + (it % STAGES) * STAGE_BYTES + A_BYTES;
-    const uint64_t bhi = H16 ? make_desc_sw64(sb) : make_desc(sb), blo = H16 ? make_desc_sw64(sb + B_PLANE) : make_desc(sb + B_PLANE);
-    wgmma_pin(acc);
-    wgmma_fence();
-#pragma unroll
-    for (int kk = 0; kk < KSTEPS; ++kk) {
-      const uint64_t adv = (uint64_t)kk * 2u;
-      if (H16) {
-        if (!FAST) {
-          Wgmma<BN>::f16_rs(acc, f.l[kk], bhi + adv);
-          Wgmma<BN>::f16_rs(acc, f.h[kk], blo + adv);
-        }
-        Wgmma<BN>::f16_rs(acc, f.h[kk], bhi + adv);
-      } else {
-        Wgmma<BN>::tf32_rs(acc, f.l[kk], bhi + adv);
-        Wgmma<BN>::tf32_rs(acc, f.h[kk], blo + adv);
-        Wgmma<BN>::tf32_rs(acc, f.h[kk], bhi + adv);
-      }
-    }
-    wgmma_commit();
-  };
-
-  int kin = 0;
-  auto step = [&](int it, const Frag& cur, Frag& nxt) {
-    mma(it, cur);
-    wgmma_wait1();
-    if (it > 0) {
-      __syncwarp();
-      if (lane == 0) mbar_arrive(bar_empty((it - 1) % STAGES));
-    }
-    if (it + 1 < nst) load_split(it + 1, nxt);
-    if (++kin == kchunk || it == nst - 1) {
-      wgmma_wait0();
-      wgmma_pin(acc);
-#pragma unroll
-      for (int j = 0; j < NACC; ++j) { tot[j] += acc[j]; acc[j] = 0.f; }
-      kin = 0;
-    }
-  };
-
-  Frag fa, fb;
-  load_split(0, fa);
-#pragma unroll 1
-  for (int it = 0; it < nst; it += 2) {
-    step(it, fa, fb);
-    if (it + 1 < nst) step(it + 1, fb, fa);
-  }
-
-  const bool fin = p.splits == 1;
-  const float alpha = H16 ? p.alpha * exp2i(-ea) * exp2i(-p.b_exp) : p.alpha;
-  long long mrow[2];
-  bool rok[2];
-#pragma unroll
-  for (int i = 0; i < 2; ++i) {
-    const int r = r0 + 8 * i;
-    if (p.mode != 1) {
-      mrow[i] = (long long)tc_.m0 + r;
-      rok[i] = mrow[i] < p.M;
-    } else {
-      rok[i] = pb[i] < p.B && px[i] < p.W && py[i] < p.H;
-      mrow[i] = ((long long)pb[i] * p.H + py[i]) * p.W + px[i];
-    }
-  }
-  float omax = 0.f;
-  const int n0 = tc_.n0, nend = tc_.nend;
-  if (!fin) {
-    float* const dst = p.ws + (long long)tc_.split * p.M * p.N;
-#pragma unroll
-    for (int j = 0; j < BN / 8; ++j)
-#pragma unroll
-      for (int i = 0; i < 2; ++i)
-#pragma unroll
-        for (int c = 0; c < 2; ++c) {
-          const int n = n0 + 8 * j + 2 * qd + c;
-          if (rok[i] && n < nend) dst[mrow[i] * p.N + n] = tot[j * 4 + i * 2 + c];
-        }
-    return;
-  }
-#pragma unroll
-  for (int j = 0; j < BN / 8; ++j)
-#pragma unroll
-    for (int c = 0; c < 2; ++c) {
-      const int n = n0 + 8 * j + 2 * qd + c;
-      const float bv = (p.bias && n < nend) ? p.bias[n] : 0.f;
-#pragma unroll
-      for (int i = 0; i < 2; ++i) {
-        float v = alpha * tot[j * 4 + i * 2 + c] + bv;
-        if (p.rowvec && rok[i] && n < nend) v += p.rowvec[(mrow[i] / p.rows_per_batch) * p.ld_rowvec + n];
-        tot[j * 4 + i * 2 + c] = v;
-      }
-    }
-  if (p.out_nchw) {
-#pragma unroll
-    for (int i = 0; i < 2; ++i) {
-      if (!rok[i]) continue;
-      const long long bimg = mrow[i] / p.rows_per_img, rimg = mrow[i] - bimg * p.rows_per_img;
-#pragma unroll
-      for (int j = 0; j < BN / 8; ++j)
-#pragma unroll
-        for (int c = 0; c < 2; ++c) {
-          const int n = n0 + 8 * j + 2 * qd + c;
-          if (n < nend) p.C[(bimg * p.N + n) * p.rows_per_img + rimg] = tot[j * 4 + i * 2 + c];
-        }
-    }
-    return;
-  }
-  if (p.Ct_hi && n0 >= p.t_col0) {
-#pragma unroll
-    for (int j = 0; j < BN / 8; ++j)
-#pragma unroll
-      for (int i = 0; i < 2; ++i)
-#pragma unroll
-        for (int c = 0; c < 2; ++c) {
-          const int n = n0 + 8 * j + 2 * qd + c;
-          if (rok[i] && n < nend) {
-            const float o = tot[j * 4 + i * 2 + c];
-            const uint32_t hi = rn_tf32(__float_as_uint(o));
-            const long long at = (long long)(n - p.t_col0) * p.ldt + mrow[i];
-            p.Ct_hi[at] = __uint_as_float(hi);
-            p.Ct_lo[at] = __uint_as_float(tf32_lo(o, hi));
-            omax = fmaxf(omax, fabsf(o));
-          }
-        }
-  } else {
-    float* const dst = p.C + tc_.zb * p.sC_b + tc_.zh * p.sC_h;
-    float* const dst_lo = p.C_lo ? p.C_lo + tc_.zb * p.sC_b + tc_.zh * p.sC_h : nullptr;
-    auto store_tile = [&](auto staged_c) {
-      constexpr bool STAGED = decltype(staged_c)::value;
-#pragma unroll
-      for (int j = 0; j < BN / 8; ++j) {
-        if (p.geglu && (j & 4)) continue;
-        const int n = n0 + 8 * j + 2 * qd;
-        const int nout = p.geglu ? (n >> 6) * 32 + (n & 63) : n;
-        const int box = p.geglu ? j >> 3 : j >> 2, cc = 8 * (j & 3) + 2 * qd;
-        float cs[2] = {0.f, 0.f}, cq[2] = {0.f, 0.f};
-#pragma unroll
-        for (int i = 0; i < 2; ++i) {
-          float2 o = make_float2(tot[j * 4 + i * 2], tot[j * 4 + i * 2 + 1]);
-          if (p.geglu) {
-            const float g0 = tot[(j + 4) * 4 + i * 2], g1 = tot[(j + 4) * 4 + i * 2 + 1];
-            o.x *= 0.5f * g0 * (1.f + erff(g0 * 0.70710678118654752440f));
-            o.y *= 0.5f * g1 * (1.f + erff(g1 * 0.70710678118654752440f));
-          }
-          if (STAGED) {
-            const int r = r0 + 8 * i;
-            const uint32_t a = epi_box(box) + (uint32_t)r * 128u + ((((uint32_t)cc >> 2) ^ (uint32_t)(r & 7)) << 4) + (uint32_t)(cc & 3) * 4u;
-            if (p.residual) {
-              float2 rv;
-              asm volatile("ld.shared.v2.f32 {%0, %1}, [%2];" : "=f"(rv.x), "=f"(rv.y) : "r"(a));
-              o.x += rv.x;
-              o.y += rv.y;
+          if (p.c_stats) {
+#pragma unroll
+            for (int c = 0; c < 2; ++c) {
+#pragma unroll
+              for (int o2 = 4; o2 < 32; o2 <<= 1) {
+                cs[c] += __shfl_xor_sync(0xffffffffu, cs[c], o2);
+                cq[c] += __shfl_xor_sync(0xffffffffu, cq[c], o2);
+              }
             }
-            asm volatile("st.shared.v2.f32 [%0], {%1, %2};" ::"r"(a), "f"(o.x), "f"(o.y) : "memory");
-          }
-          if (!rok[i] || n >= nend) continue;
-          if (!STAGED && p.residual) {
-            o.x += p.residual[mrow[i] * p.ldr + n];
-            o.y += p.residual[mrow[i] * p.ldr + n + 1];
-          }
-          if (p.c_stats) { cs[0] += o.x; cq[0] += o.x * o.x; cs[1] += o.y; cq[1] += o.y * o.y; }
-          if (!STAGED) {
-            float* const d = dst + mrow[i] * p.ldc + nout;
-            if (dst_lo) {
-              const uint32_t hx = rn_tf32(__float_as_uint(o.x)), hy = rn_tf32(__float_as_uint(o.y));
-              *reinterpret_cast<float2*>(dst_lo + mrow[i] * p.ldc + nout) = make_float2(__uint_as_float(tf32_lo(o.x, hx)), __uint_as_float(tf32_lo(o.y, hy)));
-              o = make_float2(__uint_as_float(hx), __uint_as_float(hy));
-            }
-            *reinterpret_cast<float2*>(d) = o;
-          }
-          omax = fmaxf(omax, fmaxf(fabsf(o.x), fabsf(o.y)));
-        }
-        if (p.c_stats) {
-#pragma unroll
-          for (int c = 0; c < 2; ++c) {
-#pragma unroll
-            for (int o2 = 4; o2 < 32; o2 <<= 1) {
-              cs[c] += __shfl_xor_sync(0xffffffffu, cs[c], o2);
-              cq[c] += __shfl_xor_sync(0xffffffffu, cq[c], o2);
+            const long long mq = __shfl_sync(0xffffffffu, rok[0] ? mrow[0] : -1LL, 0);
+            if (g == 0 && mq >= 0 && n < nend) {
+              double* sp = p.c_stats + ((mq / p.rows_per_batch) * p.N + n) * 2;
+              atomicAdd(sp, (double)cs[0]); atomicAdd(sp + 1, (double)cq[0]);
+              atomicAdd(sp + 2, (double)cs[1]); atomicAdd(sp + 3, (double)cq[1]);
             }
           }
-          const long long mq = __shfl_sync(0xffffffffu, rok[0] ? mrow[0] : -1LL, 0);
-          if (g == 0 && mq >= 0 && n < nend) {
-            double* sp = p.c_stats + ((mq / p.rows_per_batch) * p.N + n) * 2;
-            atomicAdd(sp, (double)cs[0]); atomicAdd(sp + 1, (double)cq[0]);
-            atomicAdd(sp + 2, (double)cs[1]); atomicAdd(sp + 3, (double)cq[1]);
+        }
+      };
+      if (!staged) {
+        store_tile(std::false_type());
+      } else {
+        mbar_wait(bar_res, PERSIST ? item & 1 : 0);
+        if (threadIdx.x == 128) TL_STAMP(4);
+        store_tile(std::true_type());
+        asm volatile("fence.proxy.async.shared::cta;" ::: "memory");
+        asm volatile("bar.sync 2, 256;" ::: "memory");
+        if (PERSIST) {
+          if (threadIdx.x == 128) mbar_arrive(bar_out);
+        } else if (threadIdx.x == 128) {
+          const int c0 = p.geglu ? n0 / 2 : n0, ncols = p.geglu ? p.N / 2 : p.N;
+          for (int b = 0; b < (p.geglu ? BN / 64 : BN / TBK) && c0 + b * TBK < ncols; ++b) {
+            if (p.mode == 0) tma_store_2d(epi_box(b), &mapC, c0 + b * TBK, tc_.m0);
+            else tma_store_4d(epi_box(b), &mapC, c0 + b * TBK, tc_.x0, tc_.y0, tc_.b0);
           }
-        }
-      }
-    };
-    if (!staged) {
-      store_tile(std::false_type());
-    } else {
-      mbar_wait(bar_res, 0);
-      store_tile(std::true_type());
-      asm volatile("fence.proxy.async.shared::cta;" ::: "memory");
-      asm volatile("bar.sync 2, 256;" ::: "memory");
-      if (threadIdx.x == 128) {
-        const int c0 = p.geglu ? n0 / 2 : n0, ncols = p.geglu ? p.N / 2 : p.N;
-        for (int b = 0; b < (p.geglu ? BN / 64 : BN / TBK) && c0 + b * TBK < ncols; ++b) {
-          if (p.mode == 0) tma_store_2d(epi_box(b), &mapC, c0 + b * TBK, tc_.m0);
-          else tma_store_4d(epi_box(b), &mapC, c0 + b * TBK, tc_.x0, tc_.y0, tc_.b0);
-        }
-        bulk_commit();
-        bulk_wait0();
-      }
-    }
+          bulk_commit();
+          TL_STAMP(5);
+          bulk_wait0();
+          TL_STAMP(6);
+        }
+      }
+    }
+    omax_cta = PERSIST ? fmaxf(omax_cta, omax) : omax;
+    if (!PERSIST) break;
+    t += gridDim.x;
+    if (t >= p.total_tiles) break;
+    ++item;
+    g0 += nst;
+    tc_ = tile_coord(p, t, num_kb);
+    nst = tc_.kb1 - tc_.kb0;
   }
   if (p.c_amax) {
 #pragma unroll
-    for (int o = 16; o > 0; o >>= 1) omax = fmaxf(omax, __shfl_xor_sync(0xffffffffu, omax, o));
-    if (lane == 0) atomicMax(reinterpret_cast<unsigned int*>(p.c_amax), __float_as_uint(omax));
+    for (int o = 16; o > 0; o >>= 1) omax_cta = fmaxf(omax_cta, __shfl_xor_sync(0xffffffffu, omax_cta, o));
+    if (lane == 0) atomicMax(reinterpret_cast<unsigned int*>(p.c_amax), __float_as_uint(omax_cta));
   }
 }
 
@@ -595,9 +695,9 @@
   if ((threadIdx.x & 31) == 0) atomicMax(reinterpret_cast<unsigned int*>(slot), __float_as_uint(m));
 }
 
-template <int KIND, int BN>
+template <int KIND, int BN, bool PERSIST = false>
 void set_smem_attr() {
-  CDX_CUDA(cudaFuncSetAttribute(tc_gemm_kernel<KIND, BN>, cudaFuncAttributeMaxDynamicSharedMemorySize, Cfg<KIND, BN>::SMEM_BYTES));
+  CDX_CUDA(cudaFuncSetAttribute(tc_gemm_kernel<KIND, BN, PERSIST>, cudaFuncAttributeMaxDynamicSharedMemorySize, Cfg<KIND, BN, PERSIST>::SMEM_BYTES));
 }
 
 void ensure_attr(int device) {
@@ -613,6 +713,10 @@
     set_smem_attr<KIND_H16, 64>();
     set_smem_attr<KIND_H16_FAST, 128>();
     set_smem_attr<KIND_H16_FAST, 64>();
+    set_smem_attr<KIND_H16, 128, true>();
+    set_smem_attr<KIND_H16, 64, true>();
+    set_smem_attr<KIND_H16_FAST, 128, true>();
+    set_smem_attr<KIND_H16_FAST, 64, true>();
     attr_set[d] = true;
   }
 }
@@ -621,6 +725,12 @@
 void launch_gemm(const TcParams& p, const CUtensorMap& mA, const CUtensorMap& mA2, const CUtensorMap& mB, const CUtensorMap& mBlo,
                  const CUtensorMap& mR, const CUtensorMap& mC, cudaStream_t s) {
   launch_ex(tc_gemm_kernel<KIND, BN>, dim3((unsigned)p.total_tiles), dim3(TC_THREADS), Cfg<KIND, BN>::SMEM_BYTES, s, 1, mA, mA2, mB, mBlo, mR, mC, p);
+}
+
+template <int KIND, int BN>
+void launch_gemm_persist(const TcParams& p, int ctas, const CUtensorMap& mA, const CUtensorMap& mA2, const CUtensorMap& mB,
+                         const CUtensorMap& mBlo, const CUtensorMap& mR, const CUtensorMap& mC, cudaStream_t s) {
+  launch_ex(tc_gemm_kernel<KIND, BN, true>, dim3((unsigned)ctas), dim3(TC_THREADS), Cfg<KIND, BN, true>::SMEM_BYTES, s, 1, mA, mA2, mB, mBlo, mR, mC, p);
 }
 
 }
@@ -822,12 +932,14 @@
                    (!a.A2 || (a.C2 % TBK) == 0);
   const int bk = h16 ? 64 : TBK;
   const int num_kb = cdiv(a.K, bk);
+  const bool persist_ok = e.persist && h16 && a.mode == 0 && !a.out_nchw && !a.Cout_lo && !a.Ct_hi;
   int best_w = TBN, best_s = 1;
   {
     static std::map<std::array<int64_t, 6>, int> plan_cache;
     static std::mutex plan_mutex;
     std::lock_guard<std::mutex> plan_lock(plan_mutex);
-    const std::array<int64_t, 6> key = {a.M, p.tiles_m, a.N, num_kb, ((a.geglu || a.Ct_hi) ? 1 : 0) | (a.out_nchw ? 2 : 0) | (h16 ? 4 : 0) | (ts ? 8 : 0), e.num_sms};
+    const std::array<int64_t, 6> key = {a.M, p.tiles_m, a.N, num_kb, ((a.geglu || a.Ct_hi) ? 1 : 0) | (a.out_nchw ? 2 : 0) | (h16 ? 4 : 0) | (ts ? 8 : 0) |
+                                        (persist_ok ? 16 : 0), e.num_sms};
     const double kc0 = h16 ? 700.0 : 400.0, kc1 = h16 ? 6.0 : 3.0;
     const int min_kbs = h16 ? 4 : 8;
     auto it = plan_cache.find(key);
@@ -846,7 +958,8 @@
           const int Sx = cdiv(num_kb, kbs);
           if (S > 1 && (Sx != S || kbs < min_kbs || a.out_nchw || a.geglu || a.Ct_hi || (long long)p.tiles_m * tn >= 4LL * e.num_sms)) continue;
           const long long items = (long long)p.tiles_m * tn * S;
-          double cost = (double)cdiv(items, (long long)e.num_sms) * (kbs * (kc0 + kc1 * w) + 3000.0);
+          const double waves = (double)cdiv(items, (long long)e.num_sms);
+          double cost = S == 1 && persist_ok ? waves * kbs * (kc0 + kc1 * w) + 3000.0 : waves * (kbs * (kc0 + kc1 * w) + 3000.0);
           if (S == 1) base = cost;
           else cost += 4000.0 + (2.0 * S + 1.0) * (double)a.M * a.N * 4.0 / 3e12 * 1.8e9;
           if (cost < best - 1e-9 && (S == 1 || cost < 0.9 * base)) { best = cost; best_w = w; best_s = S; }
@@ -918,9 +1031,15 @@
   ensure_attr(e.device);
   ProfScope ps(e, s, a.mode == 1 ? PROF_CONV_TC : PROF_DENSE_TC, 2.0 * a.M * a.N * a.K,
                4.0 * ((double)a.M * a.K / (a.mode == 1 ? 9 : 1) + (double)a.N * a.K + (double)a.M * a.N), 1);
-  ps.note("M%d N%d K%d w%d tiles%d S%d %s%s%s%s box%dx%dx%d", a.M, a.N, a.K, p.tn_w, tiles, p.splits, h16 ? (fast ? "H16x1" : "H16") : ts ? "TS" : "SS",
-          a.Cout_lo ? " planes" : "", a.geglu ? " geglu" : "", a.residual ? " res" : "", p.bw, p.bh, p.bn);
-  if (fast && p.tn_w == 128) launch_gemm<KIND_H16_FAST, 128>(p, *mA, *mA2, *mB, *mBlo, *mR, *mC, s);
+  ps.note("M%d N%d K%d w%d tiles%d S%d %s%s%s%s%s box%dx%dx%d", a.M, a.N, a.K, p.tn_w, tiles, p.splits, h16 ? (fast ? "H16x1" : "H16") : ts ? "TS" : "SS",
+          a.Cout_lo ? " planes" : "", a.geglu ? " geglu" : "", a.residual ? " res" : "", persist_ok && staged_store(p) ? " persist" : "", p.bw, p.bh, p.bn);
+  const bool persist = persist_ok && staged_store(p);
+  const int ctas = (int)std::min<long long>(p.total_tiles, e.persist_grid > 0 ? std::min(e.persist_grid, e.num_sms) : e.num_sms);
+  if (persist && fast && p.tn_w == 128) launch_gemm_persist<KIND_H16_FAST, 128>(p, ctas, *mA, *mA2, *mB, *mBlo, *mR, *mC, s);
+  else if (persist && fast) launch_gemm_persist<KIND_H16_FAST, 64>(p, ctas, *mA, *mA2, *mB, *mBlo, *mR, *mC, s);
+  else if (persist && p.tn_w == 128) launch_gemm_persist<KIND_H16, 128>(p, ctas, *mA, *mA2, *mB, *mBlo, *mR, *mC, s);
+  else if (persist) launch_gemm_persist<KIND_H16, 64>(p, ctas, *mA, *mA2, *mB, *mBlo, *mR, *mC, s);
+  else if (fast && p.tn_w == 128) launch_gemm<KIND_H16_FAST, 128>(p, *mA, *mA2, *mB, *mBlo, *mR, *mC, s);
   else if (fast) launch_gemm<KIND_H16_FAST, 64>(p, *mA, *mA2, *mB, *mBlo, *mR, *mC, s);
   else if (h16 && p.tn_w == 128) launch_gemm<KIND_H16, 128>(p, *mA, *mA2, *mB, *mBlo, *mR, *mC, s);
   else if (h16) launch_gemm<KIND_H16, 64>(p, *mA, *mA2, *mB, *mBlo, *mR, *mC, s);
@@ -940,3 +1059,9 @@
 }
 
 }
+
+#ifdef CDX_GEMM_TIMELINE
+extern "C" int cdx_gemm_timeline_buffer(void* buf) {
+  return cudaMemcpyToSymbol(cdx::g_gemm_timeline, &buf, sizeof(buf)) == cudaSuccess ? 0 : 1;
+}
+#endif
diff --git a/cycle_diffusion_b200/engine.py b/cycle_diffusion_b200/engine.py
--- a/cycle_diffusion_b200/engine.py
+++ b/cycle_diffusion_b200/engine.py
@@ -70,6 +70,9 @@
     def set_mma_mode(self, mode):
         check(lib.cdx_engine_set_mma_mode(self.h, int(mode)))
         self.mma_mode = int(mode)
+
+    def set_persist(self, enable, max_ctas=0):
+        check(lib.cdx_engine_set_persist(self.h, int(bool(enable)), int(max_ctas)))
 
     PRECISIONS = {'full': None, 'autocast': 5}
 
diff --git a/include/cdx.h b/include/cdx.h
--- a/include/cdx.h
+++ b/include/cdx.h
@@ -29,6 +29,7 @@
 int cdx_engine_profile(cdx_engine* e, int enable);
 int cdx_engine_profile_read(cdx_engine* e, int tag, double* ms, double* flops, double* bytes, uint64_t* launches);
 int cdx_engine_set_mma_mode(cdx_engine* e, int mode);
+int cdx_engine_set_persist(cdx_engine* e, int enable, int max_ctas);
 
 #define CDX_UNET_OPENAI 1
 #define CDX_UNET_IDDPM 2
```

Measured after the change: 0.9082, median of 6. 1.12x the previous value.
